# OPPO-Mente-Lab/PEA-Diffusion

Hardware: AMD Instinct MI355X
Metric: training images/sec (SDXL 1024px bf16, adapter-only bwd) (higher is better)
Workload: dtype bf16

## Files before the change

include/pea_hip.h:

```cpp
#ifndef PEA_HIP_H
#define PEA_HIP_H
#include <stdint.h>
#ifdef __cplusplus
extern "C" {
#endif

#define PEA_OK 0
#define PEA_E_INVALID (-1)
#define PEA_E_HIP (-2)
#define PEA_E_SHAPE (-3)
#define PEA_E_STATE (-4)
#define PEA_E_NOTFOUND (-5)
#define PEA_E_TIMEOUT (-6)

const char* pea_last_error(void);
int pea_version(void);
int pea_device_count(void);


int pea_op_gemm(const void* A, int lda, const void* W, int ldw, void* C, int ldc, int M, int N, int K, float alpha,
                const float* bias, const void* rowvec, int ldrv, int rows_per_batch, int act, void* preact,
                int ldpre, const void* res, int ldres, int out_f32, int accum_f32, void* stream);

int pea_op_gemm_qscale(const void* A, int lda, const void* W, int ldw, void* C, int ldc, int M, int N, int K, const float* bias,
                       int qscale_cols, float qscale, void* stream);

int pea_op_gemm_geglu(const void* A, int lda, const void* W, int ldw, const float* bias, void* y, void* stash, int M, int N,
                      int K, int stash_grad, int stash_rows, void* stream);

int pea_op_gemm_geglu_bwd(const void* A, int lda, const void* W, int ldw, const void* pre, int ldpre, void* C, int ldc,
                          int M, int N, int K, int form, void* stream);

int pea_op_ln_linear(const void* x, const float* gamma, const float* beta, const void* W, const float* bias, void* y,
                     void* geglu_y, int M, int N, int K, float eps, void* Wf, float* svec, float* tvec, float* stats,
                     void* stream);

int pea_op_conv3x3(const void* x, const void* w, void* y, int B, int Hs, int Ws, int Cin, int Cout, int stride,
                   int upsample2x, int transposed2, const float* bias, const void* rowvec, int ldrv,
                   const void* res, void* stream);
int pea_op_pack_conv(const float* w, void* out, int Co, int Ci, int dgrad, void* stream);
int pea_op_gemm_geglu_tanh(const void* A, int lda, const void* W, int ldw, const float* bias, void* y, void* stash, int M, int N,
                           int K, int stash_grad, int stash_rows, int geglu_tanh, void* stream);
int pea_op_gemm_splitk(const void* A, int lda, const void* W, int ldw, float* part, int ldc, long long split_stride, int M, int N,
                       int K, float alpha, int ksplit, void* stream);
int pea_op_conv3x3_ex(const void* x, const void* w, int ldw, void* y, int ldc, int B, int Hs, int Ws, int Cin, int Cout,
                      int stride, int pad_off, int act, const float* bias, const void* res, int ldres, void* stream);
int pea_op_pack_conv_padded(const float* w, void* out, int Co, int Ci, int Cip, void* stream);
int pea_op_pack_conv_subpixel(const float* w, void* out, int Co, int Ci, int dgrad, void* stream);
int pea_op_concat2(const void* a, int C1, const void* b, int C2, void* y, long long rows, int aH, int aW, void* stream);
int pea_op_split2(const void* dy, int C1, int C2, void* da, int accum_a, void* db, int accum_b, long long rows, int aH,
                  int aW, void* stream);
long long pea_op_freeu_scratch_bytes(int B, int H, int W, int C2);
int pea_op_freeu_coef(const void* skip, int B, int H, int W, int C2, float* coef, void* scratch, void* stream);
int pea_op_concat2_freeu(const void* a, int C1, const void* b, int C2, const float* coef, void* y, int B, int H, int W, float s,
                         float bscale, int aH, int aW, void* stream);
int pea_op_upconv_subpixel(const void* x, const void* w, void* y, int B, int Hs, int Ws, int Cin, int Cout,
                           const float* bias, void* stream);
int pea_op_upconv_subpixel_dgrad(const void* dy, const void* wt, void* dx, int B, int Hs, int Ws, int Cin, int Cout,
                                 const void* res, void* stream);
int pea_op_conv_in(const float* x_nchw, const float* w, const float* bias, void* y_nhwc, int B, int Cin, int H,
                   int W, int Cout, void* stream);
int pea_op_conv_in_gather(const float* latents, const float* mask, const float* masked_latents, const float* w,
                          const float* bias, void* y_nhwc, int B, int C, int latent_batch, int cond_batch, int H, int W,
                          int Cout, void* stream);
// ... 17 lines not shown
                         float* dgamma, float* dbeta, int R, int C, int accum, void* stream);

int pea_op_attention_fwd(const void* Q, int ldq, const void* K, int ldk, const void* V, int ldv, void* O, int ldo,
                         float* lse, int B, int H, int Sq, int Skv, float scale, int nd, void* stream);
int pea_op_attention_fwd_prescaled(const void* Q, int ldq, const void* K, int ldk, const void* V, int ldv, void* O, int ldo,
                                   float* lse, int B, int H, int Sq, int Skv, float scale, int nd, void* stream);
int pea_op_attention_fwd_masked(const void* Q, int ldq, const void* K, int ldk, const void* V, int ldv, void* O, int ldo,
                                float* lse, int B, int H, int Sq, int Skv, float scale, int causal, const int* kv_len,
                                void* stream);
int pea_op_attention_fwd_text(const void* Q, int ldq, const void* K, int ldk, const void* V, int ldv, void* O, int ldo,
                              float* lse, int B, int H, int Sq, int Skv, float scale, int q_prescaled, int causal,
                              const int* kv_len, const float* bias, void* stream);
int pea_op_attention_fwd_ip(const void* Q, int ldq, const void* K, int ldk, const void* V, int ldv, const void* K2, int ldk2,
                            const void* V2, int ldv2, void* O, int ldo, float* lse, int B, int H, int Sq, int Skv, int Skv2,
                            float scale, float ip_scale, int q_prescaled, int causal, const int* kv_len, void* stream);
typedef struct pea_attn_ip_sets {
  int n_sets;
  int n_keys[4];
  float weight[4];
  const float* mask[4];
  long long mask_stride[4];
} pea_attn_ip_sets;
int pea_op_attention_fwd_ipn(const void* Q, int ldq, const void* K, int ldk, const void* V, int ldv, const void* K2, int ldk2,
                             const void* V2, int ldv2, void* O, int ldo, float* lse, int B, int H, int Sq, int Skv,
                             const pea_attn_ip_sets* sets, float scale, int q_prescaled, int causal, const int* kv_len, void* stream);
int pea_op_attention_fwd_fewq(const void* Q, int ldq, const void* K, int ldk, const void* V, int ldv, const void* K2, int ldk2,
                              const void* V2, int ldv2, void* O, int ldo, float* lse, int B, int H, int Sq, int Skv, int Skv2,
                              float scale, int nd, int q_prescaled, void* stream);
long long pea_op_attention_bwd_scratch_bytes(int B, int H, int Sq, int Skv, int nd);
int pea_op_attention_bwd(const void* Q, int ldq, const void* K, int ldk, const void* V, int ldv, const void* O,
                         int ldo, const void* dO, int lddo, const float* lse, float* delta, void* dQ, int lddq,
                         void* dK, int lddk, void* dV, int lddv, int B, int H, int Sq, int Skv, float scale,
                         int accum_dq, int accum_dkv, int nd, void* scratch, void* stream);

int pea_op_attention_bwd_prescaled(const void* Q, int ldq, const void* K, int ldk, const void* V, int ldv, const void* O,
                                   int ldo, const void* dO, int lddo, const float* lse, float* delta, void* dQ, int lddq,
                                   void* dK, int lddk, void* dV, int lddv, int B, int H, int Sq, int Skv, float scale,
                                   int accum_dq, int accum_dkv, int nd, void* scratch, void* stream);

int pea_op_attention_bwd_masked(const void* Q, int ldq, const void* K, int ldk, const void* V, int ldv, const void* O,
                                int ldo, const void* dO, int lddo, const float* lse, float* delta, void* dQ, int lddq,
                                void* dK, int lddk, void* dV, int lddv, int B, int H, int Sq, int Skv, float scale,
                                int accum_dq, int accum_dkv, int nd, void* scratch, int q_prescaled, const int* kv_len,
                                void* stream);

int pea_op_geglu_fwd(const void* hg, void* y, long long rows, int inner, void* stream);
int pea_op_geglu_bwd(const void* hg, const void* dy, void* dhg, long long rows, int inner, void* stream);
int pea_op_sumpool2(const void* x, void* y, int B, int H, int W, int C, int accum, void* stream);
int pea_op_timestep_embed(const float* t, void* y, int n, int dim, void* stream);
int pea_op_add_noise(const float* x0, const float* eps, const long long* t, const float* ac, float* xt, int B,
                     long long per, void* stream);
int pea_op_cast_f32_bf16(const float* x, void* y, long long n, void* stream);
int pea_op_cast_bf16_f32(const void* x, float* y, long long n, void* stream);

int pea_op_inpaint_prepare(const float* image, const float* mask, int N, int H, int W, float* init_image, float* masked_image,
                           float* latent_mask, void* stream);
long long pea_op_cfg_combine_workspace_bytes(int B);
int pea_op_cfg_combine(const float* eps2, float* out, int B, long long per, float guidance_scale, float guidance_rescale,
                       void* workspace, void* stream);
int pea_op_dpm_update(float* sample, const float* eps, float* x0_prev, long long n, float alpha_s, float sigma_s,
                      float c_s, float c_0, float c_1, void* stream);
int pea_op_lcm_update(float* sample, const float* eps, const float* noise, float* denoised, long long n, float kx, float ke,
                      float c_prev, float c_noise, void* stream);
int pea_op_euler_update(float* sample, const float* eps, const float* noise, float* model_in, long long n, int dup, float k_e,
                        float k_n, float k_s, void* stream);

// ... 72 lines not shown
  int heads[4];
  int cross_dim;
  int linear_proj;
  int groups;
  float eps;
  int text_time;
  int add_time_dim;
  int proj_in_dim;
  int per_layer_depth;
  int depth_down[4][4];
  int depth_up[4][4];
  int depth_mid;
} pea_unet_config;

#define PEA_UNET_GRAD 1
#define PEA_UNET_RESIDUAL_INPUTS 2
#define PEA_UNET_INPAINT_INPUTS 4
int pea_unet_create(const pea_unet_config* cfg, int B, int H, int W, int L, int flags, int own_weights,
                    void** out);
int pea_unet_plan(const pea_unet_config* cfg, int B, int H, int W, int L, int flags, int* n_ops, int* n_weights,
                  long long* n_params, long long* weight_bytes, long long* act_bytes, long long* grad_bytes);
int pea_unet_create_cond(const pea_unet_config* cfg, int B, int H, int W, int L, int flags, int time_cond_proj_dim,
                         int own_weights, void** out);
int pea_unet_plan_cond(const pea_unet_config* cfg, int B, int H, int W, int L, int flags, int time_cond_proj_dim, int* n_ops,
                       int* n_weights, long long* n_params, long long* weight_bytes, long long* act_bytes,
                       long long* grad_bytes, int* n_attn, int* n_prescaled);
int pea_unet_plan_weight(const pea_unet_config* cfg, int B, int H, int W, int L, int flags, int time_cond_proj_dim,
                         const char* name, long long* numel, int* kind, int* d0, int* d1);
int pea_unet_set_timestep_cond(void* unet, const float* cond, void* stream);
int pea_unet_plan_scratch(const pea_unet_config* cfg, int B, int H, int W, int L, int flags, int bwd_batch,
                          long long* scratch_bytes);
int pea_tape_attention_census(void* graph, int* n_attn, int* n_prescaled);
int pea_unet_plan_attention(const pea_unet_config* cfg, int B, int H, int W, int L, int flags, int* n_attn, int* n_prescaled);
int pea_graph_plan_attention(int graph, const pea_unet_config* cfg, int B, int H, int W, int L, int* n_attn,
                             int* n_prescaled);
int pea_unet_num_residuals(void* unet);
int pea_unet_residual_info(void* unet, int i, int* C, int* H, int* W);
int pea_unet_set_residuals(void* unet, int n, const void* const* ptrs, int dtype, float scale, void* stream);
int pea_unet_set_inpaint_cond(void* unet, const float* mask, const float* masked_latents, int cond_batch, int latent_batch,
                              void* stream);
int pea_unet_clear_inpaint_cond(void* unet);
int pea_unet_set_freeu(void* unet, float s1, float s2, float b1, float b2, void* stream);
int pea_unet_clear_freeu(void* unet);
int pea_unet_ip_plan(const pea_unet_config* cfg, int n_tokens, int* n_layers, int* cols, long long* n_params);
int pea_unet_ip_create(void* unet, int n_tokens);
int pea_unet_ip_load_weight(void* unet, const char* key, const float* src, long long numel, void* stream);
int pea_unet_ip_set_tokens(void* unet, const float* tokens, void* stream);
int pea_unet_ip_set_scale(void* unet, float scale);
int pea_unet_ip_clear(void* unet);
int pea_unet_ip_destroy(void* unet);
int pea_unet_ip_export_kv(void* unet, float* out, long long* rows, int* cols, void* stream);
int pea_unet_ip_create_sets(void* unet, int n_sets, const int* n_tokens);
int pea_unet_ip_load_weight_set(void* unet, int set, const char* key, const float* src, long long numel, void* stream);
int pea_unet_ip_set_tokens_set(void* unet, int set, const float* tokens, void* stream);
int pea_unet_ip_set_scale_set(void* unet, int set, float scale);
int pea_unet_ip_clear_set(void* unet, int set);
int pea_unet_ip_set_layer_scales(void* unet, int set, const float* scales, int n_layers);
int pea_unet_ip_query_counts(void* unet, int* counts, int cap, int* n);
int pea_unet_ip_set_mask(void* unet, int set, int Sq, const float* mask, int Bm, void* stream);
int pea_unet_destroy(void* unet);

int pea_controlnet_create(const pea_unet_config* cfg, int B, int H, int W, int L, void** out);
int pea_controlnet_set_cond(void* cn, const float* image, void* stream);
int pea_controlnet_forward(void* cn, const float* x, const float* t, const void* ehs, int ehs_dtype, const void* text,
                           int text_dtype, const float* time_ids, void* stream);
int pea_controlnet_num_outputs(void* cn);
// ... 90 lines not shown
                   const long long* zh_or_not, const float* teacher_ehs, const float* teacher_neg,
                   const float* teacher_pooled, const float* time_ids, float grad_scale, float* grads,
                   int accumulate, float* losses, void* stream);
int pea_trainer_set_option(void* tr, const char* name, int value);
int pea_trainer_backward_context(void* trainer, void** unet);
int pea_trainer_get_option(void* trainer, const char* name);
int pea_trainer_release_activations(void* trainer);
int pea_trainer_export(void* tr, int which, float* out, void* stream);

int pea_comm_unique_id(void* out128);
int pea_comm_init(int rank, int world, const void* unique_id128, void** comm_out);
int pea_comm_init_timeout(int rank, int world, const void* unique_id128, double timeout_s, void** comm_out);
int pea_comm_destroy(void* comm);
int pea_comm_world(void* comm);
int pea_comm_rank(void* comm);
int pea_allreduce_grads(void* comm, float* grads, long long n, void* compute_stream);
int pea_comm_join(void* comm, void* stream);
int pea_comm_last_ms(void* comm, float* ms);
int pea_comm_last_exposed_ms(void* comm, float* ms);
int pea_comm_broadcast(void* comm, float* buf, long long n, int root, void* stream);

void pea_prof_enable(int on);
void pea_prof_reset(void);
const char* pea_prof_family_name(int fam);
int pea_prof_dump(const char* path);
int pea_prof_report(int fam, double* ms, double* flops, double* bytes, long long* launches);
int pea_probe_mfma_peak(double seconds, int shape32, double* tflops, double* clock_mhz, void* stream);

void pea_debug_set_attn_tr(int v);
void pea_debug_set_attn_fused_bwd(int v);
void pea_debug_set_attn_xattn(int v);
void pea_debug_set_xattn_bwd_v2(int v);
void pea_debug_set_geglu_bwd_fused(int v);
void pea_debug_set_gemm_variant(int v);
int pea_debug_gemm_dispatch(int M, int N, int K, int mode, int rows_per_batch, int features, int cus, int forced);
int pea_debug_attn_dispatch(const int* q, int* out);
void pea_debug_set_gemm_debug(int v);
void pea_debug_set_gemm_prefetch(const void* p, long long bytes);

int pea_op_attention_fwd_regions(const void* Q, int ldq, const void* K, int ldk, const void* V, int ldv, void* O, int ldo, int B, int H,
                                 int Sq, int R, int Lr, const float* w, int Bw, float scale, int q_prescaled, void* stream);
int pea_unet_set_prompt_regions(void* unet, int R, int Sq, const float* w, int Bw, void* stream);
int pea_unet_clear_prompt_regions(void* unet);
int pea_debug_attn_regions_dispatch(const int* q, int* out);

int pea_op_attention_maps(const void* Q, int ldq, const void* K, int ldk, float* maps, int B, int H, int Sq, int Skv, float scale,
                          int q_prescaled, const int* kv_len, int accumulate, void* stream);
int pea_unet_enable_attention_maps(void* unet, const float* layer_on, int n_layers);
int pea_unet_reset_attention_maps(void* unet, void* stream);
int pea_unet_disable_attention_maps(void* unet);
int pea_unet_attention_maps(void* unet, int Sq, float** maps, long long* n_accumulated);
int pea_debug_attn_maps_dispatch(const int* q, int* out);

int pea_op_attention_fwd_edit(const void* Q, int ldq, const void* K, int ldk, const void* V, int ldv, void* O, int ldo, int B, int H,
                              int Sq, int Skv, const int* src, const void* Mt, int ldm, const float* c, const float* d, float scale,
                              int q_prescaled, void* stream);
int pea_unet_set_prompt_edit(void* unet, const int* src, const void* Mt, const float* cd, int T, int self_until, int self_max_tokens,
                             void* stream);
int pea_unet_set_prompt_edit_step(void* unet, int step);
int pea_unet_clear_prompt_edit(void* unet);
int pea_debug_attn_edit_dispatch(const int* q, int* out);

long long pea_op_attn_adain_scratch_bytes(int B, int H, int S);
int pea_op_attn_adain_coef(const void* Q, int ldq, const void* K, int ldk, int B, int H, int S, const int* ref, float scale,
                           int q_prescaled, int adain_queries, int adain_keys, float* coef, void* scratch, void* stream);
int pea_op_attention_fwd_shared(const void* Q, int ldq, const void* K, int ldk, const void* V, int ldv, void* O, int ldo, int B, int H,
// ... 42 lines not shown
```

pea_diffusion_amd/csrc/api_model.hip:

```cpp
#include <string.h>

#include <algorithm>
#include <memory>

#include "../../include/pea_hip.h"
#include "model.h"

#define RCX(x)                        \
  do {                                \
    int rc__ = (x);                   \
    if (rc__ != PEA_OK) return rc__;  \
  } while (0)
static_assert(sizeof(pea_unet_config) == sizeof(PeaUnetCfg), "config struct mismatch");

static int finish_create(Tape* u, void** out) {
  int rc = u->build();
  if (rc == PEA_OK) rc = u->alloc();
  if (rc != PEA_OK) {
    delete u;
    return rc;
  }
  *out = u;
  return PEA_OK;
}
// ... 103 lines not shown
  Tape u;
  memcpy(&u.cfg, cfg, sizeof(PeaUnetCfg));
  u.B = B; u.H = H; u.W = W; u.L = L; set_flags(u, flags);
  u.bwd_batch = bwd_batch;
  u.plan_only = true;
  int rc = u.build();
  if (rc == PEA_OK) rc = u.alloc();
  if (rc != PEA_OK) return rc;
  size_t need[8];
  u.scratch_needs(need);
  long long t = 0;
  for (int i = 0; i < 8; ++i) t += (long long)need[i];
  *scratch_bytes = t;
  return PEA_OK;
}
int pea_tape_attention_census(void* h, int* n_attn, int* n_prescaled) {
  NOTNULL(h, "pea_tape_attention_census");
  const Tape* u = (const Tape*)h;
  if (n_attn) *n_attn = u->n_attn;
  if (n_prescaled) *n_prescaled = u->n_attn_pre;
  return PEA_OK;
}
int pea_unet_plan_attention(const pea_unet_config* cfg, int B, int H, int W, int L, int flags, int* n_attn, int* n_prescaled) {
  NOTNULL(cfg, "pea_unet_plan_attention");
  Tape u;
  memcpy(&u.cfg, cfg, sizeof(PeaUnetCfg));
  u.B = B; u.H = H; u.W = W; u.L = L; set_flags(u, flags);
  u.plan_only = true;
  int rc = u.build();
  if (rc == PEA_OK) rc = u.alloc();
  if (rc != PEA_OK) return rc;
  if (n_attn) *n_attn = u.n_attn;
  if (n_prescaled) *n_prescaled = u.n_attn_pre;
  return PEA_OK;
}
static int plan_census(Tape& u, int* n_attn, int* n_prescaled) {
  u.plan_only = true;
  int rc = u.build();
  if (rc == PEA_OK) rc = u.alloc();
  if (rc != PEA_OK) return rc;
  if (n_attn) *n_attn = u.n_attn;
  if (n_prescaled) *n_prescaled = u.n_attn_pre;
  return PEA_OK;
}
int pea_graph_plan_attention(int graph, const pea_unet_config* cfg, int B, int H, int W, int L, int* n_attn, int* n_prescaled) {
  NOTNULL(cfg, "pea_graph_plan_attention");
  if (graph < 1 || graph > 3) { pea_set_error("pea_graph_plan_attention: graph %d (1 VAE encoder, 2 ControlNet, 3 VAE decoder)", graph); return PEA_E_INVALID; }
  Tape u;
  memcpy(&u.cfg, cfg, sizeof(PeaUnetCfg));
  u.graph = graph;
  u.B = B; u.H = H; u.W = W; u.L = graph == 2 ? L : 0; u.needs_grad = false; u.owns_weights = true;
  return plan_census(u, n_attn, n_prescaled);
}
int pea_text_plan_attention(const pea_text_config* cfg, int B, int L, int* n_attn, int* n_prescaled) {
  NOTNULL(cfg, "pea_text_plan_attention");
  Tape u;
  memset(&u.cfg, 0, sizeof(PeaUnetCfg));
  memcpy(&u.tcfg, cfg, sizeof(PeaTextCfg));
  u.graph = 4;
  u.B = B; u.H = 1; u.W = L; u.L = L; u.needs_grad = false; u.owns_weights = true;
  return plan_census(u, n_attn, n_prescaled);
}
int pea_controlnet_create(const pea_unet_config* cfg, int B, int H, int W, int L, void** out) {
  NOTNULL(cfg, "pea_controlnet_create");
  NOTNULL(out, "pea_controlnet_create");
  RCX(require_device("pea_controlnet_create"));
// ... 621 lines not shown
```

pea_diffusion_amd/csrc/api_ops.hip:

```cpp
#include <stdarg.h>
#include <string.h>

#include "../../include/pea_hip.h"
#include "pea_kernels.h"

static thread_local char g_err[512] = "";
void pea_set_error(const char* fmt, ...) {
  va_list ap;
  va_start(ap, fmt);
  vsnprintf(g_err, sizeof(g_err), fmt, ap);
  va_end(ap);
}

static bf16* g_zero_page = nullptr;
int pea_zero_page(const bf16** out) {
  if (!g_zero_page) {
    HIPCHK(hipMalloc((void**)&g_zero_page, 256));
    HIPCHK(hipMemset(g_zero_page, 0, 256));
  }
  *out = g_zero_page;
  return PEA_OK;
}

template <class P = AttnP>
// ... 34 lines not shown
}

int pea_op_gemm(const void* A, int lda, const void* W, int ldw, void* C, int ldc, int M, int N, int K, float alpha,
                const float* bias, const void* rowvec, int ldrv, int rows_per_batch, int act, void* preact,
                int ldpre, const void* res, int ldres, int out_f32, int accum_f32, void* stream) {
  GemmP p;
  memset(&p, 0, sizeof(p));
  p.mode = 0;
  p.A = (const bf16*)A; p.lda = lda; p.W = (const bf16*)W; p.ldw = ldw; p.C = C; p.ldc = ldc;
  p.M = M; p.N = N; p.K = K; p.alpha = alpha; p.bias = bias;
  p.rowvec = (const bf16*)rowvec; p.ldrv = ldrv; p.rows_per_batch = rows_per_batch > 0 ? rows_per_batch : 1;
  p.act = act; p.preact = (bf16*)preact; p.ldpre = ldpre; p.res = (const bf16*)res; p.ldres = ldres;
  p.out_f32 = out_f32; p.accum_f32 = accum_f32;
  return launch_gemm(p, (hipStream_t)stream);
}

int pea_op_gemm_qscale(const void* A, int lda, const void* W, int ldw, void* C, int ldc, int M, int N, int K, const float* bias,
                       int qscale_cols, float qscale, void* stream) {
  GemmP p;
  memset(&p, 0, sizeof(p));
  p.A = (const bf16*)A; p.lda = lda; p.W = (const bf16*)W; p.ldw = ldw; p.C = C; p.ldc = ldc;
  p.M = M; p.N = N; p.K = K; p.alpha = 1.f; p.bias = bias; p.rows_per_batch = 1;
  p.qscale_cols = qscale_cols; p.qscale = qscale;
  return launch_gemm(p, (hipStream_t)stream);
}

int pea_op_gemm_geglu_bwd(const void* A, int lda, const void* W, int ldw, const void* pre, int ldpre, void* C, int ldc,
                          int M, int N, int K, int form, void* stream) {
  GemmP p;
  memset(&p, 0, sizeof(p));
  p.A = (const bf16*)A; p.lda = lda; p.W = (const bf16*)W; p.ldw = ldw; p.C = C; p.ldc = ldc;
  p.M = M; p.N = N; p.K = K; p.alpha = 1.f; p.rows_per_batch = 1;
  p.gbwd_pre = (const bf16*)pre; p.ldgp = ldpre; p.gbwd_form = form;
  return launch_gemm(p, (hipStream_t)stream);
}

int pea_op_gemm_geglu(const void* A, int lda, const void* W, int ldw, const float* bias, void* y, void* stash, int M, int N,
                      int K, int stash_grad, int stash_rows, void* stream) {
  GemmP p;
  memset(&p, 0, sizeof(p));
  p.A = (const bf16*)A; p.lda = lda; p.W = (const bf16*)W; p.ldw = ldw; p.bias = bias;
  p.M = M; p.N = N; p.K = K; p.alpha = 1.f; p.rows_per_batch = 1;
  p.geglu_y = (bf16*)y; p.ldy = N / 2; p.C = stash; p.ldc = N; p.stash_grad = stash_grad; p.stash_rows = stash_rows;
  return launch_gemm(p, (hipStream_t)stream);
}

int pea_op_gemm_geglu_tanh(const void* A, int lda, const void* W, int ldw, const float* bias, void* y, void* stash, int M, int N,
                           int K, int stash_grad, int stash_rows, int geglu_tanh, void* stream) {
  GemmP p;
  memset(&p, 0, sizeof(p));
  p.A = (const bf16*)A; p.lda = lda; p.W = (const bf16*)W; p.ldw = ldw; p.bias = bias;
  p.M = M; p.N = N; p.K = K; p.alpha = 1.f; p.rows_per_batch = 1;
  p.geglu_y = (bf16*)y; p.ldy = N / 2; p.C = stash; p.ldc = N; p.stash_grad = stash_grad; p.stash_rows = stash_rows;
  p.geglu_tanh = geglu_tanh ? 1 : 0;
  return launch_gemm(p, (hipStream_t)stream);
}

int pea_op_gemm_splitk(const void* A, int lda, const void* W, int ldw, float* part, int ldc, long long split_stride, int M, int N,
                       int K, float alpha, int ksplit, void* stream) {
  GemmP p;
  memset(&p, 0, sizeof(p));
  p.A = (const bf16*)A; p.lda = lda; p.W = (const bf16*)W; p.ldw = ldw; p.C = part; p.ldc = ldc;
  SHAPECHK(ksplit >= 2, "gemm_splitk: ksplit=%d (at least two splits)", ksplit);
  p.M = M; p.N = N; p.K = K; p.alpha = alpha; p.rows_per_batch = 1; p.out_f32 = 1;
  p.ksplit = ksplit; p.split_stride = split_stride;
  return launch_gemm(p, (hipStream_t)stream);
// ... 239 lines not shown
  return launch_attention_fwd_edit(p, (hipStream_t)stream);
}
long long pea_op_attn_adain_scratch_bytes(int B, int H, int S) { return (long long)attn_adain_scratch_bytes(B, H, S); }
int pea_op_attn_adain_coef(const void* Q, int ldq, const void* K, int ldk, int B, int H, int S, const int* ref, float scale,
                           int q_prescaled, int adain_queries, int adain_keys, float* coef, void* scratch, void* stream) {
  if (!ref) { pea_set_error("pea_op_attn_adain_coef: null ref (a host int[B]; negative entries for plain samples)"); return PEA_E_INVALID; }
  return launch_attn_adain_coef((const bf16*)Q, ldq, (const bf16*)K, ldk, B, H, S, ref, scale, q_prescaled, adain_queries, adain_keys,
                                coef, (float*)scratch, (hipStream_t)stream);
}
int pea_op_attention_fwd_shared(const void* Q, int ldq, const void* K, int ldk, const void* V, int ldv, void* O, int ldo, int B, int H,
                                int Sq, int Skv, const int* ref, const float* coef, float scale, int q_prescaled,
                                float shared_score_scale, float shared_score_shift, int nd, void* stream) {
  if (!ref) { pea_set_error("pea_op_attention_fwd_shared: null ref (a host int[B]; negative entries for plain samples)"); return PEA_E_INVALID; }
  AttnSharedP p = attn_operands<AttnSharedP>(Q, ldq, K, ldk, V, ldv, O, ldo, nullptr, B, H, Sq, Skv, scale, nd, q_prescaled);
  p.coef = coef; p.share_scale = shared_score_scale; p.share_shift = shared_score_shift;
  for (int b = 0; b < 32; ++b) p.ref[b] = b < B ? ref[b] : -1;
  return launch_attention_fwd_shared(p, (hipStream_t)stream);
}
int pea_op_attention_fwd_fewq(const void* Q, int ldq, const void* K, int ldk, const void* V, int ldv, const void* K2, int ldk2,
                              const void* V2, int ldv2, void* O, int ldo, float* lse, int B, int H, int Sq, int Skv, int Skv2,
                              float scale, int nd, int q_prescaled, void* stream) {
  AttnP p = attn_operands(Q, ldq, K, ldk, V, ldv, O, ldo, lse, B, H, Sq, Skv, scale, nd);
  p.q_prescaled = q_prescaled;
  p.K2 = (const bf16*)K2; p.V2 = (const bf16*)V2; p.ldk2 = ldk2; p.ldv2 = ldv2; p.Skv2 = Skv2;
  return launch_attention_fwd_fewq(p, (hipStream_t)stream);
}
int pea_op_attention_bwd(const void* Q, int ldq, const void* K, int ldk, const void* V, int ldv, const void* O,
                         int ldo, const void* dO, int lddo, const float* lse, float* delta, void* dQ, int lddq,
                         void* dK, int lddk, void* dV, int lddv, int B, int H, int Sq, int Skv, float scale,
                         int accum_dq, int accum_dkv, int nd, void* scratch, void* stream) {
  return attention_bwd_impl(Q, ldq, K, ldk, V, ldv, O, ldo, dO, lddo, lse, delta, dQ, lddq, dK, lddk, dV, lddv, B, H, Sq, Skv,
                            scale, accum_dq, accum_dkv, nd, scratch, 0, nullptr, stream);
}
int pea_op_attention_bwd_prescaled(const void* Q, int ldq, const void* K, int ldk, const void* V, int ldv, const void* O,
                                   int ldo, const void* dO, int lddo, const float* lse, float* delta, void* dQ, int lddq,
                                   void* dK, int lddk, void* dV, int lddv, int B, int H, int Sq, int Skv, float scale,
                                   int accum_dq, int accum_dkv, int nd, void* scratch, void* stream) {
  return attention_bwd_impl(Q, ldq, K, ldk, V, ldv, O, ldo, dO, lddo, lse, delta, dQ, lddq, dK, lddk, dV, lddv, B, H, Sq, Skv,
                            scale, accum_dq, accum_dkv, nd, scratch, 1, nullptr, stream);
}
int pea_op_attention_bwd_masked(const void* Q, int ldq, const void* K, int ldk, const void* V, int ldv, const void* O,
                                int ldo, const void* dO, int lddo, const float* lse, float* delta, void* dQ, int lddq,
                                void* dK, int lddk, void* dV, int lddv, int B, int H, int Sq, int Skv, float scale,
                                int accum_dq, int accum_dkv, int nd, void* scratch, int q_prescaled, const int* kv_len,
                                void* stream) {
  return attention_bwd_impl(Q, ldq, K, ldk, V, ldv, O, ldo, dO, lddo, lse, delta, dQ, lddq, dK, lddk, dV, lddv, B, H, Sq, Skv,
                            scale, accum_dq, accum_dkv, nd, scratch, q_prescaled, kv_len, stream);
}

int pea_op_geglu_fwd(const void* hg, void* y, long long rows, int inner, void* stream) {
  return launch_geglu_fwd((const bf16*)hg, (bf16*)y, rows, inner, (hipStream_t)stream);
}
int pea_op_geglu_bwd(const void* hg, const void* dy, void* dhg, long long rows, int inner, void* stream) {
  return launch_geglu_bwd((const bf16*)hg, (const bf16*)dy, (bf16*)dhg, rows, inner, (hipStream_t)stream);
}
int pea_op_sumpool2(const void* x, void* y, int B, int H, int W, int C, int accum, void* stream) {
  return launch_sumpool2((const bf16*)x, (bf16*)y, B, H, W, C, accum, (hipStream_t)stream);
}
int pea_op_timestep_embed(const float* t, void* y, int n, int dim, void* stream) {
  return launch_timestep_embed(t, (bf16*)y, n, dim, (hipStream_t)stream);
}
int pea_op_add_noise(const float* x0, const float* eps, const long long* t, const float* ac, float* xt, int B,
                     long long per, void* stream) {
  return launch_add_noise(x0, eps, t, ac, xt, B, per, (hipStream_t)stream);
}
int pea_op_cast_f32_bf16(const float* x, void* y, long long n, void* stream) {
// ... 252 lines not shown
```

pea_diffusion_amd/csrc/attention.hip:

```cpp
#include <stdlib.h>

#include "pea_kernels.h"

#define TILE_BYTES 8192
__device__ __forceinline__ float fast_exp2(float x) { return __builtin_amdgcn_exp2f(x); }
#define LOG2E 1.4426950408889634f
__device__ __forceinline__ float xhalf_max(float x) {
  float a = x, b = x;
  asm volatile("s_nop 1\n\tv_permlane32_swap_b32 %0, %1\n\ts_nop 1" : "+v"(a), "+v"(b));
  return fmaxf(a, b);
}

__device__ __forceinline__ bf16x8 scale_frag(bf16x8 f, float c) {
  bf16x8 o;
#pragma unroll
  for (int j = 0; j < 8; ++j) o[j] = (bf16)((float)f[j] * c);
  return o;
}
#define ATTN_MOVE_THR 8.0f

__device__ __forceinline__ int swz_x(int row) {
  const int x = (row >> 1) & 7;
  return ((x & 1) << 2) | (x >> 1);
}
// ... 227 lines not shown
      const float e = fast_exp2(sacc[kb][r]);
      sacc[kb][r] = e;
      ls += e;
    }
  l_run += ls;
  return mx;
}
__device__ __forceinline__ void attn_pack_p(const f32x16 (&sacc)[2], bf16x8 (&pf)[4]) {
#pragma unroll
  for (int ks = 0; ks < 4; ++ks)
#pragma unroll
    for (int j = 0; j < 8; ++j) pf[ks][j] = (bf16)sacc[ks >> 1][8 * (ks & 1) + j];
}
template <bool USE_TR>
__device__ __forceinline__ void attn_cols_product(const char* smem, const AttnFragOff& ro, int sub, const char* Ts, int lane,
                                                  const bf16x8 (&pf)[4], f32x16* acc) {
  bf16x8 tfr[4][2];
#pragma unroll
  for (int ks = 0; ks < 4; ++ks)
#pragma unroll
    for (int db = 0; db < 2; ++db) {
      if constexpr (USE_TR)
        tfr[ks][db] = read_transposed_frag_at(smem + ro.tr[db][0] + (sub + ks * 2048), smem + ro.tr[db][1] + (sub + ks * 2048));
      else tfr[ks][db] = read_transposed_frag<false>(Ts, ks * 16, db * 32, lane);
    }
  __builtin_amdgcn_sched_barrier(0);
#pragma unroll
  for (int ks = 0; ks < 4; ++ks)
#pragma unroll
    for (int db = 0; db < 2; ++db) acc[db] = __builtin_amdgcn_mfma_f32_32x32x16_bf16(tfr[ks][db], pf[ks], acc[db], 0, 0, 0);
}
template <int NO>
__device__ __forceinline__ void attn_fwd_exit(const f32x16 (&oacc)[2 * NO], float m_run, float l_run, float* lse, long long lse_i,
                                              bool lse_lane, char* ost, int lane, bf16* Ob, int ldo, int q0, int Sq) {
  float la = l_run, lb = l_run;
  swap_halves32(la, lb);
  const float l_tot = la + lb;
  const float inv = 1.f / l_tot;
  if (lse && lse_lane) lse[lse_i] = (m_run + log2f(l_tot)) * 0.6931471805599453f;
#pragma unroll
  for (int no = 0; no < NO; ++no)
    store_o_image_144(ost, lane, [&](int db, int i) { return oacc[2 * no + db][i] * inv; }, Ob + no * 64, ldo, q0, Sq);
}

template <int MODE, bool USE_TR, int ND, bool TXT, bool WRITE_DELTA>
__device__ __forceinline__ void attn_q_body(const AttnP& p, char* smem, int blk_x, int head, int b) {
  constexpr int STG = 2 * ND * TILE_BYTES;
  constexpr int NO = MODE == 0 ? ND : 1;
  const int tid = threadIdx.x, lane = tid & 63;
  const int wave = __builtin_amdgcn_readfirstlane(tid >> 6);
  const int qblk = MODE == 0 ? blk_x : blk_x / ND;
  const int chunk = MODE == 0 ? 0 : blk_x % ND;
  const int q0 = qblk * 128 + wave * 32;
  const int frow = lane & 31, fh = lane >> 5;
  const float c = p.scale * LOG2E;

  const bf16* Qb = p.Q + (long long)b * p.Sq * p.ldq + head * 64 * ND;
  const bf16* Kb = p.K + (long long)b * p.Skv * p.ldk + head * 64 * ND;
  const bf16* Vb = p.V + (long long)b * p.Skv * p.ldv + head * 64 * ND;

  int qrow = q0 + frow;
  const bool qvalid = qrow < p.Sq;
  qrow = qvalid ? qrow : p.Sq - 1;
  bf16x8 qf[ND][4], dof[MODE == 1 ? ND : 1][4];
#pragma unroll
  for (int nd = 0; nd < ND; ++nd)
#pragma unroll
    for (int s = 0; s < 4; ++s) {
      qf[nd][s] = *(const bf16x8*)(Qb + (long long)qrow * p.ldq + nd * 64 + 16 * s + 8 * fh);
      if (!p.q_prescaled && !TXT) qf[nd][s] = scale_frag(qf[nd][s], c);
    }
  [[maybe_unused]] const float qs = (TXT && !p.q_prescaled) ? c : 1.f;
  [[maybe_unused]] const float inv_qs = (TXT && !p.q_prescaled) ? 1.f / c : 1.f;
  float lse2 = 0.f, dlt = 0.f;
  if (MODE == 1) {
    const bf16* dOb = p.dO + (long long)b * p.Sq * p.lddo + head * 64 * ND;
#pragma unroll
    for (int nd = 0; nd < ND; ++nd)
#pragma unroll
      for (int s = 0; s < 4; ++s)
        dof[nd][s] = *(const bf16x8*)(dOb + (long long)qrow * p.lddo + nd * 64 + 16 * s + 8 * fh);
    const long long li = ((long long)b * p.H + head) * p.Sq + qrow;
    if (!WRITE_DELTA) {
      dlt = -p.delta[li];
      lse2 = -p.delta[(long long)p.B * p.H * p.Sq + li];
    } else {
      lse2 = p.lse[li] * LOG2E;
      const bf16* Ob = p.O + (long long)b * p.Sq * p.ldo + head * 64 * ND;
      float dsum = 0.f;
#pragma unroll
      for (int nd = 0; nd < ND; ++nd)
#pragma unroll
        for (int s = 0; s < 4; ++s) {
          const bf16x8 o = *(const bf16x8*)(Ob + (long long)qrow * p.ldo + nd * 64 + 16 * s + 8 * fh);
#pragma unroll
          for (int j = 0; j < 8; ++j) dsum += (float)dof[nd][s][j] * (float)o[j];
        }
      { float da = dsum, db = dsum; swap_halves32(da, db); dsum = da + db; }
      dlt = dsum;
      if (WRITE_DELTA && qvalid && fh == 0 && chunk == 0) {
        p.delta[li] = -dsum;
        p.delta[(long long)p.B * p.H * p.Sq + li] = -lse2;
      }
    }
  }
  f32x16 negd, rowc;
#pragma unroll
  for (int r = 0; r < 16; ++r) { negd[r] = -dlt; rowc[r] = MODE == 1 ? -lse2 : 0.f; }

  f32x16 oacc[2 * NO];
#pragma unroll
  for (int i = 0; i < 2 * NO; ++i)
#pragma unroll
    for (int r = 0; r < 16; ++r) oacc[i][r] = 0.f;
  float m_run = 0.f, l_run = 0.f;
  [[maybe_unused]] bool seen = false;

  TileSrc ksrc[ND], vsrc[ND];
#pragma unroll
  for (int nd = 0; nd < ND; ++nd) {
    ksrc[nd] = tile_src(Kb + nd * 64, p.ldk, p.Skv, wave, lane);
    vsrc[nd] = tile_src(Vb + nd * 64, p.ldv, p.Skv, wave, lane);
  }
  auto stage_kv = [&](char* dst, int r0) {
#pragma unroll
    for (int nd = 0; nd < ND; ++nd) {
      stage_tile(ksrc[nd], r0, dst + nd * TILE_BYTES, wave);
      stage_tile(vsrc[nd], r0, dst + (ND + nd) * TILE_BYTES, wave);
    }
  };
  const int nt = (p.Skv + 63) / 64;
  const int skv_all = __builtin_amdgcn_readfirstlane(p.kv_len ? p.kv_len[b] : p.Skv);
  stage_kv(smem, 0);
// ... 41 lines not shown
        attn_mask_tail(sacc, kv0, kmax, fh);
      }
      const float mx = attn_online_softmax<TXT>(sacc, TXT ? !seen : t == 0, m_run, l_run, oacc, rowc,
                                                [&](float m) { return TXT ? -m * inv_qs : -m; });
      if constexpr (TXT) seen = seen || mx > -INFINITY;
    } else {
      const int skv_b = skv_all;
      f32x16 dpacc[2];
      attn_rows_product<ND>(smem, ro, ND * TILE_BYTES, dof, negd, dpacc);
      if (kv0 + 64 > skv_b) {
        attn_mask_tail(sacc, kv0, skv_b, fh);
        __builtin_amdgcn_sched_barrier(0);
      }
#pragma unroll
      for (int kb = 0; kb < 2; ++kb)
#pragma unroll
        for (int r = 0; r < 16; ++r) {
          const float pr = fast_exp2(sacc[kb][r]);
          sacc[kb][r] = pr * dpacc[kb][r];
        }
    }
    bf16x8 pf[4];
    attn_pack_p(sacc, pf);
#pragma unroll
    for (int no = 0; no < NO; ++no)
      attn_cols_product<USE_TR>(smem, ro, no * TILE_BYTES, MODE == 0 ? Vs + no * TILE_BYTES : Ks + chunk * TILE_BYTES, lane, pf, oacc + 2 * no);
    WAIT_VM0();
    __syncthreads();
  }

  char* const ost = smem + wave * (32 * 144);
  if constexpr (MODE == 0)
    attn_fwd_exit<NO>(oacc, m_run, l_run, p.lse, ((long long)b * p.H + head) * p.Sq + qrow, qvalid && fh == 0, ost, lane,
                      p.O + (long long)b * p.Sq * p.ldo + head * 64 * ND, p.ldo, q0, p.Sq);
  else
    store_o_image_144(ost, lane, [&](int db, int i) { return oacc[db][i] * p.scale; }, p.dQ + (long long)b * p.Sq * p.lddq + head * 64 * ND + chunk * 64,
                      p.lddq, q0, p.Sq, p.accum_dq != 0);
}

template <int MODE, bool USE_TR, int ND, bool TXT = false>
__global__ __launch_bounds__(256, (ND == 1 ? (MODE == 0 ? 3 : 2) : 1)) void attn_q_kernel(const AttnP p) {
  extern __shared__ __attribute__((aligned(16))) char smem[];
  int blk_x, head, b;
  attn_block_coords(blk_x, head, b);
  attn_q_body<MODE, USE_TR, ND, TXT, true>(p, smem, blk_x, head, b);
}

struct AttnKeyLane { int k0, krow; bool kstored, wave_active; };
__device__ __forceinline__ AttnKeyLane attn_key_lane(int kblk, int wave, int frow, int Skv) {
  AttnKeyLane k;
  k.k0 = kblk * 128 + wave * 32;
  k.kstored = k.k0 + frow < Skv;
  k.krow = k.kstored ? k.k0 + frow : Skv - 1;
  k.wave_active = k.k0 < Skv;
  return k;
}
__device__ __forceinline__ void stage_rowconst(const float* src, int r0, int rmax, char* dst, int lane) {
  int r = r0 + lane;
  r = r < rmax ? r : rmax - 1;
  lds_dma4(src + r, dst);
}

template <bool USE_TR, int ND>
__device__ __forceinline__ void attn_dkv_body(const AttnP& p, char* smem, int blk_x, int head, int b) {
  constexpr int STG = 2 * ND * TILE_BYTES + 512;
  const int tid = threadIdx.x, lane = tid & 63;
  const int wave = __builtin_amdgcn_readfirstlane(tid >> 6);
  const int nsplit = p.nsplit > 1 ? p.nsplit : 1;
  const int chunk = blk_x % ND;
  const int bx = blk_x / ND;
  const int kblk = bx / nsplit, split = bx - kblk * nsplit;
  const int frow = lane & 31, fh = lane >> 5;
  const auto [k0, krow, kstored, wave_active] = attn_key_lane(kblk, wave, frow, p.Skv);
  const float c = p.scale * LOG2E;

  const bf16* Qb = p.Q + (long long)b * p.Sq * p.ldq + head * 64 * ND;
  const bf16* dOb = p.dO + (long long)b * p.Sq * p.lddo + head * 64 * ND;
  const bf16* Kb = p.K + (long long)b * p.Skv * p.ldk + head * 64 * ND;
  const bf16* Vb = p.V + (long long)b * p.Skv * p.ldv + head * 64 * ND;
  const float* dltb = p.delta + ((long long)b * p.H + head) * p.Sq;
  const float* lseb = dltb + (long long)p.B * p.H * p.Sq;

  const int skv_b = p.kv_len ? p.kv_len[b] : p.Skv;
  const bool kvalid = k0 + frow < skv_b;
  bf16x8 kf[ND][4], vf[ND][4];
#pragma unroll
  for (int nd = 0; nd < ND; ++nd)
#pragma unroll
    for (int s = 0; s < 4; ++s) {
      kf[nd][s] = *(const bf16x8*)(Kb + (long long)krow * p.ldk + nd * 64 + 16 * s + 8 * fh);
      if (!p.q_prescaled) kf[nd][s] = scale_frag(kf[nd][s], c);
      vf[nd][s] = *(const bf16x8*)(Vb + (long long)krow * p.ldv + nd * 64 + 16 * s + 8 * fh);
    }
  f32x16 dk[2], dv[2];
#pragma unroll
  for (int i = 0; i < 2; ++i)
#pragma unroll
    for (int r = 0; r < 16; ++r) dk[i][r] = dv[i][r] = 0.f;
  const bool all_valid = __all(kvalid);

  TileSrc qsrc[ND], dosrc[ND];
#pragma unroll
  for (int nd = 0; nd < ND; ++nd) {
    qsrc[nd] = tile_src(Qb + nd * 64, p.ldq, p.Sq, wave, lane);
    dosrc[nd] = tile_src(dOb + nd * 64, p.lddo, p.Sq, wave, lane);
  }
  auto stage_q = [&](char* dst, int r0) {
#pragma unroll
    for (int nd = 0; nd < ND; ++nd) {
      stage_tile(qsrc[nd], r0, dst + nd * TILE_BYTES, wave);
      stage_tile(dosrc[nd], r0, dst + (ND + nd) * TILE_BYTES, wave);
    }
    if (wave == 0) {
      stage_rowconst(lseb, r0, p.Sq, dst + 2 * ND * TILE_BYTES, lane);
      stage_rowconst(dltb, r0, p.Sq, dst + 2 * ND * TILE_BYTES + 256, lane);
    }
  };
  const int nt_all = (p.Sq + 63) / 64;
  const int tps = (nt_all + nsplit - 1) / nsplit;
  const int t_begin = split * tps;
  const int nt = min(nt_all, t_begin + tps);
  if (t_begin < nt) stage_q(smem, t_begin * 64);
  WAIT_VM0();
  __syncthreads();

  for (int t = t_begin; t < nt; ++t) {
    const int cur = (t - t_begin) & 1;
    if (t + 1 < nt) stage_q(smem + (cur ^ 1) * STG, (t + 1) * 64);
    const char* Qs = smem + cur * STG;
    const char* dOs = Qs + ND * TILE_BYTES;
    const float* rc = (const float*)(Qs + 2 * ND * TILE_BYTES);
    if (t * 64 + 64 > p.Sq) {
      if (wave == 0 && t * 64 + lane >= p.Sq) {
        float* rw = (float*)(Qs + 2 * ND * TILE_BYTES);
        rw[lane] = -INFINITY;
        rw[64 + lane] = 0.f;
      }
      __syncthreads();
    }
    if (wave_active) {
      f32x16 sacc[2], dpacc[2];
      bf16x8 rq[2][ND * 4], rd[2][ND * 4];
      auto load_rows = [&](int buf, int qb) {
#pragma unroll
        for (int nd = 0; nd < ND; ++nd)
#pragma unroll
          for (int s = 0; s < 4; ++s) {
            rq[buf][nd * 4 + s] = read_row_frag(Qs + nd * TILE_BYTES, qb * 32 + frow, s, fh);
            rd[buf][nd * 4 + s] = read_row_frag(dOs + nd * TILE_BYTES, qb * 32 + frow, s, fh);
          }
#pragma unroll
        for (int g = 0; g < 4; ++g) {
          const f32x4 d4 = *(const f32x4*)(rc + 64 + qb * 32 + 8 * g + 4 * fh);
          const f32x4 l4 = *(const f32x4*)(rc + qb * 32 + 8 * g + 4 * fh);
#pragma unroll
          for (int j = 0; j < 4; ++j) {
            dpacc[qb][4 * g + j] = d4[j];
            sacc[qb][4 * g + j] = l4[j];
          }
        }
      };
// ... 26 lines not shown
        __builtin_amdgcn_sched_barrier(0);
      }
      bf16x8 pfr[4], dsfr[4];
#pragma unroll
      for (int qb = 0; qb < 2; ++qb)
#pragma unroll
        for (int g = 0; g < 4; ++g) {
#pragma unroll
          for (int j = 0; j < 4; ++j) {
            const int r = 4 * g + j;
            const float pr = fast_exp2(sacc[qb][r]);
            const float ds = pr * dpacc[qb][r];
            const int ks = qb * 2 + (g >> 1), e = (g & 1) * 4 + j;
            pfr[ks][e] = (bf16)pr;
            dsfr[ks][e] = (bf16)ds;
          }
        }
      __builtin_amdgcn_sched_barrier(0);
      load_tr(0);
      load_tr(1);
      __builtin_amdgcn_sched_barrier(0);
#pragma unroll
      for (int bt = 0; bt < 2; ++bt) {
#pragma unroll
        for (int kk = 0; kk < 2; ++kk)
#pragma unroll
          for (int db = 0; db < 2; ++db) {
            dv[db] = __builtin_amdgcn_mfma_f32_32x32x16_bf16(dot[bt][kk][db], pfr[2 * bt + kk], dv[db], 0, 0, 0);
            dk[db] = __builtin_amdgcn_mfma_f32_32x32x16_bf16(qt[bt][kk][db], dsfr[2 * bt + kk], dk[db], 0, 0, 0);
          }
        __builtin_amdgcn_sched_barrier(0);
      }
    }
    WAIT_VM0();
    __syncthreads();
  }
  const bool lds_epi = p.nsplit <= 1 && !p.accum_dkv;
  if (lds_epi ? !wave_active : !kstored) return;
#pragma unroll
  for (int i = 0; i < 2; ++i)
#pragma unroll
    for (int r = 0; r < 16; ++r) dk[i][r] *= p.q_prescaled ? 0.6931471805599453f : p.scale;
  const int D = 64 * ND;
  if (p.nsplit > 1) {
    float* pr = p.dkv_part + ((((long long)split * p.B + b) * p.H + head) * p.Skv + krow) * 2 * D + chunk * 64;
#pragma unroll
    for (int db = 0; db < 2; ++db)
#pragma unroll
      for (int g = 0; g < 4; ++g) {
        const int d = db * 32 + 8 * g + 4 * fh;
        f32x4 a, cc;
#pragma unroll
        for (int j = 0; j < 4; ++j) { a[j] = dk[db][4 * g + j]; cc[j] = dv[db][4 * g + j]; }
        *(f32x4*)(pr + d) = a;
        *(f32x4*)(pr + D + d) = cc;
      }
    return;
  }
  if (lds_epi) {
    char* const ost = smem + wave * (32 * 144);
    store_o_image_144(ost, lane, [&](int db, int i) { return dk[db][i]; }, p.dK + (long long)b * p.Skv * p.lddk + head * D + chunk * 64,
                      p.lddk, k0, p.Skv, p.accum_dkv != 0);
    store_o_image_144(ost, lane, [&](int db, int i) { return dv[db][i]; }, p.dV + (long long)b * p.Skv * p.lddv + head * D + chunk * 64,
                      p.lddv, k0, p.Skv, p.accum_dkv != 0);
    return;
  }
  bf16* dKr = p.dK + ((long long)b * p.Skv + krow) * p.lddk + head * D + chunk * 64;
  bf16* dVr = p.dV + ((long long)b * p.Skv + krow) * p.lddv + head * D + chunk * 64;
#pragma unroll
  for (int db = 0; db < 2; ++db)
#pragma unroll
    for (int g = 0; g < 4; ++g) {
      const int d = db * 32 + 8 * g + 4 * fh;
      bf16x4 ok, ov;
      if (p.accum_dkv) {
        ok = *(const bf16x4*)(dKr + d);
        ov = *(const bf16x4*)(dVr + d);
      }
#pragma unroll
      for (int j = 0; j < 4; ++j) {
        ok[j] = (bf16)(dk[db][4 * g + j] + (p.accum_dkv ? (float)ok[j] : 0.f));
        ov[j] = (bf16)(dv[db][4 * g + j] + (p.accum_dkv ? (float)ov[j] : 0.f));
      }
      *(bf16x4*)(dKr + d) = ok;
      *(bf16x4*)(dVr + d) = ov;
    }
}

template <bool USE_TR, int ND>
__global__ __launch_bounds__(256, (ND == 1 ? 2 : 1)) void attn_dkv_kernel(const AttnP p) {
  extern __shared__ __attribute__((aligned(16))) char smem[];
  int blk_x, head, b;
  attn_block_coords(blk_x, head, b);
  attn_dkv_body<USE_TR, ND>(p, smem, blk_x, head, b);
}

template <bool USE_TR, int ND>
__global__ __launch_bounds__(256, (ND == 1 ? 2 : 1)) void attn_bwd_fused_kernel(const AttnP p, int n_dq, int n_dkv) {
  extern __shared__ __attribute__((aligned(16))) char smem[];
  const unsigned lin = xcd_contiguous(blockIdx.x, gridDim.x);
  const int per_head = n_dq + n_dkv;
  const int bh = (int)(lin / per_head), rem = (int)(lin - (unsigned)bh * per_head);
  const int b = bh / p.H, head = bh - b * p.H;
  if (rem < n_dkv) attn_dkv_body<USE_TR, ND>(p, smem, rem, head, b);
  else attn_q_body<1, USE_TR, ND, false, false>(p, smem, rem - n_dkv, head, b);
}

struct XattnCtx {
  int split, head, b, u_begin, u_end, skv_b;
  float c;
  const bf16 *Qb, *dOb, *Ob, *Kb, *Vb;
  const float* lseb;
};
template <int UQ, int PRE = -1>
__device__ __forceinline__ XattnCtx xattn_ctx(const AttnP& p, int upw) {
  XattnCtx x;
  attn_block_coords(x.split, x.head, x.b);
  const int nu = (p.Sq + UQ - 1) >> (UQ == 128 ? 7 : 6);
  x.u_begin = x.split * upw;
  x.u_end = min(nu, x.u_begin + upw);
  x.c = (PRE < 0 ? p.q_prescaled != 0 : PRE != 0) ? 1.f : p.scale * LOG2E;
  x.Qb = p.Q + (long long)x.b * p.Sq * p.ldq + x.head * 64;
  x.dOb = p.dO + (long long)x.b * p.Sq * p.lddo + x.head * 64;
  x.Ob = p.O + (long long)x.b * p.Sq * p.ldo + x.head * 64;
  x.Kb = p.K + (long long)x.b * p.Skv * p.ldk + x.head * 64;
  x.Vb = p.V + (long long)x.b * p.Skv * p.ldv + x.head * 64;
  x.lseb = p.lse + ((long long)x.b * p.H + x.head) * p.Sq;
  x.skv_b = __builtin_amdgcn_readfirstlane(p.kv_len ? p.kv_len[x.b] : p.Skv);
  return x;
}
__device__ __forceinline__ float xhalf_sum(float x) {
  float a = x, b = x;
  asm volatile("s_nop 1\n\tv_permlane32_swap_b32 %0, %1\n\ts_nop 1" : "+v"(a), "+v"(b));
  return a + b;
}

__device__ __forceinline__ f32x16 zero_f32x16() {
  return f32x16{0.f, 0.f, 0.f, 0.f, 0.f, 0.f, 0.f, 0.f, 0.f, 0.f, 0.f, 0.f, 0.f, 0.f, 0.f, 0.f};
// ... 1665 lines not shown
  if (idx >= total) return;
  const int d4 = (int)(idx % D4) * 4;
  long long r = idx / D4;
  const int which = (int)(r & 1); r >>= 1;
  const int key = (int)(r % p.Skv); r /= p.Skv;
  const int head = (int)(r % p.H);
  const int b = (int)(r / p.H);
  f32x4 acc = {0.f, 0.f, 0.f, 0.f};
  for (int s = 0; s < p.nsplit; ++s) {
    const f32x4 v = *(const f32x4*)(p.dkv_part + ((((long long)s * p.B + b) * p.H + head) * p.Skv + key) * 2 * D +
                                    which * D + d4);
#pragma unroll
    for (int j = 0; j < 4; ++j) acc[j] += v[j];
  }
  bf16* dst = which ? p.dV + ((long long)b * p.Skv + key) * p.lddv + head * D + d4
                    : p.dK + ((long long)b * p.Skv + key) * p.lddk + head * D + d4;
  bf16x4 o;
  if (p.accum_dkv) o = *(const bf16x4*)dst;
#pragma unroll
  for (int j = 0; j < 4; ++j) o[j] = (bf16)(acc[j] + (p.accum_dkv ? (float)o[j] : 0.f));
  *(bf16x4*)dst = o;
}

enum AttnKernel : int {
  AK_XFWD = 0, AK_Q = 12, AK_Q_TXT = 24, AK_DKV = 25, AK_FUSED = 31, AK_XBWD1 = 37, AK_XBWD2 = 41, AK_XBWD3 = 45, AK_FEWQ = 49,
  AK_DELTA = 50, AK_REDUCE = 51, AK_COUNT = 52
};
struct AttnLaunch { int kernel; dim3 grid; int lds, a0, a1; };
struct AttnPlan {
  AttnLaunch l[3]; int n = 0, nsplit = 1;
  void add(int kernel, dim3 grid, int lds, int a0 = 0, int a1 = 0) { l[n++] = AttnLaunch{kernel, grid, lds, a0, a1}; }
};
struct AttnEnv { int xattn_ver, use_tr, xattn, fused_bwd; };
static AttnEnv g_attn_env = {getenv("PEA_XATTN_BWD_VER") ? atoi(getenv("PEA_XATTN_BWD_VER")) : 3, 1, getenv("PEA_XATTN_OFF") ? 0 : 1,
                             getenv("PEA_ATTN_BWD_SPLIT") ? 0 : 1};
extern "C" void pea_debug_set_xattn_bwd_v2(int v) { g_attn_env.xattn_ver = v; }
extern "C" void pea_debug_set_attn_tr(int v) { g_attn_env.use_tr = v; }
extern "C" void pea_debug_set_attn_xattn(int v) { g_attn_env.xattn = v; }
extern "C" void pea_debug_set_attn_fused_bwd(int v) { g_attn_env.fused_bwd = v; }
static bool xattn_v2_keys(int Skv, const AttnEnv& e) { return e.xattn_ver && Skv > 32 && Skv <= 96; }
static int wgs_per_cu(int lds) { return 2 * lds <= 160 * 1024 ? 2 : 1; }
static int wg_slots(int per_cu) { return 256 * per_cu; }
static int units_per_wg(long long units, int nu, int per_cu) {
  const long long upw = (units + wg_slots(per_cu) - 1) / wg_slots(per_cu);
  return (int)(upw < 1 ? 1 : (upw > nu ? nu : upw));
}
static int attn_nsplit(int B, int H, int Sq, int Skv, const AttnEnv& e) {
  if (Skv > 128 || Sq < 512) return 1;
  const bool v2 = xattn_v2_keys(Skv, e);
  const int uq = v2 ? 64 : 128;
  const int fixed = v2 ? 2 : 0;
  const int nu = (Sq + uq - 1) / uq;
  const long long bh = (long long)B * H;
  long long best = -1;
  int best_ns = 1;
  for (int u = 1; u <= nu; ++u) {
    const int ns = (nu + u - 1) / u;
    const long long rounds = (bh * ns + wg_slots(2) - 1) / wg_slots(2);
    const long long cost = rounds * (u + fixed) * (uq / 2) + ns;
    if (best < 0 || cost < best) { best = cost; best_ns = ns; }
  }
  return best_ns;
}
int attention_bwd_nsplit(int B, int H, int Sq, int Skv) { return attn_nsplit(B, H, Sq, Skv, g_attn_env); }
size_t attention_bwd_scratch_bytes(int B, int H, int Sq, int Skv, int nd) {
  const int ns = attention_bwd_nsplit(B, H, Sq, Skv);
  return ns > 1 ? (size_t)ns * B * H * Skv * 128 * nd * sizeof(float) : 0;
}
static bool attn_resident_kv(const AttnP& p, const AttnEnv& e) { return e.xattn && e.use_tr && p.nd == 1 && p.Skv <= 128; }
static int attn_decide_fwd(const AttnP& p, const AttnEnv& e, AttnPlan& plan) {
  const int nu = cdiv(p.Sq, 128);
  if (p.K2 || (attn_resident_kv(p, e) && !p.causal && !p.bias && p.Sq >= 128)) {
    const int kb = cdiv(p.Skv, 32), kt = (kb + 1) / 2;
    const int lds = 2 * kt * TILE_BYTES + 4 * 32 * 144 + 4 * 4096 + (p.K2 ? 2 * 4096 : 0);
    const int upw = units_per_wg((long long)p.B * p.H * nu, nu, 2);
    plan.add(AK_XFWD + 4 * (!p.K2 ? 0 : p.nset ? 2 : 1) + (kb - 1), dim3(cdiv(nu, upw), p.H, p.B), lds, upw);
    return PEA_OK;
  }
  const bool txt = p.causal || p.kv_len || p.bias;
  SHAPECHK(!txt || p.nd == 1, "attention: causal / key-length masks need head_dim 64");
  plan.add(txt ? AK_Q_TXT : AK_Q + 3 * (e.use_tr != 0) + (p.nd - 1), dim3(nu, p.H, p.B), 2 * 2 * p.nd * TILE_BYTES);
  return PEA_OK;
}
static int attn_decide_bwd(const AttnP& p, const AttnEnv& e, AttnPlan& plan) {
  const int ns = plan.nsplit = p.dkv_part ? attn_nsplit(p.B, p.H, p.Sq, p.Skv, e) : 1;
  const int nd = p.nd, tr = e.use_tr != 0;
  bool all = p.dQ && p.dK && p.dV, partials = true;
  if (attn_resident_kv(p, e) && all) {
    const int kb = cdiv(p.Skv, 32);
    const dim3 grid(ns, p.H, p.B);
    if (xattn_v2_keys(p.Skv, e)) {
      const bool v3 = e.xattn_ver != 2 && p.Skv <= 80;
      const int lds = v3 ? 2 * (TILE_BYTES + TILE_BYTES / 2) + 2 * (2 * TILE_BYTES + 512) + 2 * (TILE_BYTES + 2048)
                         : 4 * TILE_BYTES + 2 * (2 * TILE_BYTES + 512) + 2 * 32 * 144;
      plan.add((v3 ? AK_XBWD3 : AK_XBWD2) + 2 * (kb - 2) + (p.q_prescaled != 0), grid, lds, cdiv(cdiv(p.Sq, 64), ns));
    } else {
      plan.add(AK_XBWD1 + (kb - 1), grid, 4 * TILE_BYTES + (4 * TILE_BYTES + 1024), cdiv(cdiv(p.Sq, 128), ns));
    }
  } else {
    const int lq = 2 * 2 * nd * TILE_BYTES, lk = 2 * (2 * nd * TILE_BYTES + 512);
    const int n_dq = cdiv(p.Sq, 128) * nd, n_dkv = cdiv(p.Skv, 128) * ns * nd;
    const bool fused = all && e.fused_bwd;
    if (fused || !p.dQ) plan.add(AK_DELTA, dim3((unsigned)cdivl((long long)p.B * p.Sq * p.H * 8, 256 * ATTN_DELTA_ROWS)), 0);
    partials = fused || (p.dK && p.dV);
    if (fused) plan.add(AK_FUSED + 3 * tr + (nd - 1), dim3((unsigned)((n_dq + n_dkv) * p.H * p.B)), lk, n_dq, n_dkv);
    if (!fused && p.dQ) plan.add(AK_Q + 6 + 3 * tr + (nd - 1), dim3(n_dq, p.H, p.B), lq);
    if (!fused && partials) plan.add(AK_DKV + 3 * tr + (nd - 1), dim3(n_dkv, p.H, p.B), lk);
  }
  if (ns > 1 && partials) plan.add(AK_REDUCE, dim3((unsigned)cdivl((long long)p.B * p.H * p.Skv * 2 * 16 * nd, 256)), 0);
  return PEA_OK;
}
static int attn_check_ip(const AttnP& p) {
  SHAPECHK(p.K2 != nullptr && p.V2 != nullptr, "attention: a second key set needs both K2 and V2");
  SHAPECHK(p.nd == 1, "attention: a second key set needs head_dim 64 (nd=%d)", p.nd);
  SHAPECHK(!p.causal && !p.bias, "attention: a second key set cannot be combined with a causal mask or a score bias");
  SHAPECHK(p.Skv <= 128, "attention: a second key set needs at most 128 text keys (Skv=%d)", p.Skv);
  SHAPECHK(p.Skv2 >= 1 && p.Skv2 <= 32, "attention: the second key set holds 1..32 keys (Skv2=%d)", p.Skv2);
  SHAPECHK(p.ldk2 % 8 == 0 && p.ldv2 % 8 == 0 && p.ldk2 >= 64 * p.H && p.ldv2 >= 64 * p.H,
           "attention: ldk2 / ldv2 must be multiples of 8 and hold every head (ldk2=%d ldv2=%d)", p.ldk2, p.ldv2);
  SHAPECHK(p.nset >= 0 && p.nset <= 4, "attention: 1..4 image key sets (%d)", p.nset);
  for (int j = 0, lo = 0; j < p.nset; lo = p.set_end[j++]) {
    SHAPECHK(p.set_end[j] > lo, "attention: image key set %d is empty", j);
    SHAPECHK(!p.set_mask[j] || p.set_mstride[j] == 0 || p.set_mstride[j] >= p.Sq,
             "attention: the mask of image key set %d has batch stride %lld: 0 (shared) or >= Sq=%d", j, p.set_mstride[j], p.Sq);
  }
  SHAPECHK(p.nset == 0 || p.set_end[p.nset - 1] == p.Skv2, "attention: the image key sets end at row %d of %d", p.set_end[p.nset - 1], p.Skv2);
  return PEA_OK;
}
static void attn_resolve_sets(AttnP& p) {
  if (!p.nset) return;
  bool any = false;
  for (int j = 0; j < p.nset; ++j) any = any || p.set_w[j] != 0.f;
  if (!any) {
    p.K2 = p.V2 = nullptr;
    p.nset = 0;
  } else if (p.nset == 1 && !p.set_mask[0]) {
// ... 46 lines not shown
    SHAPECHK(p.k2_brows == 0 || p.k2_brows >= p.Skv2, "attention: %d image key rows per sample hold no %d keys", p.k2_brows, p.Skv2);
    if (!p.k2_brows) p.k2_brows = p.Skv2;
    attn_resolve_sets(p);
  }
  return attn_decide_fwd(p, e, plan);
}
template <auto K, int THREADS = 256, int LIMIT = 0, typename... Args>
static int launch_lds(dim3 grid, int bytes, hipStream_t s, const Args&... args) {
  static bool raised = false;
  if (!raised) {
    HIPCHK(hipFuncSetAttribute((const void*)K, hipFuncAttributeMaxDynamicSharedMemorySize, LIMIT ? LIMIT : bytes));
    raised = true;
  }
  hipLaunchKernelGGL(K, grid, dim3(THREADS), bytes, s, args...);
  return PEA_OK;
}
static int attn_launch(const AttnLaunch& l, const AttnP& p, hipStream_t s) {
#define ATTN_CASE(e, K, ...) case e: return launch_lds<K>(l.grid, l.lds, s, p, ##__VA_ARGS__);
  switch (l.kernel) {
    ATTN_CASE(AK_XFWD + 0, (xattn_fwd_kernel<1, false, false>), l.a0) ATTN_CASE(AK_XFWD + 1, (xattn_fwd_kernel<2, false, false>), l.a0)
    ATTN_CASE(AK_XFWD + 2, (xattn_fwd_kernel<3, false, false>), l.a0) ATTN_CASE(AK_XFWD + 3, (xattn_fwd_kernel<4, false, false>), l.a0)
    ATTN_CASE(AK_XFWD + 4, (xattn_fwd_kernel<1, true, false>), l.a0) ATTN_CASE(AK_XFWD + 5, (xattn_fwd_kernel<2, true, false>), l.a0)
    ATTN_CASE(AK_XFWD + 6, (xattn_fwd_kernel<3, true, false>), l.a0) ATTN_CASE(AK_XFWD + 7, (xattn_fwd_kernel<4, true, false>), l.a0)
    ATTN_CASE(AK_XFWD + 8, (xattn_fwd_kernel<1, true, true>), l.a0) ATTN_CASE(AK_XFWD + 9, (xattn_fwd_kernel<2, true, true>), l.a0)
    ATTN_CASE(AK_XFWD + 10, (xattn_fwd_kernel<3, true, true>), l.a0) ATTN_CASE(AK_XFWD + 11, (xattn_fwd_kernel<4, true, true>), l.a0)
    ATTN_CASE(AK_Q + 0, (attn_q_kernel<0, false, 1>)) ATTN_CASE(AK_Q + 1, (attn_q_kernel<0, false, 2>)) ATTN_CASE(AK_Q + 2, (attn_q_kernel<0, false, 3>))
    ATTN_CASE(AK_Q + 3, (attn_q_kernel<0, true, 1>)) ATTN_CASE(AK_Q + 4, (attn_q_kernel<0, true, 2>)) ATTN_CASE(AK_Q + 5, (attn_q_kernel<0, true, 3>))
    ATTN_CASE(AK_Q + 6, (attn_q_kernel<1, false, 1>)) ATTN_CASE(AK_Q + 7, (attn_q_kernel<1, false, 2>)) ATTN_CASE(AK_Q + 8, (attn_q_kernel<1, false, 3>))
    ATTN_CASE(AK_Q + 9, (attn_q_kernel<1, true, 1>)) ATTN_CASE(AK_Q + 10, (attn_q_kernel<1, true, 2>)) ATTN_CASE(AK_Q + 11, (attn_q_kernel<1, true, 3>))
    ATTN_CASE(AK_Q_TXT, (attn_q_kernel<0, true, 1, true>)) ATTN_CASE(AK_FEWQ, attn_fewq_kernel)
    ATTN_CASE(AK_DKV + 0, (attn_dkv_kernel<false, 1>)) ATTN_CASE(AK_DKV + 1, (attn_dkv_kernel<false, 2>)) ATTN_CASE(AK_DKV + 2, (attn_dkv_kernel<false, 3>))
    ATTN_CASE(AK_DKV + 3, (attn_dkv_kernel<true, 1>)) ATTN_CASE(AK_DKV + 4, (attn_dkv_kernel<true, 2>)) ATTN_CASE(AK_DKV + 5, (attn_dkv_kernel<true, 3>))
    ATTN_CASE(AK_FUSED + 0, (attn_bwd_fused_kernel<false, 1>), l.a0, l.a1) ATTN_CASE(AK_FUSED + 1, (attn_bwd_fused_kernel<false, 2>), l.a0, l.a1)
    ATTN_CASE(AK_FUSED + 2, (attn_bwd_fused_kernel<false, 3>), l.a0, l.a1) ATTN_CASE(AK_FUSED + 3, (attn_bwd_fused_kernel<true, 1>), l.a0, l.a1)
    ATTN_CASE(AK_FUSED + 4, (attn_bwd_fused_kernel<true, 2>), l.a0, l.a1) ATTN_CASE(AK_FUSED + 5, (attn_bwd_fused_kernel<true, 3>), l.a0, l.a1)
    ATTN_CASE(AK_XBWD1 + 0, xattn_bwd_kernel<1>, l.a0) ATTN_CASE(AK_XBWD1 + 1, xattn_bwd_kernel<2>, l.a0)
    ATTN_CASE(AK_XBWD1 + 2, xattn_bwd_kernel<3>, l.a0) ATTN_CASE(AK_XBWD1 + 3, xattn_bwd_kernel<4>, l.a0)
    ATTN_CASE(AK_XBWD2 + 0, (xattn_bwd2_kernel<2, false>), l.a0) ATTN_CASE(AK_XBWD2 + 1, (xattn_bwd2_kernel<2, true>), l.a0)
    ATTN_CASE(AK_XBWD2 + 2, (xattn_bwd2_kernel<3, false>), l.a0) ATTN_CASE(AK_XBWD2 + 3, (xattn_bwd2_kernel<3, true>), l.a0)
    ATTN_CASE(AK_XBWD3 + 0, (xattn_bwd3_kernel<2, false>), l.a0) ATTN_CASE(AK_XBWD3 + 1, (xattn_bwd3_kernel<2, true>), l.a0)
    ATTN_CASE(AK_XBWD3 + 2, (xattn_bwd3_kernel<3, false>), l.a0) ATTN_CASE(AK_XBWD3 + 3, (xattn_bwd3_kernel<3, true>), l.a0)
    case AK_DELTA: hipLaunchKernelGGL(attn_delta_kernel, l.grid, dim3(256), 0, s, p); return PEA_OK;
    case AK_REDUCE: hipLaunchKernelGGL(attn_dkv_reduce_kernel, l.grid, dim3(256), 0, s, p); return PEA_OK;
  }
#undef ATTN_CASE
  pea_set_error("attention: no kernel for enumerator %d", l.kernel);
  return PEA_E_SHAPE;
}
static int attn_go(int dir, const AttnP& p0, hipStream_t s) {
  AttnP p = p0;
  AttnPlan plan;
  int rc = attn_plan(dir, p, g_attn_env, plan);
  if (rc) return rc;
  const int keys = p.Skv + (dir != 1 && p.K2 ? p.Skv2 : 0);
  if (g_prof_on) { g_prof_tag[0] = p.B * p.H; g_prof_tag[1] = p.Sq; g_prof_tag[2] = dir == 2 ? keys : p.Skv; g_prof_tag[3] = p.nd; }
  const double w = dir == 1 ? 4.0 : 2.0;
  PROF_BEGIN(dir == 1 ? 3 : 2, (dir == 1 ? 10.0 : 4.0) * p.B * p.H * (double)p.Sq * keys * 64 * p.nd,
             2.0 * p.B * p.H * 64 * p.nd * (w * p.Sq + w * keys), s);
  for (int i = 0; i < plan.n && !rc; ++i) rc = attn_launch(plan.l[i], p, s);
  PROF_END(s);
  if (rc) return rc;
  HIPCHK(hipGetLastError());
  return PEA_OK;
}
int launch_attention_fwd(const AttnP& p, hipStream_t s) { return attn_go(0, p, s); }
int launch_attention_bwd(const AttnP& p, hipStream_t s) { return attn_go(1, p, s); }
int launch_attention_fwd_fewq(const AttnP& p, hipStream_t s) { return attn_go(2, p, s); }
static float g_standin_page[64] __attribute__((aligned(16)));
template <class F>
static F attn_standin(int B, int H, int Sq, int Skv, int nd, int ldk = 0) {
  AttnP a = AttnP();
  a.Q = a.K = a.V = a.O = (bf16*)g_standin_page; a.scale = 0.125f;
  a.B = B; a.H = H; a.Sq = Sq; a.Skv = Skv; a.nd = nd;
  a.ldq = a.ldk = a.ldv = a.ldo = 64 * H * (nd > 0 ? nd : 1);
  if (ldk > 0) a.ldk = ldk;
  return attn_feature_p<F>(a);
}
extern "C" int pea_debug_attn_dispatch(const int* q, int* out) {
  const int dir = q[0], feat = q[6];
  if (dir < 0 || dir > 2) return q[1] >= 0 && q[1] < AK_COUNT ? q[1] : -1;
  const AttnEnv e = {q[10] < 0 ? g_attn_env.xattn_ver : q[10], q[11] < 0 ? g_attn_env.use_tr : q[11],
                     q[12] < 0 ? g_attn_env.xattn : q[12], q[13] < 0 ? g_attn_env.fused_bwd : q[13]};
  float* const page = g_standin_page;
  bf16* const any = (bf16*)page;
  AttnP p = attn_standin<AttnP>(q[1], q[2], q[3], q[4], q[5]);
  p.dO = any; p.lse = p.delta = page;
  p.lddo = p.lddq = p.lddk = p.lddv = p.ldk2 = p.ldv2 = p.ldq;
  p.causal = feat & 1; p.kv_len = feat & 2 ? (const int*)page : nullptr; p.bias = feat & 4 ? page : nullptr; p.q_prescaled = feat >> 3 & 1;
  if (feat & 16) { p.K2 = p.V2 = any; p.Skv2 = q[7]; p.scale2 = 1.f; p.nset = dir == 2 ? 0 : q[8]; }
  for (int j = 0; j < p.nset && j < 4; ++j) {
    p.set_end[j] = (int)((long long)(j + 1) * p.Skv2 / p.nset);
    p.set_w[j] = feat & 32 ? 0.f : 1.f;
    p.set_mask[j] = q[9] >> j & 1 ? page : nullptr;
  }
  p.dQ = feat & 64 ? any : nullptr; p.dK = feat & 128 ? any : nullptr; p.dV = feat & 256 ? any : nullptr;
  p.dkv_part = feat & 512 ? page : nullptr; p.accum_dq = p.accum_dkv = feat >> 10 & 1;
  AttnPlan plan;
  const int rc = attn_plan(dir, p, e, plan);
  if (rc) return rc;
  out[0] = plan.n; out[1] = plan.nsplit;
  for (int i = 0; i < plan.n; ++i) {
    const AttnLaunch& l = plan.l[i];
    int* const o = out + 2 + 7 * i;
    o[0] = l.kernel; o[1] = (int)l.grid.x; o[2] = (int)l.grid.y; o[3] = (int)l.grid.z; o[4] = l.lds; o[5] = l.a0; o[6] = l.a1;
  }
  return PEA_OK;
}

struct AttnOperands { const bf16 *Q, *K, *V; int ldq, ldk, ldv; const bf16* O; int ldo, o_bytes; const void *f32, *f32_opt; bool need_f32; };
static int attn_check_operands(const char* who, const AttnOperands& a, int H, float scale) {
  SHAPECHK(a.Q && a.K && a.V && (a.O || !a.o_bytes) && (a.f32 || !a.need_f32), "%s: null operand", who);
  SHAPECHK(scale > 0.f && scale <= 3.0e38f, "%s: a finite positive scale (%g)", who, (double)scale);
  const int C = 64 * H;
  SHAPECHK(a.ldq % 8 == 0 && a.ldk % 8 == 0 && a.ldv % 8 == 0 && a.ldq >= C && a.ldk >= C && a.ldv >= C,
           "%s: leading dimensions ldq / ldk / ldv must be multiples of 8 and hold every head (%d %d %d)", who, a.ldq, a.ldk, a.ldv);
  SHAPECHK(!a.o_bytes || (a.ldo % (a.o_bytes / 2) == 0 && a.ldo >= C),
           "%s: leading dimension ldo must be a multiple of %d and hold every head (ldo=%d)", who, a.o_bytes / 2, a.ldo);
  const unsigned long long in_bits = (unsigned long long)a.Q | (unsigned long long)a.K | (unsigned long long)a.V;
  SHAPECHK(in_bits % 16 == 0 && (!a.o_bytes || (unsigned long long)a.O % a.o_bytes == 0) &&
               ((unsigned long long)a.f32 | (unsigned long long)a.f32_opt) % 4 == 0,
           "%s: Q / K / V 16-byte, O %d-byte, fp32 operands 4-byte aligned", who, a.o_bytes);
  return PEA_OK;
}
template <class Launch>
static int attn_feature_launch(int BH, int Sq, int keys, double flops, double bytes, hipStream_t s, Launch launch) {
  if (g_prof_on) { g_prof_tag[0] = BH; g_prof_tag[1] = Sq; g_prof_tag[2] = keys; g_prof_tag[3] = 1; }
  PROF_BEGIN(2, flops, bytes, s);
  const int rc = launch();
  PROF_END(s);
// ... 528 lines not shown
```

pea_diffusion_amd/csrc/attn_features.hip:

```cpp
#include <stdio.h>
#include <string.h>

#include <algorithm>
#include <memory>

#include "../../include/pea_hip.h"
#include "model.h"

#define REFUSE(rc, ...)         \
  do {                          \
    pea_set_error(__VA_ARGS__); \
    return rc;                  \
  } while (0)

static const Op* kv_stack_op(const Tape& u) {
  const Op* kv = nullptr;
  for (const Op& o : u.ops)
    if (o.out == u.t_kvall && o.fused >= 0) kv = &o;
  return kv;
}
int Tape::ip_live_set() const {
  for (int j = 0; ip && j < ip->nsets; ++j)
    if (ip->set[j].live) return j;
  return -1;
// ... 174 lines not shown
}

static AttnRegionsP regions_p(const Tape::RegionState& st, const AttnP& p) {
  AttnRegionsP r = attn_feature_p<AttnRegionsP>(p);
  const auto& wt = st.w.find(p.Sq)->second;
  r.R = st.R; r.Lr = p.Skv / st.R; r.w = wt.first; r.Bw = wt.second;
  return r;
}
static AttnEditP edit_p(const Tape::EditState& st, const AttnP& p, int L) {
  AttnEditP e = attn_feature_p<AttnEditP>(p);
  e.Mt = st.Mt; e.ldm = st.ldm;
  e.c = st.cd + (size_t)st.step * 2 * p.B * L; e.d = e.c + (size_t)p.B * L;
  memcpy(e.src, st.src, sizeof(e.src));
  return e;
}
static AttnSharedP shared_p(const Tape::StyleState& st, const AttnP& p) {
  AttnSharedP e = attn_feature_p<AttnSharedP>(p);
  e.coef = st.coef; e.share_scale = st.share_scale; e.share_shift = st.share_shift;
  memcpy(e.ref, st.ref, sizeof(e.ref));
  return e;
}
static AttnColsumP colsum_p(const Tape::SagState& st, const AttnP& p) {
  AttnColsumP c = attn_feature_p<AttnColsumP>(p);
  c.Q = p.Q + (size_t)st.first * p.Sq * p.ldq; c.K = p.K + (size_t)st.first * p.Skv * p.ldk; c.B = st.n;
  c.lse = st.lse + (size_t)st.first * p.H * p.Sq; c.part = st.part;
  return c;
}
static AttnMapsP maps_p(float* acc, const int* kv_len, const AttnP& p) {
  AttnMapsP m = attn_feature_p<AttnMapsP>(p);
  m.maps = acc; m.kv_len = kv_len; m.accumulate = 1;
  return m;
}

int Tape::attn_forward(size_t oi, hipStream_t s) {
  const Op& o = ops[oi];
  const bool text = o.b == t_kvall;
  AttnP p; memset(&p, 0, sizeof(p));
  p.Q = tn[o.a].d + o.acol; p.ldq = tn[o.a].cols; p.K = tn[o.b].d + o.bcol; p.ldk = tn[o.b].cols;
  p.V = tn[o.c].d + o.ccol; p.ldv = tn[o.c].cols; p.O = tn[o.out].d; p.ldo = tn[o.out].cols; p.lse = o.aux;
  p.B = B; p.H = o.p0; p.Sq = o.p1; p.Skv = o.p2; p.scale = o.f0; p.nd = o.p3;
  p.causal = o.mask & 1; p.kv_len = (o.mask & 2) ? kvlen : nullptr;
  p.q_prescaled = o.pre;
  if (o.mask & 4) p.bias = rel_bias;
  if (cross_kvlen && text) p.kv_len = cross_kvlen;
  if (regions && text) return launch_attention_fwd_regions(regions_p(*regions, p), s);
  if (edit && text && edit->cd_live[edit->step])
    return launch_attention_fwd_edit(edit_p(*edit, p, L), s);
  if (ip && text) RC(ip_attach(o, p));
  if (style && style->n_targets && is_self_attn(o) && style->on[style->layer_of_op.find((int)oi)->second]) {
    RC(launch_attn_adain_coef(p.Q, p.ldq, p.K, p.ldk, B, o.p0, o.p1, style->ref, o.f0, o.pre, style->adain_q, style->adain_k,
                              style->coef, style->scratch, s));
    return launch_attention_fwd_shared(shared_p(*style, p), s);
  }
  const int perturbed = perturb && is_self_attn(o) && perturb->on[perturb->layer_of_op.find((int)oi)->second] ? perturb->mode : 0;
  if (perturbed == PerturbState::BLUR) {
    const PerturbState::Grid& g = perturb->grid.find(o.p1)->second;
    RC(launch_query_blur((bf16*)p.Q + (size_t)perturb->first * p.Sq * p.ldq, p.ldq, B - perturb->first, g.h, g.w, 64 * p.H, g.Mh, g.Mw, s));
  }
  if (perturbed == PerturbState::IDENTITY) p.B = perturb->first;
  const bool sag_here = sag && sag->op == (int)oi;
  if (sag_here) p.lse = sag->lse;
  RC(launch_attention_fwd(p, s));
  if (perturbed == PerturbState::IDENTITY) {
    p.B = B;
    RC(launch_copy2d(p.V + (size_t)perturb->first * p.Skv * p.ldv, p.ldv, p.O + (size_t)perturb->first * p.Sq * p.ldo, p.ldo,
                     (long long)(B - perturb->first) * p.Sq, 64 * p.H, 0, s));
  }
  if (sag_here) RC(launch_attention_colsum(colsum_p(*sag, p), s));
  if (edit && graph == 0 && !text && !o.mask && o.p1 == o.p2 && o.p1 <= edit->self_max_tokens && edit->step < edit->self_until) {
    for (int b = 0; b < B; ++b) {
      const int sb = edit->src[b];
      if (sb < 0) continue;
      AttnP e = p;
      e.B = 1; e.lse = nullptr;
      e.Q = p.Q + (size_t)sb * p.Sq * p.ldq; e.K = p.K + (size_t)sb * p.Skv * p.ldk;
      e.V = p.V + (size_t)b * p.Skv * p.ldv; e.O = p.O + (size_t)b * p.Sq * p.ldo;
      RC(launch_attention_fwd(e, s));
    }
  }
  if (maps && text) {
    const auto lay = maps->layer_of_col.find(o.bcol);
    if (lay != maps->layer_of_col.end() && maps->on[lay->second]) {
      RC(launch_attention_maps(maps_p(maps->acc.find(o.p1)->second, cross_kvlen, p), s));
      ++maps->count[o.p1];
    }
  }
  return PEA_OK;
}

static int unet_handle(void* h, const char* who, bool text, const char* why, Tape** out) {
  NOTNULL(h, who);
  Tape* const u = (Tape*)h;
  if (u->graph != 0 || (text && u->t_kvall < 0)) {
    char fmt[160];
// ... 502 lines not shown
```

pea_diffusion_amd/csrc/gemm.hip:

```cpp
#include <stdint.h>
#include <stdlib.h>

#include <type_traits>

#include "pea_kernels.h"

#define BK 64
constexpr int GEMM_ILV_M = 1;
constexpr int GEMM_ILV_HEAD = 4;

__device__ __forceinline__ int swz_off(int row, int chunk) { return row * 128 + ((chunk ^ ((row >> 1) & 7)) << 4); }

#ifdef PEA_GEMM_PROBES
#define PEA_PROBE(bit) (p.debug & (bit))
#else
#define PEA_PROBE(bit) false
#endif

template <int N>
__device__ __forceinline__ void wait_vmcnt() {
  static_assert(N >= 0 && N < 64, "vmcnt is a 6-bit counter");
  asm volatile("s_waitcnt vmcnt(%0)" ::"n"(N) : "memory");
}

// ... 215 lines not shown
        f32x4 o;
        if (p.accum_f32) {
          o = *(const f32x4*)cp;
#pragma unroll
          for (int j = 0; j < 4; ++j) o[j] += v[j];
        } else {
#pragma unroll
          for (int j = 0; j < 4; ++j) o[j] = v[j];
        }
        *(f32x4*)cp = o;
      } else {
        bf16x4 o;
#pragma unroll
        for (int j = 0; j < 4; ++j) o[j] = (bf16)v[j];
        *(bf16x4*)((bf16*)p.C + (long long)m * p.ldc + n) = o;
      }
    }
  }
}

typedef __attribute__((ext_vector_type(4))) unsigned epi_u32x4;
typedef __attribute__((ext_vector_type(2))) unsigned epi_u32x2;
template <typename T>
__device__ __forceinline__ void epi_consumed(const T& v) { asm volatile("" :: "v"(v)); }
__device__ __forceinline__ void epi_store16(void* ptr, epi_u32x4 v) { *(epi_u32x4*)ptr = v; }
__device__ __forceinline__ void epi_store8(void* ptr, epi_u32x2 v) { *(epi_u32x2*)ptr = v; }
__device__ __forceinline__ void epi_store4(void* ptr, unsigned v) { *(unsigned*)ptr = v; }
template <int MT, int NT, int EK = 0>
__device__ __forceinline__ void gemm_epilogue16_fast(const GemmP& p, f32x4 (&acc)[NT][MT], int m_base, int n_base, int r16,
                                                     int q4) {
  constexpr bool LNF = EK == 1;
  typedef __attribute__((ext_vector_type(4))) unsigned u32x4;
  typedef __attribute__((ext_vector_type(2))) unsigned u32x2;
  f32x4 bq[NT];
#pragma unroll
  for (int nt = 0; nt < NT; ++nt) bq[nt] = (f32x4){0.f, 0.f, 0.f, 0.f};
  if (p.bias) {
#pragma unroll
    for (int nt = 0; nt < NT; ++nt) bq[nt] = *(const f32x4*)(p.bias + min(n_base + nt * 16 + 4 * q4, p.N - 4));
  }
  bf16x4 rvq[NT];
  if (!LNF && p.rowvec) {
    const int bidx = min(m_base, p.M - 1) / p.rows_per_batch;
#pragma unroll
    for (int nt = 0; nt < NT; ++nt)
      rvq[nt] = *(const bf16x4*)(p.rowvec + (long long)bidx * p.ldrv + min(n_base + nt * 16 + 4 * q4, p.N - 4));
  }
  if (!LNF && p.rowvec) {
#pragma unroll
    for (int nt = 0; nt < NT; ++nt)
#pragma unroll
      for (int j = 0; j < 4; ++j) bq[nt][j] += (float)rvq[nt][j];
  }
  const bool has_res = !LNF && p.res != nullptr;
  float al[NT];
#pragma unroll
  for (int nt = 0; nt < NT; ++nt) {
    const float f = (n_base + nt * 16 < p.qscale_cols) ? p.qscale : 1.f;
    al[nt] = p.alpha * f;
    if (p.qscale_cols > 0) {
#pragma unroll
      for (int j = 0; j < 4; ++j) bq[nt][j] *= f;
    }
  }
  f32x4 sq[LNF ? NT : 1];
  float2 st[LNF ? MT : 1];
// ... 335 lines not shown
__device__ __forceinline__ __amdgpu_buffer_rsrc_t tile_rsrc(const GemmP& p, int bm, int& org) {
  long long first, left;
  if (MODE == 0) {
    org = __builtin_amdgcn_readfirstlane(bm * BM);
    first = (long long)org * p.lda;
    left = (long long)(p.M - org) * p.lda;
  } else {
    const int hw = p.Ho * p.Wo;
    const long long sample = (long long)p.Hs * p.Ws * conv_pix(p);
    org = __builtin_amdgcn_readfirstlane((bm * BM) / hw);
    first = org * sample;
    left = (p.M / hw - org) * sample;
  }
  return __builtin_amdgcn_make_buffer_rsrc((void*)(p.A + first), 0, (int)min(left * 2, 0x7f000000LL), 0x00020000);
}
#endif

template <int MT, int NT>
__device__ __forceinline__ void mfma_half_interleaved(f32x4 (&acc)[NT][MT], const bf16x8 (&wf)[NT], const bf16x8 (&af)[MT]) {
#pragma unroll
  for (int nt = 0; nt < NT; ++nt)
#pragma unroll
    for (int mt = 0; mt < MT; ++mt)
      acc[nt][mt] = __builtin_amdgcn_mfma_f32_16x16x32_bf16(wf[nt], af[mt], acc[nt][mt], 0, 0, 0);
  __builtin_amdgcn_sched_group_barrier(0x008, GEMM_ILV_HEAD, 0);
#pragma unroll
  for (int i = 0; i < MT + NT; ++i) {
    __builtin_amdgcn_sched_group_barrier(0x100, 1, 0);
    __builtin_amdgcn_sched_group_barrier(0x008, GEMM_ILV_M, 0);
  }
  __builtin_amdgcn_sched_group_barrier(0x008, MT * NT, 0);
}
template <int MODE, int BM, int BN, int WM, int WN, int LW, int S, bool PROBE16 = false, bool M16 = false, int MINW = 1,
          bool LNF = false, bool KSW = false>
__global__ __launch_bounds__((WM * WN * (KSW ? 2 : 1) + LW) * 64, MINW) void gemm_lc_kernel(const bf16* pl_A, const bf16* pl_W, int pl_lda, int pl_ldw, int pl_M,
                                                                           int pl_N, int pl_K, int pl_ksplit, int pl_debug, const GemmP p_in) {
  GemmP p = p_in;
  p.A = pl_A; p.W = pl_W; p.lda = pl_lda; p.ldw = pl_ldw; p.M = pl_M; p.N = pl_N; p.K = pl_K; p.ksplit = pl_ksplit; p.debug = pl_debug;
  extern __shared__ __attribute__((aligned(16))) char smem[];
  constexpr int NWC = WM * WN * (KSW ? 2 : 1);
  constexpr int STAGE = (BM + BN) * 128;
  constexpr int A_BYTES = BM * 128;
  constexpr int PA = BM / 8 / LW, PB = BN / 8 / LW;
  constexpr int PP = PA + PB;
  constexpr int MI = BM / WM / 32, NI = BN / WN / 32;
  static_assert(BM % (8 * LW) == 0 && BN % (8 * LW) == 0, "tile / loader split");
  const int tid = threadIdx.x;
  const int lane = tid & 63;
  const int wave = __builtin_amdgcn_readfirstlane(tid >> 6);

  const int nbm = (p.M + BM - 1) / BM, nbn = (p.N + BN - 1) / BN;
  const int nwg = nbm * nbn;
  int bid = blockIdx.x;
  {
    const int q = nwg >> 3, r = nwg & 7, xcd = bid & 7, idx = bid >> 3;
    bid = (xcd < r ? xcd * (q + 1) : r * (q + 1) + (xcd - r) * q) + idx;
  }
  constexpr int GROUP = BM >= 256 ? 4 : 8;
  const int per_group = GROUP * nbn;
  const int gid = bid / per_group;
  const int first_m = gid * GROUP;
  const int gsize = min(nbm - first_m, GROUP);
  const int bm = first_m + (bid % per_group) % gsize;
  const int bn = (bid % per_group) / gsize;
  int nt = p.K / BK, kt0 = 0;
  if (p.ksplit > 1) {
    const int per = (nt + p.ksplit - 1) / p.ksplit;
// ... 154 lines not shown
      for (int j = 0; j < MH; ++j)
#pragma unroll
        for (int n_ = 0; n_ < NT; ++n_) {
          const f32x4 o = *(const f32x4*)(theirs + (j * NT + n_) * 1024);
          const f32x4 a = acc[n_][K0 + j];
          if constexpr (K0 == 0) fin[n_][j] = (f32x4){a[0] + o[0], a[1] + o[1], a[2] + o[2], a[3] + o[3]};
          else fin[n_][j] = (f32x4){o[0] + a[0], o[1] + a[1], o[2] + a[2], o[3] + a[3]};
        }
    };
    if (wk == 0) xchg(std::integral_constant<int, MH>{}, std::integral_constant<int, 0>{});
    else xchg(std::integral_constant<int, 0>{}, std::integral_constant<int, MH>{});
    const int keep0 = wk == 0 ? 0 : MH;
    gemm_epilogue16_fast<MH, NT>(p, fin, bm * BM + wr * (BM / WM) + keep0 * 16, bn * BN + wc * (BN / WN), r16, q4);
    return;
  }
  if constexpr (M16) {
    constexpr int MT = BM / WM / 16, NT = BN / WN / 16;
    const int wr = wave / WN, wc = wave % WN;
    const int r16 = lane & 15, q4 = lane >> 4;
    const int a_row0 = wr * (BM / WM) + r16, w_row0 = wc * (BN / WN) + r16;
    f32x4 acc[NT][MT];
#pragma unroll
    for (int i = 0; i < NT; ++i)
#pragma unroll
      for (int j = 0; j < MT; ++j) acc[i][j] = (f32x4){0.f, 0.f, 0.f, 0.f};
    bf16x8 af[2][MT], wf[2][NT];
    auto load_frags = [&](int which, const char* tile, int s2) {
#pragma unroll
      for (int mt = 0; mt < MT; ++mt) af[which][mt] = *(const bf16x8*)(tile + swz_off(a_row0 + mt * 16, 4 * s2 + q4));
#pragma unroll
      for (int nt = 0; nt < NT; ++nt)
        wf[which][nt] = *(const bf16x8*)(tile + A_BYTES + swz_off(w_row0 + nt * 16, 4 * s2 + q4));
    };
    __builtin_amdgcn_s_barrier();
    load_frags(0, smem, 0);
    int cur = 0;
    for (int t = 0; t < nt; ++t) {
      const char* tile = smem + cur * STAGE;
      const int nxt = cur + 1 == S ? 0 : cur + 1;
#pragma unroll
      for (int s2 = 0; s2 < 2; ++s2) {
        bool late_frags = false;
        if (s2 == 1) {
          if (t + 1 < nt) {
            asm volatile("s_waitcnt lgkmcnt(0)" ::: "memory");
            __builtin_amdgcn_s_barrier();
            late_frags = true;
          }
        } else if (MT < 4) {
          load_frags(1, tile, 1);
        }
#pragma unroll
        for (int nt_ = 0; nt_ < NT; ++nt_) {
#pragma unroll
          for (int mt = 0; mt < MT; ++mt)
            acc[nt_][mt] = __builtin_amdgcn_mfma_f32_16x16x32_bf16(wf[s2][nt_], af[s2][mt], acc[nt_][mt], 0, 0, 0);
          if (nt_ == 0 && (s2 == 1 || MT >= 4)) {
            __builtin_amdgcn_sched_barrier(0);
            if (s2 == 0) load_frags(1, tile, 1);
            else if (late_frags) load_frags(0, smem + nxt * STAGE, 0);
            __builtin_amdgcn_sched_barrier(0);
          }
        }
      }
      cur = nxt;
    }
    if constexpr (LNF) {
      gemm_epilogue16_lnf<MT, NT>(p, acc, bm * BM + wr * (BM / WM), bn * BN + wc * (BN / WN), r16, q4);
      return;
    }
    if (p.epi_fast) {
      gemm_epilogue16_fast<MT, NT>(p, acc, bm * BM + wr * (BM / WM), bn * BN + wc * (BN / WN), r16, q4);
      return;
    }
    GemmP q = p;
    if (p.ksplit > 1) q.C = (float*)p.C + (long long)blockIdx.y * p.split_stride;
    gemm_epilogue16<MT, NT, 0, MT, true>(q, acc, bm * BM + wr * (BM / WM), bn * BN + wc * (BN / WN), r16, q4);
    return;
  }
  const int wr = wave / WN, wc = wave % WN;
  const int frow = lane & 31, fh = lane >> 5;
  const int a_row0 = wr * (BM / WM) + frow, w_row0 = wc * (BN / WN) + frow;
  f32x16 acc[NI][MI];
#pragma unroll
  for (int i = 0; i < NI; ++i)
#pragma unroll
    for (int j = 0; j < MI; ++j)
#pragma unroll
      for (int r = 0; r < 16; ++r) acc[i][j][r] = 0.f;
  bf16x8 af[2][MI], wf[2][NI];
  auto load_frags = [&](int which, const char* tile, int s) {
#pragma unroll
    for (int mi = 0; mi < MI; ++mi) af[which][mi] = *(const bf16x8*)(tile + swz_off(a_row0 + mi * 32, 2 * s + fh));
#pragma unroll
    for (int ni = 0; ni < NI; ++ni)
      wf[which][ni] = *(const bf16x8*)(tile + A_BYTES + swz_off(w_row0 + ni * 32, 2 * s + fh));
  };
  __builtin_amdgcn_s_barrier();
  load_frags(0, smem, 0);
  int cur = 0;
  for (int t = 0; t < nt; ++t) {
// ... 12 lines not shown
      }
      if constexpr (PROBE16) {
#pragma unroll
        for (int ni = 0; ni < NI; ++ni)
#pragma unroll
          for (int mi = 0; mi < MI; ++mi) {
            f32x4 q0 = {acc[ni][mi][0], acc[ni][mi][1], acc[ni][mi][2], acc[ni][mi][3]};
            f32x4 q1 = {acc[ni][mi][4], acc[ni][mi][5], acc[ni][mi][6], acc[ni][mi][7]};
            q0 = __builtin_amdgcn_mfma_f32_16x16x32_bf16(wf[s & 1][ni], af[s & 1][mi], q0, 0, 0, 0);
            q1 = __builtin_amdgcn_mfma_f32_16x16x32_bf16(wf[s & 1][ni], af[s & 1][mi], q1, 0, 0, 0);
#pragma unroll
            for (int j = 0; j < 4; ++j) { acc[ni][mi][j] = q0[j]; acc[ni][mi][4 + j] = q1[j]; }
          }
      } else {
#pragma unroll
      for (int ni = 0; ni < NI; ++ni)
#pragma unroll
        for (int mi = 0; mi < MI; ++mi)
          acc[ni][mi] = __builtin_amdgcn_mfma_f32_32x32x16_bf16(wf[s & 1][ni], af[s & 1][mi], acc[ni][mi], 0, 0, 0);
      }
    }
    cur = nxt;
  }
  if (p.ksplit > 1) {
    GemmP q = p;
    q.C = (float*)p.C + (long long)blockIdx.y * p.split_stride;
    gemm_epilogue<MI, NI>(q, acc, bm * BM + wr * (BM / WM), bn * BN + wc * (BN / WN), frow, fh);
    return;
  }
  gemm_epilogue<MI, NI>(p, acc, bm * BM + wr * (BM / WM), bn * BN + wc * (BN / WN), frow, fh);
}

template <int MODE, int BM, int BN, int WM, int WN, int LW, int S, bool PROBE16 = false, bool M16 = false, int MINW = 1,
          bool LNF = false, bool KSW = false>
static int launch_lc(const GemmP& p, hipStream_t stream) {
  constexpr int lds = S * (BM + BN) * 128;
  static_assert(lds <= 160 * 1024, "LDS budget");
  static_assert(!KSW || WM * WN * 2 * (BM / WM / 32) * (BN / WN / 16) * 1024 <= lds, "K-split exchange fits the ring");
  static bool attr_set = false;
  if (!attr_set) {
    HIPCHK(hipFuncSetAttribute((const void*)gemm_lc_kernel<MODE, BM, BN, WM, WN, LW, S, PROBE16, M16, MINW, LNF, KSW>,
                               hipFuncAttributeMaxDynamicSharedMemorySize, lds));
    attr_set = true;
  }
  SHAPECHK(!KSW || (p.epi_fast && p.ksplit <= 1), "gemm: the K-split form needs the batched-load epilogue");
  const int grid = cdiv(p.M, BM) * cdiv(p.N, BN);
  hipLaunchKernelGGL((gemm_lc_kernel<MODE, BM, BN, WM, WN, LW, S, PROBE16, M16, MINW, LNF, KSW>),
                     dim3(grid, p.ksplit > 1 ? p.ksplit : 1), dim3((WM * WN * (KSW ? 2 : 1) + LW) * 64), lds, stream, p.A, p.W, p.lda, p.ldw,
                     p.M, p.N, p.K, p.ksplit, p.debug, p);
  return PEA_OK;
}

template <int MODE, int BM, int BN, int WM, int WN, int LW, int S, int SW = 0, int DF = 0, int EPI = 0, int OCC = 1>
__global__ __launch_bounds__((WM * WN + LW + SW) * 64, (OCC == 2 ? 3 : 1)) void gemm_lcp_kernel(const GemmP p) {
  constexpr bool FASTONLY = EPI != 0;
  constexpr int PITCH = BN * 2 + 16;
  extern __shared__ __attribute__((aligned(16))) char smem[];
  constexpr int NWC = WM * WN;
  constexpr int STAGE = (BM + BN) * 128;
  constexpr int A_BYTES = BM * 128;
  constexpr int PA = BM / 8 / LW, PB = BN / 8 / LW;
  constexpr int PP = PA + PB;
  static_assert(BM % (8 * LW) == 0 && BN % (8 * LW) == 0, "tile / loader split");
  const int tid = threadIdx.x;
  const int lane = tid & 63;
  const int wave = __builtin_amdgcn_readfirstlane(tid >> 6);

  const int nbm = (p.M + BM - 1) / BM, nbn = (p.N + BN - 1) / BN;
  const int nwg = nbm * nbn;
  const int nblk = gridDim.x;
  const int xcd = blockIdx.x & 7, idx = blockIdx.x >> 3;
  const int nbx = (nblk - xcd + 7) >> 3;
  const int tq = nwg >> 3, tr = nwg & 7;
  const int cnt_x = tq + (xcd < tr ? 1 : 0);
  const int start_x = xcd < tr ? xcd * (tq + 1) : tr * (tq + 1) + (xcd - tr) * tq;
  const int my_n = idx < cnt_x ? (cnt_x - idx + nbx - 1) / nbx : 0;
  const int nt = p.K / BK;
  const int G = my_n * nt;
  if (G == 0) return;
  constexpr int GROUP = BM >= 256 ? 4 : 8;
// ... 350 lines not shown
  hipLaunchKernelGGL((gemm_lcp_kernel<MODE, BM, BN, WM, WN, LW, S, SW, DF, EPI, OCC>), dim3(grid),
                     dim3((WM * WN + LW + SW) * 64), lds, stream, p);
  return PEA_OK;
}

#define GEMM_TABLE(X)                                                                   \
  X(18, launch_lc,  1, 1,  0, 128, 128, 2, 2, 4, 4)                                     \
  X(19, launch_lc,  1, 1,  0, 128, 160, 4, 1, 4, 3)                                     \
  X(20, launch_lc,  1, 1,  0, 128, 160, 4, 1, 4, 3, true)        \
  X(22, launch_lc,  1, 1,  0, 128, 160, 2, 2, 4, 4, false, true)                        \
  X(23, launch_lc,  1, 1,  0, 128, 128, 2, 2, 4, 4, false, true)                        \
  X(24, launch_lc,  1, 1,  0, 256, 160, 4, 2, 4, 3, false, true)                        \
  X(25, launch_lc,  1, 1,  0, 128, 160, 4, 2, 4, 3, false, true)                        \
  X(27, launch_lcp, 1, 1, 28, 256, 160, 4, 2, 4, 3, 0, 0, 1)                            \
  X(28, launch_lcp, 1, 1,  0, 128, 160, 4, 2, 4, 3)                                     \
  X(29, launch_lcp, 1, 1,  0, 128, 160, 2, 2, 4, 4)                                     \
  X(30, launch_lcp, 1, 1,  0, 128, 128, 2, 2, 4, 4)                                     \
  X(31, launch_lcp, 1, 1,  0, 64, 160, 2, 2, 4, 4)                                      \
  X(33, launch_lcp, 1, 1, 30, 256, 128, 4, 2, 4, 3, 0, 0, 1)                            \
  X(34, launch_lcp, 0, 1,  0, 128, 160, 4, 2, 4, 3, 4)             \
  X(35, launch_lcp, 0, 1,  0, 128, 160, 4, 2, 4, 3, 0, 1)        \
  X(36, launch_lcp, 1, 1,  0, 128, 160, 2, 2, 2, 2, 0, 0, 1, 2)  \
  X(37, launch_lcp, 1, 1,  0, 128, 128, 2, 2, 2, 2, 0, 0, 1, 2)                         \
  X(39, launch_lc,  1, 0,  0, 192, 160, 4, 2, 4, 3, false, true)  \
  X(40, launch_lcp, 1, 0, 28, 192, 160, 4, 2, 4, 3, 0, 0, 1)                            \
  X(41, launch_lc,  1, 1,  0, 128, 160, 2, 2, 4, 3, false, true, 1, false, true)

enum GemmInst : int {
#define X(id, fn, cg, rf, gen, ...) GEMM_V##id = id,
  GEMM_TABLE(X)
#undef X
  GEMM_GBWD_256 = 127, GEMM_GBWD_128 = 128, GEMM_GBWD_64 = 131,
  GEMM_LNF_LC256 = 224, GEMM_LNF_LC128 = 225, GEMM_LNF_256 = 227, GEMM_LNF_128 = 228, GEMM_LNF_64 = 231,
};
static constexpr GemmInst kGemmInsts[] = {
#define X(id, fn, cg, rf, gen, ...) GEMM_V##id,
    GEMM_TABLE(X)
#undef X
    GEMM_GBWD_256, GEMM_GBWD_128, GEMM_GBWD_64, GEMM_LNF_LC256, GEMM_LNF_LC128, GEMM_LNF_256, GEMM_LNF_128, GEMM_LNF_64};
struct GemmVariantRow { int id; bool colscale_geglu, rowvec_fused; int generic_id; };
static constexpr GemmVariantRow kGemmRows[] = {
#define X(id, fn, cg, rf, gen, ...) {id, cg != 0, rf != 0, gen},
    GEMM_TABLE(X)
#undef X
};
static const GemmVariantRow* gemm_row(int id) {
  for (const GemmVariantRow& r : kGemmRows)
    if (r.id == id) return &r;
  return nullptr;
}

struct GemmEnv {
  bool defer;
  int ksw_mink;
  bool slow_epilogue;
  bool pf_on;
  long long pf_max;
};
static const GemmEnv& gemm_env() {
  static const GemmEnv e = {getenv("PEA_GEMM_DEFER") != nullptr, getenv("PEA_GEMM_KSW_MINK") ? atoi(getenv("PEA_GEMM_KSW_MINK")) : 0,
                            getenv("PEA_GEMM_SLOW_EPILOGUE") != nullptr, !(getenv("PEA_GEMM_PF") && atoi(getenv("PEA_GEMM_PF")) == 0),
                            (getenv("PEA_GEMM_PF_MAX_MB") ? atoll(getenv("PEA_GEMM_PF_MAX_MB")) : 64) << 20};
  return e;
}

static bool gemm_epi_fast(const GemmP& p, const GemmEnv& env) {
// ... 11 lines not shown
  const int t128 = cdiv(p.M, 128) * cdiv(p.N, 160), t256 = cdiv(p.M, 256) * cdiv(p.N, 160);
  if (p.mode == 1) {
    if (t256 >= cus) return 27;
    return 29;
  }
  if (p.M < 1024 && t128 > 2 * cus)
    return p.M * 100 >= cdiv(p.M, 256) * 256 * 78 ? 27 : 29;
  if (p.M < 1024 || t128 <= cus * 5 / 8) return 31;
  const bool lean = env.defer && !p.out_f32 && !p.res && !p.rowvec && !p.act && !p.geglu_y && !p.gbwd_pre && !p.preact && !p.qscale_cols && p.ksplit <= 1 &&
                    p.ldc % 8 == 0 && (((unsigned long long)p.C & 15) == 0);
  if (!p.rowvec && p.mode == 0 && epi_fast && p.M >= 1024) {
    const int t192 = cdiv(p.M, 192) * cdiv(p.N, 160);
    const int r128 = cdiv(t128, cus) * 128, r192 = cdiv(t192, cus) * 192, r256 = cdiv(t256, cus) * 256;
    const int cur = t128 <= cus ? r128 : (t256 <= cus ? (t256 > cus * 3 / 4 ? r256 : r128)
                                                       : (t256 * 100 >= cdiv(t256, cus) * cus * 85 ? r256 : r128));
    if (r192 * 10 <= cur * 9) return t192 <= cus ? 39 : 40;
  }
  if (t128 <= cus && env.ksw_mink > 0 && p.K >= env.ksw_mink && (p.K / BK) % 2 == 0 && epi_fast && p.ksplit <= 1 && p.mode == 0 && t128 > cus * 5 / 8) return 41;
  if (t128 <= cus) return lean ? 35 : 25;
  if (t256 <= cus) return t256 > cus * 3 / 4 ? 24 : (lean ? 35 : 28);
  const int rounds = cdiv(t256, cus);
  if (t256 * 100 >= rounds * cus * 85) return 27;
  return lean ? 35 : 28;
}

struct GemmDecision { GemmInst inst; bool epi_fast; };
static GemmDecision gemm_decide(const GemmP& p, int cus, int forced, const GemmEnv& env) {
  const bool epi_fast = gemm_epi_fast(p, env);
  int v = forced >= 0 ? forced : pick_variant(p, epi_fast, cus > 0 ? cus : 256, env);
  const GemmVariantRow* row = gemm_row(v);
  if (row && !row->colscale_geglu && (p.qscale_cols || p.geglu_y)) v = 28;
  if (row && !row->rowvec_fused && (p.gbwd_pre || p.ln_stats || (p.rowvec && epi_fast))) v = 28;
  if (p.ksplit > 1) v = 18;
  if (p.gbwd_pre) {
    return {v == 27 || v == 24 ? GEMM_GBWD_256 : (v == 31 ? GEMM_GBWD_64 : GEMM_GBWD_128), epi_fast};
  }
  row = gemm_row(v);
  if (!epi_fast && row && row->generic_id) v = row->generic_id;
  if (p.ln_stats) {
    switch (v) {
      case 27: return {GEMM_LNF_256, epi_fast};
      case 24: return {GEMM_LNF_LC256, epi_fast};
      case 28: case 35: return {GEMM_LNF_128, epi_fast};
      case 31: return {GEMM_LNF_64, epi_fast};
      default: return {GEMM_LNF_LC128, epi_fast};
    }
  }
  return {gemm_row(v) ? (GemmInst)v : GEMM_V23, epi_fast};
}

int g_gemm_variant = -1;
extern "C" void pea_debug_set_gemm_variant(int v) { g_gemm_variant = v; }
int g_gemm_debug = 0;
extern "C" void pea_debug_set_gemm_debug(int v) { g_gemm_debug = v; }
static const void* g_dbg_pf_ptr = nullptr;
static long long g_dbg_pf_bytes = 0;
extern "C" void pea_debug_set_gemm_prefetch(const void* p, long long bytes) { g_dbg_pf_ptr = p; g_dbg_pf_bytes = bytes; }

extern "C" int pea_debug_gemm_dispatch(int M, int N, int K, int mode, int rows_per_batch, int features, int cus, int forced) {
  if (M <= 0) return N >= 0 && N < (int)(sizeof(kGemmInsts) / sizeof(kGemmInsts[0])) ? (int)kGemmInsts[N] : -1;
  GemmP p = {};
  const bool al = (features & 1024) != 0;
  char* const base = (char*)(uintptr_t)(al ? 0x1000 : 0x1004);
  const int pad = al ? 0 : 4;
  p.mode = mode; p.M = M; p.N = N; p.K = K; p.alpha = 1.f;
  p.lda = K; p.ldw = K;
  p.rows_per_batch = rows_per_batch > 0 ? rows_per_batch : M;
  p.C = base; p.ldc = ((features & 64) ? 2 * N : N) + pad;
  if (features & 1) { p.res = (const bf16*)base; p.ldres = N + pad; }
  if (features & 2) { p.rowvec = (const bf16*)base; p.ldrv = N; }
  if (features & 4) p.out_f32 = 1;
  if (features & 8) p.act = 1;
  if (features & 32) { p.geglu_y = (bf16*)base; p.ldy = N / 2 + pad; if (!(features & 16)) p.C = nullptr; }
  else if (features & 16) { p.preact = (bf16*)base; p.ldpre = N + pad; }
  if (features & 64) { p.gbwd_pre = (const bf16*)base; p.ldgp = 2 * N + pad; }
  if (features & 128) { p.ln_stats = (const float*)base; p.ln_s = (const float*)base; }
  if (features & 256) { p.qscale_cols = 16; p.qscale = 1.f; }
  if (features & 512) p.ksplit = 2;
  return gemm_decide(p, cus, forced, gemm_env()).inst;
}

int launch_gemm(const GemmP& p_in, hipStream_t stream) {
  const GemmP& p0 = p_in;
  SHAPECHK(p0.M > 0 && p0.N > 0 && p0.K > 0, "gemm: empty problem M=%d N=%d K=%d", p0.M, p0.N, p0.K);
  SHAPECHK(p0.K % BK == 0, "gemm: K=%d must be a multiple of %d", p0.K, BK);
  SHAPECHK(p0.N % 4 == 0, "gemm: N=%d must be a multiple of 4", p0.N);
  SHAPECHK(p0.ldw % 8 == 0 && p0.ldc % 4 == 0, "gemm: ldw=%d ldc=%d alignment", p0.ldw, p0.ldc);
  if (p0.mode == 0) {
    SHAPECHK(p0.lda % 8 == 0, "gemm: lda=%d must be a multiple of 8", p0.lda);
  } else {
    const int ntaps = p0.kside == 2 ? 4 : (p0.kside == 4 ? 16 : 9);
    SHAPECHK(p0.kside == 0 || p0.kside == 2 || p0.kside == 3 || p0.kside == 4, "conv: kside=%d", p0.kside);
    SHAPECHK(p0.Cin % BK == 0 && p0.K == ntaps * p0.Cin, "conv: Cin=%d must be a multiple of %d and K=%d*Cin", p0.Cin, BK, ntaps);
    SHAPECHK(p0.pix == 0 || (p0.pix % 8 == 0 && p0.pix >= (p0.kside == 4 ? 4 : 1) * p0.Cin), "conv: pixel stride %d vs Cin=%d", p0.pix, p0.Cin);
    SHAPECHK(p0.kside < 4 || (!p0.shift && !p0.parity && p0.stride == 1), "conv: the 16-tap form is stride 1 on a plain source");
    SHAPECHK(p0.zeros != nullptr, "conv: zero page missing");
    SHAPECHK(p0.M % (p0.Ho * p0.Wo) == 0, "conv: M=%d not a multiple of Ho*Wo", p0.M);
  }
  {
    const long long hw = p0.mode ? (long long)p0.Ho * p0.Wo : 1;
    const long long pix = p0.pix ? p0.pix : p0.Cin;
    const long long span = p0.mode ? (256 / hw + 2) * (long long)p0.Hs * p0.Ws * pix * 2 : 256LL * p0.lda * 2;
    const long long whole = p0.mode ? (p0.M / hw) * (long long)p0.Hs * p0.Ws * pix * 2 : (long long)p0.M * p0.lda * 2;
    SHAPECHK((span < whole ? span : whole) <= 0x7f000000LL, "gemm: one row tile of A spans %lld bytes (limit 0x7f000000)", span);
    SHAPECHK((long long)p0.N * p0.ldw * 2 <= 0x7fffffffLL, "gemm: W of %d x %d exceeds the 2 GB buffer range", p0.N, p0.ldw);
  }
  {
    double fl = 2.0 * p0.M * (double)p0.N * p0.K * (p0.parity ? 0.25 : 1.0);
    double by = 2.0 * ((double)p0.M * p0.N + (double)p0.N * p0.K + (p0.mode ? (double)p0.M * p0.K / (p0.kside == 2 ? 4.0 : (p0.kside == 4 ? 4.0 : 9.0)) : (double)p0.M * p0.K));
    if (g_prof_on) { g_prof_tag[0] = p0.M; g_prof_tag[1] = p0.N; g_prof_tag[2] = p0.K; g_prof_tag[3] = (p0.res ? 1 : 0) | (p0.bias ? 2 : 0) | (p0.rowvec ? 4 : 0); }
    PROF_BEGIN(p0.mode ? 1 : 0, fl, by, stream);
  }
  const GemmEnv& env = gemm_env();
  GemmP p = p_in;
  p.debug = g_gemm_debug;
  if (g_dbg_pf_ptr) { p.pf_ptr = g_dbg_pf_ptr; p.pf_bytes = g_dbg_pf_bytes; g_dbg_pf_ptr = nullptr; }
  if (!env.pf_on || p.pf_bytes <= 0) { p.pf_ptr = nullptr; p.pf_bytes = 0; }
  if (p.pf_bytes > env.pf_max) p.pf_bytes = env.pf_max;
  SHAPECHK(p.qscale_cols % 16 == 0 && p.qscale_cols >= 0 && p.qscale_cols <= p.N && (!p.qscale_cols || (!p.act && !p.geglu_y && !p.gbwd_pre && p.ksplit <= 1)),
           "gemm: qscale_cols=%d must be a multiple of 16 within N, on a plain (no activation / GEGLU / split-K) epilogue", p.qscale_cols);
  if (p.ksplit > 1) {
    SHAPECHK(p.out_f32 && !p.accum_f32 && !p.bias && !p.res && !p.rowvec && !p.preact && p.act == 0 && p.mode == 0,
             "gemm: split-K writes plain fp32 partials");
    SHAPECHK(p.split_stride >= (long long)(p.M - 1) * p.ldc + p.N && p.split_stride % 4 == 0,
             "gemm: split-K split_stride=%lld (M=%d N=%d ldc=%d): partials overlap or leave 16-byte alignment", p.split_stride, p.M, p.N, p.ldc);
  }
  SHAPECHK(!(p.stash_grad && p.geglu_tanh), "gemm: the gradient-form GEGLU stash exists for the erf gate only (geglu_tanh set)");
  if (!g_num_cus) HIPCHK(gemm_query_cus());
  const GemmDecision d = gemm_decide(p, g_num_cus, g_gemm_variant, env);
  p.epi_fast = d.epi_fast;
  if (p.gbwd_pre) {
    SHAPECHK(p.epi_fast && p.mode == 0 && !p.res && !p.rowvec && !p.bias && !p.geglu_y && !p.ln_stats && p.ldgp % 8 == 0 &&
                 p.ldc >= 2 * p.N && (((unsigned long long)p.gbwd_pre & 15) == 0),
             "gemm: the fused GEGLU backward needs the batched-load epilogue (bf16 [M][2N] output, no bias / residual / row vector)");
  } else if (p.ln_stats) {
    SHAPECHK(p.epi_fast && p.ln_s && p.alpha == 1.f && p.mode == 0 && !p.res && !p.rowvec,
             "gemm: the folded-LayerNorm epilogue needs the batched-load epilogue (bf16 output, no activation / residual)");
  }
  int rc = PEA_OK;
  switch (d.inst) {
#define X(id, fn, cg, rf, gen, ...) \
    case GEMM_V##id: rc = p.mode == 0 ? fn<0, __VA_ARGS__>(p, stream) : fn<1, __VA_ARGS__>(p, stream); break;
    GEMM_TABLE(X)
#undef X
    case GEMM_GBWD_256: rc = launch_lcp<0, 256, 160, 4, 2, 4, 3, 0, 0, 3>(p, stream); break;
    case GEMM_GBWD_128: rc = launch_lcp<0, 128, 160, 4, 2, 4, 3, 0, 0, 3>(p, stream); break;
    case GEMM_GBWD_64: rc = launch_lcp<0, 64, 160, 2, 2, 4, 4, 0, 0, 3>(p, stream); break;
    case GEMM_LNF_256: rc = launch_lcp<0, 256, 160, 4, 2, 4, 3, 0, 0, 2>(p, stream); break;
    case GEMM_LNF_LC256: rc = launch_lc<0, 256, 160, 4, 2, 4, 3, false, true, 1, true>(p, stream); break;
    case GEMM_LNF_128: rc = launch_lcp<0, 128, 160, 4, 2, 4, 3, 0, 0, 2>(p, stream); break;
    case GEMM_LNF_64: rc = launch_lcp<0, 64, 160, 2, 2, 4, 4, 0, 0, 2>(p, stream); break;
    case GEMM_LNF_LC128: rc = launch_lc<0, 128, 160, 4, 2, 4, 3, false, true, 1, true>(p, stream); break;
  }
  PROF_END(stream);
  if (rc != PEA_OK) return rc;
  HIPCHK(hipGetLastError());
  return PEA_OK;
}

__global__ __launch_bounds__(256) void conv_in_kernel(const float* __restrict__ x, const float* __restrict__ w,
                                                      const float* __restrict__ bias, bf16* __restrict__ y, int B,
                                                      int Cin, int H, int W, int Cout, int pix_per_block, int ldy,
                                                      int silu) {
  extern __shared__ __attribute__((aligned(16))) char cism[];
  float* wl = (float*)cism;
  const int K = Cin * 9;
  for (int i = threadIdx.x; i < K * Cout; i += blockDim.x) {
    const int co = i / K, k = i - co * K;
    wl[k * Cout + co] = w[i];
  }
  __syncthreads();
  const int nchunk = Cout / 8;
  const int ppb = blockDim.x / nchunk;
  const int ck = threadIdx.x % nchunk, pl = threadIdx.x / nchunk;
  if (pl >= ppb) return;
  const int c0 = ck * 8;
  float bs[8];
#pragma unroll
  for (int j = 0; j < 8; ++j) bs[j] = bias[c0 + j];
  const long long npix = (long long)B * H * W;
  const long long p0 = (long long)blockIdx.x * pix_per_block;
  const long long p1 = p0 + pix_per_block < npix ? p0 + pix_per_block : npix;
  for (long long pix = p0 + pl; pix < p1; pix += ppb) {
    const int xw = (int)(pix % W), yh = (int)((pix / W) % H), b = (int)(pix / ((long long)W * H));
    float acc[8];
// ... 400 lines not shown
```

pea_diffusion_amd/csrc/model.h:

```cpp
#pragma once
#include <string.h>

#include <deque>
#include <map>
#include <string>
#include <vector>

#include "pea_kernels.h"

#define RC(x)                \
  do {                       \
    int rc__ = (x);          \
    if (rc__ != PEA_OK) return rc__; \
  } while (0)

#define NOTNULL(p, what)                         \
  do {                                           \
    if (!(p)) {                                  \
      pea_set_error("%s: null handle", what);    \
      return PEA_E_INVALID;                      \
    }                                            \
  } while (0)

inline size_t al256(size_t x) { return (x + 255) & ~(size_t)255; }
// ... 90 lines not shown
  int B = 0, H = 0, W = 0;
  bf16* d = nullptr; bf16* g = nullptr;
  bool rg = false;
  bool zero_init = false;
  bool gw = false;
  const bf16* gpend = nullptr;
  size_t off_d = 0, off_g = 0;
  bool external = false;
  bool d2s = false;
};

enum OpKind { OP_CONV_IN, OP_CONV3, OP_LINEAR, OP_GN, OP_LN, OP_ATTN, OP_GEGLU, OP_CONCAT, OP_SILU, OP_TEMB,
              OP_CONV_OUT, OP_ADD, OP_ATTN_MAT, OP_EMBED, OP_GATHER_EOS, OP_VIS_EMBED, OP_CLS_ROW, OP_ATTN_FEWQ };
inline bool is_flash_attn(int kind) { return kind == OP_ATTN || kind == OP_ATTN_FEWQ; }

struct Op {
  int kind;
  int a = -1, b = -1, c = -1;
  int acol = 0, bcol = 0, ccol = 0;
  int out = -1;
  int res = -1;
  int rv = -1, rv_off = 0;
  int w = -1, bias = -1;
  int fused = -1;
  int p0 = 0, p1 = 0, p2 = 0, p3 = 0;
  float f0 = 0.f;
  float* aux = nullptr; size_t aux_off = 0, aux_bytes = 0;
  int src = 0;
  int mask = 0;
  int fold = -1;
  int qs_cols = 0; float qs = 1.f;
  int k2col = 0, v2col = 0;
  int pre = 0;
  int stash_form = -1;
};

struct Tape {
  PeaUnetCfg cfg;
  int B, H, W, L;
  bool needs_grad;
  int bwd_batch = 0;
  int graph = 0;
  std::vector<int> cn_out;
  int ce_begin = -1, ce_end = -1;
  bool ce_valid = false;
  const float* cond_in = nullptr;
  int cond_scale_f = 8;
  int w_quant = -1, b_quant = -1;
  bf16* am_scores = nullptr;
  bf16* am_vt = nullptr;
  float* vae_h = nullptr;
  bool residual_inputs = false;
  std::vector<int> ext_res;
  bool inpaint_inputs = false;
  float* inp_buf = nullptr;
  bool inp_set = false;
  int inp_cond_b = 0, inp_lat_b = 0;
  int set_inpaint_cond(const float* mask, const float* masked, int cond_b, int lat_b, hipStream_t s);
  int time_cond_dim = 0;
  int t_tcond = -1;
  int set_timestep_cond(const float* cond, hipStream_t s);
  bool fu_on = false;
  float fu_s[2] = {1.f, 1.f}, fu_b[2] = {1.f, 1.f};
  float* fu_buf = nullptr;
  size_t fu_coef_bytes = 0;
  int set_freeu(float s1, float s2, float b1, float b2, hipStream_t s);
// ... 65 lines not shown
      if (scratch) (void)hipFree(scratch);
    }
  };
  StyleState* style = nullptr;
  bool is_self_attn(const Op& o) const { return graph == 0 && o.kind == OP_ATTN && o.b != t_kvall && !o.mask && o.p1 == o.p2; }
  struct SagState {
    int layer = 0, op = -1, first = 0, n = 0, G = 0, S = 0, H = 0;
    float* lse = nullptr;
    float* part = nullptr;
    ~SagState() {
      if (lse) (void)hipFree(lse);
      if (part) (void)hipFree(part);
    }
  };
  SagState* sag = nullptr;
  struct PerturbState {
    enum { IDENTITY = 1, BLUR = 2 };
    int mode = 0, first = 0;
    std::map<int, int> layer_of_op;
    std::vector<char> on;
    struct Grid { int h = 0, w = 0; float* Mh = nullptr; float* Mw = nullptr; };
    std::map<int, Grid> grid;
    ~PerturbState() {
      for (auto& g : grid) {
        if (g.second.Mh) (void)hipFree(g.second.Mh);
        if (g.second.Mw) (void)hipFree(g.second.Mw);
      }
    }
  };
  PerturbState* perturb = nullptr;
  enum { AF_IP = 1, AF_REGIONS = 2, AF_MAPS = 4, AF_EDIT = 8, AF_STYLE = 16, AF_SAG = 32, AF_PERTURB = 64 };
  int attn_rules(unsigned which, bool forward, int arg = 0) const;
  int attn_forward(size_t oi, hipStream_t s);
  std::deque<WSlot> slots;
  std::map<std::string, int> slot_by_name;
  std::deque<FusedMat> fused;
  std::vector<Tn> tn;
  std::vector<Op> ops;
  std::vector<LnFold> folds;
  bool fold_dirty = true;
  Tape* weights_owner = nullptr;
  bool tap_layout_queried = false;
  int ensure_folded(hipStream_t s);
  std::vector<int> taps;
  std::vector<std::string> tap_names;
  int t_ehs = -1, t_text = -1, t_tproj = -1, t_out_in = -1, t_kvall = -1;
  int tproj_total = 0, kvall_total = 0, kv_nsplit = 1;
  float* kv_part = nullptr;
  bf16* geglu_tmp = nullptr;
  char* warena = nullptr; size_t wbytes = 0; bool owns_weights = true;
  bool plan_only = false;
  char* aarena = nullptr; size_t abytes = 0;
  char* garena = nullptr; size_t gbytes = 0;
  double* gn_scratch = nullptr; float* cs_scratch = nullptr; float* attn_part = nullptr; float* delta = nullptr; bf16* ups_tmp = nullptr; float* tproj_grad = nullptr;
  float* tmp_f32 = nullptr; size_t tmp_f32_elems = 0;
  const bf16* zeros = nullptr;
  const float* x_in = nullptr; const float* t_in = nullptr; const float* tid_in = nullptr;
  float* eps_out = nullptr; const float* deps_in = nullptr;

  int build();
  int check_attn_bwd_tokens() const;
  int build_vae_encoder();
  int build_vae_decoder();
  int release_acts();
  int build_text();
  int build_text_t5();
// ... 104 lines not shown
```

pea_diffusion_amd/csrc/pea_kernels.h:

```cpp
#pragma once
#include "pea_common.h"

struct GemmP {
  int mode;
  const bf16* A; int lda;
  const bf16* W; int ldw;
  void* C; int ldc; int out_f32;
  int accum_f32;
  int M, N, K;
  float alpha;
  const float* bias;
  const bf16* rowvec; int ldrv; int rows_per_batch;
  int act;
  bf16* preact; int ldpre;
  const bf16* res; int ldres;
  int Hs, Ws, Cin, Ho, Wo;
  int stride;
  int pad_off;
  int shift;
  int parity;
  int kside;
  int pad_dx;
  int pix;
  const bf16* zeros;
  int debug;
  bf16* geglu_y; int ldy;
  int geglu_tanh;
  int stash_rows;
  int stash_grad;
  int ksplit; long long split_stride;
  int epi_fast;
  const float* ln_stats; const float* ln_s;
  const bf16* gbwd_pre; int ldgp;
  int qscale_cols; float qscale;
  int gbwd_form;
  const void* pf_ptr; long long pf_bytes;
};
int launch_splitk_reduce(const float* part, int nsplit, long long stride, bf16* out, int ldo, int M, int N, int accum,
                         hipStream_t s);
int launch_gemm(const GemmP& p, hipStream_t stream);

int launch_conv_in(const float* x, const float* w, const float* bias, bf16* y, int B, int Cin, int H, int W,
                   int Cout, hipStream_t s, int ldy = 0, int silu = 0);
int launch_conv_in_gather(const float* lat, const float* mask, const float* masked, const float* w, const float* bias, bf16* y,
                          int B, int C, int lat_b, int cond_b, int H, int W, int Cout, hipStream_t s, int ldy = 0);
int launch_conv_out(const bf16* x, const float* w, const float* bias, float* y, int B, int Cin, int H, int W,
                    int Cout, hipStream_t s);
int launch_conv_out_dgrad(const float* dy, const float* w, bf16* dx, int B, int Cin, int H, int W, int Cout,
                          hipStream_t s);

int launch_groupnorm_fwd(const bf16* x, const float* gamma, const float* beta, bf16* y, float* stats,
                         double* scratch, int B, int HW, int C, int groups, float eps, int silu, hipStream_t s);
int launch_groupnorm_bwd(const bf16* x, const bf16* dy, const float* gamma, const float* beta, const float* stats,
                         bf16* dx, double* scratch, int B, int HW, int C, int groups, int silu, const bf16* add,
                         hipStream_t s);
int launch_layernorm_fwd(const bf16* x, const float* gamma, const float* beta, bf16* y, float* stats, int R, int C,
                         float eps, hipStream_t s);
int launch_rmsnorm_fwd(const bf16* x, const float* gamma, bf16* y, int R, int C, float eps, hipStream_t s);
int launch_layernorm_fwd_f32(const float* x, const float* gamma, const float* beta, float* y, int R, int C, float eps,
                             hipStream_t s);
int launch_layernorm_stats(const bf16* x, float* stats, int R, int C, float eps, hipStream_t s);
int launch_ln_fold(const bf16* W, int ldw, const float* gamma, const float* beta, const float* bias, bf16* Wf, float* svec,
                   float* tvec, int N, int K, hipStream_t s);
int launch_layernorm_bwd(const bf16* x, const bf16* dy, const float* gamma, const float* stats, bf16* dx,
                         float* dgamma, float* dbeta, int R, int C, const bf16* add, hipStream_t s);

struct AttnP {
  const bf16 *Q, *K, *V; int ldq, ldk, ldv;
  bf16* O; int ldo;
  float* lse;
  int B, H, Sq, Skv;
  float scale;
  const bf16* dO; int lddo;
  bf16 *dQ, *dK, *dV; int lddq, lddk, lddv;
  float* delta;
  int accum_dq, accum_dkv;
  float* dkv_part; int nsplit;
  int nd;
  int causal;
  const int* kv_len;
  int q_prescaled;
  const float* bias;
  const bf16 *K2, *V2; int ldk2, ldv2, Skv2;
  float scale2;
  int nset; int set_end[4]; float set_w[4]; int k2_brows;
  const float* set_mask[4]; long long set_mstride[4];
};
int attention_bwd_nsplit(int B, int H, int Sq, int Skv);
size_t attention_bwd_scratch_bytes(int B, int H, int Sq, int Skv, int nd = 1);
int launch_attention_fwd(const AttnP& p, hipStream_t s);
int launch_attention_fwd_fewq(const AttnP& p, hipStream_t s);
int launch_attention_bwd(const AttnP& p, hipStream_t s);
struct AttnRegionsP {
  const bf16 *Q, *K, *V; int ldq, ldk, ldv;
  bf16* O; int ldo;
  int B, H, Sq, R, Lr;
  const float* w; int Bw;
  float scale; int q_prescaled;
  int nd;
};
int launch_attention_fwd_regions(const AttnRegionsP& p, hipStream_t s);
struct AttnEditP {
  const bf16 *Q, *K, *V; int ldq, ldk, ldv;
  bf16* O; int ldo;
  int B, H, Sq, Skv;
  const bf16* Mt; int ldm;
  const float *c, *d;
  float scale; int q_prescaled;
  int nd;
  int src[32];
};
int launch_attention_fwd_edit(const AttnEditP& p, hipStream_t s);
struct AttnSharedP {
  const bf16 *Q, *K, *V; int ldq, ldk, ldv;
  bf16* O; int ldo;
  int B, H, Sq, Skv;
  const float* coef;
  float scale; int q_prescaled;
  float share_scale, share_shift;
  int nd;
// ... 189 lines not shown
```

pea_diffusion_amd/csrc/tape.hip:

```cpp
#include <stdlib.h>

#include <algorithm>

#include "model.h"

int Tape::alloc() {
  tag_q_prescale();
  for (const Op& o : ops) {
    const int in[5] = {o.a, o.kind == OP_LINEAR || o.kind == OP_EMBED ? -1 : o.b, o.kind == OP_LINEAR || o.kind == OP_EMBED ? -1 : o.c, o.res, o.rv};
    for (int k = 0; k < 5; ++k) {
      if (in[k] < 0 || in[k] >= (int)tn.size() || !tn[in[k]].d2s) continue;
      SHAPECHK(o.kind == OP_CONCAT && k == 0 && o.a != o.b, "tape: op kind %d reads a depth-to-space tensor", o.kind);
    }
  }
  size_t off = 0;
  size_t max_numel = 0;
  if (owns_weights) {
    for (FusedMat& f : fused) {
      f.off_w = off; off += al256((size_t)f.N * f.K * 2);
      if (f.need_wt) { f.off_wt = off; off += al256((size_t)f.N * f.K * 2); }
      if (f.has_bias) { f.off_bias = off; off += al256((size_t)f.N * 4); }
    }
    for (WSlot& s : slots) {
      max_numel = std::max(max_numel, (size_t)s.numel);
// ... 674 lines not shown

int Tape::backward(const float* deps, hipStream_t s) {
  SHAPECHK(needs_grad, "unet: created without gradient support");
  RC(ensure_acts());
  const int Bb = bwd_batch > 0 ? bwd_batch : B;
  auto rb = [&](const Tn& t) -> long long { return t.rows / B * Bb; };
  HIPCHK(hipMemsetAsync(tproj_grad, 0, sizeof(float) * Bb * tproj_total, s));
  struct WSeqScope {
    Tape* t; bool ok = false;
    ~WSeqScope() { if (ok) t->wseq_end(); else t->wseq_cur = nullptr; }
  } wscope{this};
  if (graph == 0) wseq_begin(wseq_bwd);
  auto addend = [](Tn& t) -> const bf16* {
    if (t.gw) return t.g;
    const bf16* p = t.gpend;
    t.gpend = nullptr;
    return p;
  };
  auto materialize = [&](Tn& t) -> int {
    if (!t.gw && t.gpend) {
      RC(launch_accum(t.gpend, t.g, rb(t) * t.cols, 0, s));
      t.gpend = nullptr;
      t.gw = true;
    }
    return PEA_OK;
  };
  auto pass_on = [&](Tn& from, Tn& r) -> int {
    if (!r.gw && !r.gpend) { r.gpend = from.g; return PEA_OK; }
    RC(materialize(r));
    RC(launch_accum(from.g, r.g, rb(r) * r.cols, 1, s));
    return PEA_OK;
  };
  int dpre_of = -1;
  for (int oi = (int)ops.size() - 1; oi >= 0; --oi) {
    Op& o = ops[oi];
    if (o.kind == OP_CONV_OUT) {
      if (!deps) continue;
      Tn& a = tn[o.a];
      SHAPECHK(!a.gw, "unet: conv_out input gradient already written");
      RC(launch_conv_out_dgrad(deps, slots[o.w].f32, a.g, Bb, a.cols, H, W, cfg.out_channels, s));
      a.gw = true;
      continue;
    }
    if (o.out < 0) continue;
    Tn& out = tn[o.out];
    if (!out.rg) continue;
    if (o.kind == OP_LINEAR && o.p3 == 1) {
      RC(launch_cast_f32_bf16(tproj_grad, out.g, (long long)Bb * tproj_total, s));
      out.gw = true;
    }
    RC(materialize(out));
    if (!out.gw) continue;
    switch (o.kind) {
      case OP_LINEAR: {
        Tn& a = tn[o.a];
        if (a.rg && o.p3 == 2) {
          FusedMat& f = fused[o.fused];
          GemmP p; fill_gemm(p);
          p.A = out.g; p.lda = out.cols; p.M = (int)rb(out); p.K = out.cols; p.N = a.cols;
          p.W = f.wt; p.ldw = f.N; p.C = kv_part; p.ldc = a.cols; p.out_f32 = 1;
          p.ksplit = kv_nsplit; p.split_stride = rb(out) * a.cols;
          RC(gemm(p, s));
          RC(materialize(a));
          RC(launch_splitk_reduce(kv_part, kv_nsplit, p.split_stride, a.g, a.cols, (int)rb(a), a.cols, a.gw, s));
          a.gw = true;
          break;
// ... 2 lines not shown
          Tn& hg = tn[o.c];
          SHAPECHK(o.stash_form == 1, "unet: GEGLU op %d has no stash from a forward pass", oi);
          if (dpre_of != o.out) RC(launch_geglu_bwd_il(hg.d, out.g, geglu_tmp, rb(out), out.cols, s));
          dpre_of = -1;
          WSlot& w = slots[o.w];
          GemmP p; fill_gemm(p);
          p.A = geglu_tmp; p.lda = hg.cols; p.M = (int)rb(out); p.K = hg.cols; p.N = a.cols;
          p.W = w.wt; p.ldw = w.ldwt; p.C = a.g; p.ldc = a.cols;
          SHAPECHK(p.W != nullptr, "unet: dgrad weights missing for op %d", oi);
          if (const bf16* ad = addend(a)) { p.res = ad; p.ldres = a.cols; }
          RC(gemm(p, s));
          a.gw = true;
          break;
        }
        if (a.rg) {
          GemmP p; fill_gemm(p);
          p.A = out.g; p.lda = out.cols; p.M = (int)rb(out); p.K = out.cols; p.N = a.cols;
          if (o.fused >= 0) { FusedMat& f = fused[o.fused]; p.W = f.wt; p.ldw = f.N; }
          else { WSlot& w = slots[o.w]; p.W = w.wt; p.ldw = w.ldwt; }
          SHAPECHK(p.W != nullptr, "unet: dgrad weights missing for op %d", oi);
          const Op* prev = oi > 0 ? &ops[oi - 1] : nullptr;
          if (g_geglu_bwd_fused && prev && prev->kind == OP_LINEAR && prev->p3 == 3 && prev->out == o.a && prev->c >= 0 &&
              tn[prev->a].rg && !a.gw && !a.gpend && geglu_tmp && a.cols % 16 == 0) {
            Tn& hg = tn[prev->c];
            SHAPECHK(prev->stash_form >= 0, "unet: GEGLU op %d has no stash from a forward pass", oi - 1);
            p.gbwd_pre = hg.d; p.ldgp = hg.cols; p.gbwd_form = prev->stash_form;
            p.C = geglu_tmp; p.ldc = hg.cols;
            RC(gemm(p, s));
            a.gw = true;
            dpre_of = o.a;
          } else {
            p.C = a.g; p.ldc = a.cols;
            if (const bf16* ad = addend(a)) { p.res = ad; p.ldres = a.cols; }
            RC(gemm(p, s));
            a.gw = true;
          }
        }
        if (o.res >= 0 && tn[o.res].rg) RC(pass_on(out, tn[o.res]));
        break;
      }
      case OP_SILU: {
        Tn& a = tn[o.a];
        if (a.rg) { RC(materialize(a)); RC(launch_silu_bwd(a.d, out.g, a.g, rb(a) * a.cols, a.gw, s)); a.gw = true; }
        break;
      }
      case OP_CONCAT: {
        Tn &a = tn[o.a], &b = tn[o.b];
        if (o.a == o.b) {
          if (a.rg) {
            RC(materialize(a));
            RC(launch_split2(out.g, a.cols, b.cols, a.g, a.gw, nullptr, false, rb(a), s));
            RC(launch_split2(out.g, a.cols, b.cols, nullptr, false, a.g, true, rb(a), s));
            a.gw = true;
          }
          break;
        }
        if (a.rg) RC(materialize(a));
        if (b.rg) RC(materialize(b));
        RC(launch_split2(out.g, a.cols, b.cols, a.rg ? a.g : nullptr, a.gw, b.rg ? b.g : nullptr, b.gw, rb(a), s,
                         a.d2s ? a.H : 0, a.d2s ? a.W : 0));
        if (a.rg) a.gw = true;
        if (b.rg) b.gw = true;
        break;
      }
      case OP_CONV3: {
        Tn& a = tn[o.a];
// ... 21 lines not shown
          }
          a.gw = true;
        }
        if (o.rv >= 0 && tn[o.rv].rg)
          RC(launch_colsum_batched(out.g, tproj_grad + o.rv_off, Bb, out.H * out.W, out.cols, tproj_total, cs_scratch, s));
        if (o.res >= 0 && tn[o.res].rg) RC(pass_on(out, tn[o.res]));
        break;
      }
      case OP_GN: {
        Tn& a = tn[o.a];
        if (a.rg) {
          RC(launch_groupnorm_bwd(a.d, out.g, slots[o.w].f32, slots[o.bias].f32, o.aux, a.g, gn_scratch, Bb,
                                  a.H * a.W, a.cols, cfg.groups, o.p0, addend(a), s));
          a.gw = true;
        }
        break;
      }
      case OP_LN: {
        Tn& a = tn[o.a];
        if (a.rg) {
          RC(launch_layernorm_bwd(a.d, out.g, slots[o.w].f32, o.aux, a.g, nullptr, nullptr, (int)rb(a), a.cols,
                                  addend(a), s));
          a.gw = true;
        }
        break;
      }
      case OP_ATTN: {
        Tn &q = tn[o.a], &k = tn[o.b], &v = tn[o.c];
        AttnP p; memset(&p, 0, sizeof(p));
        p.Q = q.d + o.acol; p.ldq = q.cols; p.K = k.d + o.bcol; p.ldk = k.cols; p.V = v.d + o.ccol; p.ldv = v.cols;
        p.O = out.d; p.ldo = out.cols; p.lse = o.aux; p.B = Bb; p.H = o.p0; p.Sq = o.p1; p.Skv = o.p2; p.scale = o.f0;
        p.nd = o.p3; p.q_prescaled = o.pre;
        p.dO = out.g; p.lddo = out.cols; p.delta = delta; p.dkv_part = attn_part;
        if (cross_kvlen && o.b == t_kvall) p.kv_len = cross_kvlen;
        SHAPECHK(!q.gw && !q.gpend && !k.gpend && (!k.gw || o.b == t_kvall), "unet: attention operand gradient written twice");
        if (q.rg) { p.dQ = q.g + o.acol; p.lddq = q.cols; }
        if (k.rg) { p.dK = k.g + o.bcol; p.lddk = k.cols; p.dV = v.g + o.ccol; p.lddv = v.cols; }
        RC(launch_attention_bwd(p, s));
        if (q.rg) q.gw = true;
        if (k.rg) { k.gw = true; v.gw = true; }
        break;
      }
      case OP_GEGLU: {
        Tn& a = tn[o.a];
        if (a.rg) {
          SHAPECHK(!a.gw, "unet: geglu input gradient written twice");
          RC(launch_geglu_bwd(a.d, out.g, a.g, rb(a), out.cols, s));
          a.gw = true;
        }
        break;
      }
      default:
        break;
    }
  }
  for (Tn& t : tn)
    if (t.rg) RC(materialize(t));
  wscope.ok = true;
  return PEA_OK;
}
```

pea_diffusion_amd/ops.py:

```python
from __future__ import annotations

import ctypes
from typing import List, Optional, Sequence

import torch

from ._lib import PeaError, check, lib, ptr, stream_ptr

BF = torch.bfloat16


def _dev(t):
    return t.device


def gemm(a, w, bias=None, rowvec=None, rows_per_batch=1, act=0, res=None, want_preact=False, out_f32=False,
         alpha=1.0, out=None, accum_f32=False):
    M, K = a.shape
    N = w.shape[0]
    if out is None:
        out = torch.empty(M, N, device=a.device, dtype=torch.float32 if out_f32 else BF)
    pre = torch.empty(M, N, device=a.device, dtype=BF) if want_preact else None
    check(lib().pea_op_gemm(ptr(a), a.stride(0), ptr(w), w.stride(0), ptr(out), out.stride(0), M, N, K, alpha,
                            ptr(bias), ptr(rowvec), rowvec.stride(0) if rowvec is not None else 0, rows_per_batch,
# ... 3 lines not shown


def gemm_geglu(a, w, bias=None, want_stash=True, stash_grad=True, stash_rows=0, tanh=False, y=None, stash=None):
    M, K = a.shape
    N = w.shape[0]
    if y is None:
        y = torch.empty(M, N // 2, device=a.device, dtype=BF)
    st = stash if stash is not None else (torch.zeros(M, N, device=a.device, dtype=BF) if want_stash else None)
    if tanh:
        check(lib().pea_op_gemm_geglu_tanh(ptr(a), a.stride(0), ptr(w), w.stride(0), ptr(bias), ptr(y), ptr(st), M, N, K,
                                           int(stash_grad), stash_rows, 1, stream_ptr()))
        return y, st
    check(lib().pea_op_gemm_geglu(ptr(a), a.stride(0), ptr(w), w.stride(0), ptr(bias), ptr(y), ptr(st), M, N, K,
                                  int(stash_grad), stash_rows, stream_ptr()))
    return y, st


def gemm_splitk(a, w, ksplit, part, ldc, split_stride, alpha=1.0):
    M, K = a.shape
    N = w.shape[0]
    assert part.dtype == torch.float32 and part.numel() >= (ksplit - 1) * split_stride + (M - 1) * ldc + N
    check(lib().pea_op_gemm_splitk(ptr(a), a.stride(0), ptr(w), w.stride(0), ptr(part), ldc, split_stride, M, N, K, alpha,
                                   ksplit, stream_ptr()))
    return part


def gemm_geglu_bwd(a, w, pre, form=0):
    M, K = a.shape
    N = w.shape[0]
    out = torch.empty(M, 2 * N, device=a.device, dtype=BF)
    check(lib().pea_op_gemm_geglu_bwd(ptr(a), a.stride(0), ptr(w), w.stride(0), ptr(pre), pre.stride(0), ptr(out), out.stride(0),
                                      M, N, K, form, stream_ptr()))
    return out


def ln_linear(x, gamma, beta, w, bias=None, eps=1e-5, geglu=False):
    M, K = x.shape
    N = w.shape[0]
    y = torch.empty(M, N, device=x.device, dtype=BF)
    gy = torch.empty(M, N // 2, device=x.device, dtype=BF) if geglu else None
    wf = torch.empty(N, K, device=x.device, dtype=BF)
    sv = torch.empty(N, device=x.device, dtype=torch.float32)
    tv = torch.empty(N, device=x.device, dtype=torch.float32)
    st = torch.empty(M, 2, device=x.device, dtype=torch.float32)
    check(lib().pea_op_ln_linear(ptr(x), ptr(gamma), ptr(beta), ptr(w), ptr(bias), ptr(y), ptr(gy), M, N, K, eps, ptr(wf),
                                 ptr(sv), ptr(tv), ptr(st), stream_ptr()))
    return (gy, y) if geglu else y


def pack_conv(w_fp32, dgrad=False, cin_stored=None):
    Co, Ci = w_fp32.shape[:2]
    if cin_stored is not None:
        assert not dgrad, "the padded pack is a forward pack"
        out = torch.empty(Co, 9 * cin_stored, device=w_fp32.device, dtype=BF)
        check(lib().pea_op_pack_conv_padded(ptr(w_fp32.contiguous()), ptr(out), Co, Ci, cin_stored, stream_ptr()))
        return out
    out = torch.empty((Ci, 9 * Co) if dgrad else (Co, 9 * Ci), device=w_fp32.device, dtype=BF)
    check(lib().pea_op_pack_conv(ptr(w_fp32.contiguous()), ptr(out), Co, Ci, int(dgrad), stream_ptr()))
    return out


def conv3x3(x, w_packed, bias=None, stride=1, upsample2x=False, transposed2=False, rowvec=None, res=None):
    B, H, W, Cin = x.shape
    Cout = w_packed.shape[0]
    sh = 1 if (upsample2x or transposed2) else 0
    Hv, Wv = H << sh, W << sh
# ... 372 lines not shown
def attention_bias_pitch(Skv):
    return (Skv + 63) // 64 * 64


def attention_fwd_text(q, k, v, heads, scale=None, q_prescaled=False, causal=False, kv_len=None, bias=None, want_lse=True):
    B, Sq, C = q.shape
    Skv = k.shape[1]
    if bias is not None and (bias.dtype != torch.float32 or tuple(bias.shape) != (heads, Sq, attention_bias_pitch(Skv))
                             or not bias.is_contiguous()):
        raise PeaError(f"attention_fwd_text: bias must be contiguous fp32 [{heads}, {Sq}, {attention_bias_pitch(Skv)}]")
    B, Sq, C, scale, o, lse = _attn_fwd_out(q, heads, scale, want_lse)
    check(lib().pea_op_attention_fwd_text(ptr(q), q.stride(1), ptr(k), k.stride(1), ptr(v), v.stride(1), ptr(o), C, ptr(lse),
                                          B, heads, Sq, Skv, scale, int(q_prescaled), int(causal), ptr(kv_len), ptr(bias),
                                          stream_ptr()))
    return (o, lse) if want_lse else o


def attention_bwd(q, k, v, o, do, lse, heads, scale=None, q_prescaled=False):
    B, Sq, C = q.shape
    Skv = k.shape[1]
    nd = C // heads // 64
    scale = scale if scale is not None else (C // heads) ** -0.5
    dq, dk, dv = torch.empty_like(q), torch.empty_like(k), torch.empty_like(v)
    delta = torch.empty(2, B, heads, Sq, device=q.device, dtype=torch.float32)
    nb = lib().pea_op_attention_bwd_scratch_bytes(B, heads, Sq, Skv, nd)
    scratch = torch.empty(nb, device=q.device, dtype=torch.uint8) if nb else None
    fn = lib().pea_op_attention_bwd_prescaled if q_prescaled else lib().pea_op_attention_bwd
    check(fn(ptr(q), q.stride(1), ptr(k), k.stride(1), ptr(v), v.stride(1), ptr(o), C, ptr(do),
                                     C, ptr(lse), ptr(delta), ptr(dq), C, ptr(dk), C, ptr(dv), C, B, heads, Sq, Skv,
                                     scale, 0, 0, nd, ptr(scratch), stream_ptr()))
    return dq, dk, dv


def attention_bwd_masked(q, k, v, o, do, lse, heads, scale=None, q_prescaled=False, kv_len=None, use_scratch=True):
    B, Sq, C = q.shape
    Skv = k.shape[1]
    nd = C // heads // 64
    scale = scale if scale is not None else (C // heads) ** -0.5
    dq, dk, dv = torch.empty_like(q), torch.empty_like(k), torch.empty_like(v)
    delta = torch.empty(2, B, heads, Sq, device=q.device, dtype=torch.float32)
    nb = lib().pea_op_attention_bwd_scratch_bytes(B, heads, Sq, Skv, nd) if use_scratch else 0
    scratch = torch.empty(nb, device=q.device, dtype=torch.uint8) if nb else None
    check(lib().pea_op_attention_bwd_masked(ptr(q), q.stride(1), ptr(k), k.stride(1), ptr(v), v.stride(1), ptr(o), C, ptr(do),
                                            C, ptr(lse), ptr(delta), ptr(dq), C, ptr(dk), C, ptr(dv), C, B, heads, Sq, Skv,
                                            scale, 0, 0, nd, ptr(scratch), int(q_prescaled), ptr(kv_len), stream_ptr()))
    return dq, dk, dv


def geglu_fwd(hg):
    rows, two = hg.shape
    y = torch.empty(rows, two // 2, device=hg.device, dtype=BF)
    check(lib().pea_op_geglu_fwd(ptr(hg), ptr(y), rows, two // 2, stream_ptr()))
    return y


def geglu_bwd(hg, dy):
    d = torch.empty_like(hg)
    check(lib().pea_op_geglu_bwd(ptr(hg), ptr(dy), ptr(d), hg.shape[0], hg.shape[1] // 2, stream_ptr()))
    return d


def sumpool2(x):
    B, H2, W2, C = x.shape
    y = torch.empty(B, H2 // 2, W2 // 2, C, device=x.device, dtype=BF)
    check(lib().pea_op_sumpool2(ptr(x), ptr(y), B, H2 // 2, W2 // 2, C, 0, stream_ptr()))
    return y
# ... 495 lines not shown
```

Baseline: 41.90.

## Fuse attention-backward row constants into output-projection dgrad GEMM epilogue

Measured after the change: 42.09, median of 6. Within noise of the previous version (+0.4%).

```diff
diff --git a/include/pea_hip.h b/include/pea_hip.h
--- a/include/pea_hip.h
+++ b/include/pea_hip.h
@@ -30,6 +30,9 @@
 
 int pea_op_gemm_geglu_bwd(const void* A, int lda, const void* W, int ldw, const void* pre, int ldpre, void* C, int ldc,
                           int M, int N, int K, int form, void* stream);
+
+int pea_op_gemm_delta(const void* A, int lda, const void* W, int ldw, void* C, int ldc, const void* O, int ldo, float* delta,
+                      long long delta_stride, int M, int N, int K, int heads, int rows_per_sample, int features, void* stream);
 
 int pea_op_ln_linear(const void* x, const float* gamma, const float* beta, const void* W, const float* bias, void* y,
                      void* geglu_y, int M, int N, int K, float eps, void* Wf, float* svec, float* tvec, float* stats,
@@ -113,6 +116,13 @@
                          int ldo, const void* dO, int lddo, const float* lse, float* delta, void* dQ, int lddq,
                          void* dK, int lddk, void* dV, int lddv, int B, int H, int Sq, int Skv, float scale,
                          int accum_dq, int accum_dkv, int nd, void* scratch, void* stream);
+
+int pea_op_attention_fwd_lse2(const void* Q, int ldq, const void* K, int ldk, const void* V, int ldv, void* O, int ldo, float* lse2,
+                              int B, int H, int Sq, int Skv, float scale, void* stream);
+int pea_op_attention_bwd_rowconst(const void* Q, int ldq, const void* K, int ldk, const void* V, int ldv, const void* O,
+                                  int ldo, const void* dO, int lddo, const float* lse2, float* delta, void* dQ, int lddq,
+                                  void* dK, int lddk, void* dV, int lddv, int B, int H, int Sq, int Skv, float scale,
+                                  void* stream);
 
 int pea_op_attention_bwd_prescaled(const void* Q, int ldq, const void* K, int ldk, const void* V, int ldv, const void* O,
                                    int ldo, const void* dO, int lddo, const float* lse, float* delta, void* dQ, int lddq,
@@ -251,6 +261,7 @@
                           long long* scratch_bytes);
 int pea_tape_attention_census(void* graph, int* n_attn, int* n_prescaled);
 int pea_unet_plan_attention(const pea_unet_config* cfg, int B, int H, int W, int L, int flags, int* n_attn, int* n_prescaled);
+int pea_unet_plan_rowconst(const pea_unet_config* cfg, int B, int H, int W, int L, int flags, int* n_self64, int* n_linear);
 int pea_graph_plan_attention(int graph, const pea_unet_config* cfg, int B, int H, int W, int L, int* n_attn,
                              int* n_prescaled);
 int pea_unet_num_residuals(void* unet);
@@ -407,6 +418,8 @@
 void pea_debug_set_attn_xattn(int v);
 void pea_debug_set_xattn_bwd_v2(int v);
 void pea_debug_set_geglu_bwd_fused(int v);
+void pea_debug_set_attn_delta_fused(int v);
+int pea_debug_gemm_delta_dispatch(int M, int N, int K, int cus);
 void pea_debug_set_gemm_variant(int v);
 int pea_debug_gemm_dispatch(int M, int N, int K, int mode, int rows_per_batch, int features, int cus, int forced);
 int pea_debug_attn_dispatch(const int* q, int* out);
diff --git a/pea_diffusion_amd/csrc/api_model.hip b/pea_diffusion_amd/csrc/api_model.hip
--- a/pea_diffusion_amd/csrc/api_model.hip
+++ b/pea_diffusion_amd/csrc/api_model.hip
@@ -159,6 +159,27 @@
   if (rc != PEA_OK) return rc;
   if (n_attn) *n_attn = u.n_attn;
   if (n_prescaled) *n_prescaled = u.n_attn_pre;
+  return PEA_OK;
+}
+int pea_unet_plan_rowconst(const pea_unet_config* cfg, int B, int H, int W, int L, int flags, int* n_self64, int* n_linear) {
+  NOTNULL(cfg, "pea_unet_plan_rowconst");
+  Tape u;
+  memcpy(&u.cfg, cfg, sizeof(PeaUnetCfg));
+  u.B = B; u.H = H; u.W = W; u.L = L; set_flags(u, flags);
+  u.plan_only = true;
+  int rc = u.build();
+  if (rc == PEA_OK) rc = u.alloc();
+  if (rc != PEA_OK) return rc;
+  int ns = 0, nl = 0;
+  std::vector<char> taken(u.ops.size(), 0);
+  for (size_t i = 0; i < u.ops.size(); ++i) {
+    const Op& o = u.ops[i];
+    if (u.needs_grad && u.is_self_attn(o) && o.p3 == 1 && u.tn[o.out].cols == 64 * o.p0 && u.tn[o.a].rg) ++ns;
+    const int l = u.rowconst_linear(i);
+    if (l >= 0 && !taken[l]) { taken[l] = 1; ++nl; }
+  }
+  if (n_self64) *n_self64 = ns;
+  if (n_linear) *n_linear = nl;
   return PEA_OK;
 }
 static int plan_census(Tape& u, int* n_attn, int* n_prescaled) {
diff --git a/pea_diffusion_amd/csrc/api_ops.hip b/pea_diffusion_amd/csrc/api_ops.hip
--- a/pea_diffusion_amd/csrc/api_ops.hip
+++ b/pea_diffusion_amd/csrc/api_ops.hip
@@ -90,6 +90,20 @@
   p.A = (const bf16*)A; p.lda = lda; p.W = (const bf16*)W; p.ldw = ldw; p.C = C; p.ldc = ldc;
   p.M = M; p.N = N; p.K = K; p.alpha = 1.f; p.rows_per_batch = 1;
   p.gbwd_pre = (const bf16*)pre; p.ldgp = ldpre; p.gbwd_form = form;
+  return launch_gemm(p, (hipStream_t)stream);
+}
+
+int pea_op_gemm_delta(const void* A, int lda, const void* W, int ldw, void* C, int ldc, const void* O, int ldo, float* delta,
+                      long long delta_stride, int M, int N, int K, int heads, int rows_per_sample, int features, void* stream) {
+  GemmP p;
+  memset(&p, 0, sizeof(p));
+  p.A = (const bf16*)A; p.lda = lda; p.W = (const bf16*)W; p.ldw = ldw; p.C = C; p.ldc = ldc;
+  p.M = M; p.N = N; p.K = K; p.alpha = 1.f; p.rows_per_batch = 1;
+  p.delta_o = (const bf16*)O; p.lddo = ldo; p.delta_out = delta; p.delta_heads = heads; p.delta_rows = rows_per_sample;
+  p.delta_stride = delta_stride;
+  if (features & 1) p.out_f32 = 1;
+  if (features & 2) p.act = 1;
+  if (features & 4) { p.res = (const bf16*)C; p.ldres = ldc; }
   return launch_gemm(p, (hipStream_t)stream);
 }
 
@@ -395,6 +409,22 @@
   return attention_bwd_impl(Q, ldq, K, ldk, V, ldv, O, ldo, dO, lddo, lse, delta, dQ, lddq, dK, lddk, dV, lddv, B, H, Sq, Skv,
                             scale, accum_dq, accum_dkv, nd, scratch, 0, nullptr, stream);
 }
+int pea_op_attention_fwd_lse2(const void* Q, int ldq, const void* K, int ldk, const void* V, int ldv, void* O, int ldo, float* lse2,
+                              int B, int H, int Sq, int Skv, float scale, void* stream) {
+  AttnP p = attn_operands(Q, ldq, K, ldk, V, ldv, O, ldo, lse2, B, H, Sq, Skv, scale, 1);
+  p.lse_neg_log2 = 1;
+  return launch_attention_fwd(p, (hipStream_t)stream);
+}
+int pea_op_attention_bwd_rowconst(const void* Q, int ldq, const void* K, int ldk, const void* V, int ldv, const void* O,
+                                  int ldo, const void* dO, int lddo, const float* lse2, float* delta, void* dQ, int lddq,
+                                  void* dK, int lddk, void* dV, int lddv, int B, int H, int Sq, int Skv, float scale,
+                                  void* stream) {
+  AttnP p = attn_operands(Q, ldq, K, ldk, V, ldv, O, ldo, lse2, B, H, Sq, Skv, scale, 1);
+  p.dO = (const bf16*)dO; p.lddo = lddo; p.delta = delta;
+  p.dQ = (bf16*)dQ; p.lddq = lddq; p.dK = (bf16*)dK; p.lddk = lddk; p.dV = (bf16*)dV; p.lddv = lddv;
+  p.rowconst_ready = 1;
+  return launch_attention_bwd(p, (hipStream_t)stream);
+}
 int pea_op_attention_bwd_prescaled(const void* Q, int ldq, const void* K, int ldk, const void* V, int ldv, const void* O,
                                    int ldo, const void* dO, int lddo, const float* lse, float* delta, void* dQ, int lddq,
                                    void* dK, int lddk, void* dV, int lddv, int B, int H, int Sq, int Skv, float scale,
diff --git a/pea_diffusion_amd/csrc/attention.hip b/pea_diffusion_amd/csrc/attention.hip
--- a/pea_diffusion_amd/csrc/attention.hip
+++ b/pea_diffusion_amd/csrc/attention.hip
@@ -283,18 +283,19 @@
 }
 template <int NO>
 __device__ __forceinline__ void attn_fwd_exit(const f32x16 (&oacc)[2 * NO], float m_run, float l_run, float* lse, long long lse_i,
-                                              bool lse_lane, char* ost, int lane, bf16* Ob, int ldo, int q0, int Sq) {
+                                              bool lse_lane, char* ost, int lane, bf16* Ob, int ldo, int q0, int Sq,
+                                              bool neg_log2 = false) {
   float la = l_run, lb = l_run;
   swap_halves32(la, lb);
   const float l_tot = la + lb;
   const float inv = 1.f / l_tot;
-  if (lse && lse_lane) lse[lse_i] = (m_run + log2f(l_tot)) * 0.6931471805599453f;
+  if (lse && lse_lane) lse[lse_i] = neg_log2 ? -(m_run + log2f(l_tot)) : (m_run + log2f(l_tot)) * 0.6931471805599453f;
 #pragma unroll
   for (int no = 0; no < NO; ++no)
     store_o_image_144(ost, lane, [&](int db, int i) { return oacc[2 * no + db][i] * inv; }, Ob + no * 64, ldo, q0, Sq);
 }
 
-template <int MODE, bool USE_TR, int ND, bool TXT, bool WRITE_DELTA>
+template <int MODE, bool USE_TR, int ND, bool TXT, int WRITE_DELTA>
 __device__ __forceinline__ void attn_q_body(const AttnP& p, char* smem, int blk_x, int head, int b) {
   constexpr int STG = 2 * ND * TILE_BYTES;
   constexpr int NO = MODE == 0 ? ND : 1;
@@ -332,7 +333,10 @@
       for (int s = 0; s < 4; ++s)
         dof[nd][s] = *(const bf16x8*)(dOb + (long long)qrow * p.lddo + nd * 64 + 16 * s + 8 * fh);
     const long long li = ((long long)b * p.H + head) * p.Sq + qrow;
-    if (!WRITE_DELTA) {
+    if (WRITE_DELTA == 2) {
+      dlt = -(p.delta[li] + p.delta[(long long)p.B * p.H * p.Sq + li]);
+      lse2 = -p.lse[li];
+    } else if (!WRITE_DELTA) {
       dlt = -p.delta[li];
       lse2 = -p.delta[(long long)p.B * p.H * p.Sq + li];
     } else {
@@ -349,7 +353,7 @@
         }
       { float da = dsum, db = dsum; swap_halves32(da, db); dsum = da + db; }
       dlt = dsum;
-      if (WRITE_DELTA && qvalid && fh == 0 && chunk == 0) {
+      if (WRITE_DELTA == 1 && qvalid && fh == 0 && chunk == 0) {
         p.delta[li] = -dsum;
         p.delta[(long long)p.B * p.H * p.Sq + li] = -lse2;
       }
@@ -457,7 +461,7 @@
   char* const ost = smem + wave * (32 * 144);
   if constexpr (MODE == 0)
     attn_fwd_exit<NO>(oacc, m_run, l_run, p.lse, ((long long)b * p.H + head) * p.Sq + qrow, qvalid && fh == 0, ost, lane,
-                      p.O + (long long)b * p.Sq * p.ldo + head * 64 * ND, p.ldo, q0, p.Sq);
+                      p.O + (long long)b * p.Sq * p.ldo + head * 64 * ND, p.ldo, q0, p.Sq, !TXT && p.lse_neg_log2 != 0);
   else
     store_o_image_144(ost, lane, [&](int db, int i) { return oacc[db][i] * p.scale; }, p.dQ + (long long)b * p.Sq * p.lddq + head * 64 * ND + chunk * 64,
                       p.lddq, q0, p.Sq, p.accum_dq != 0);
@@ -468,7 +472,7 @@
   extern __shared__ __attribute__((aligned(16))) char smem[];
   int blk_x, head, b;
   attn_block_coords(blk_x, head, b);
-  attn_q_body<MODE, USE_TR, ND, TXT, true>(p, smem, blk_x, head, b);
+  attn_q_body<MODE, USE_TR, ND, TXT, 1>(p, smem, blk_x, head, b);
 }
 
 struct AttnKeyLane { int k0, krow; bool kstored, wave_active; };
@@ -486,7 +490,7 @@
   lds_dma4(src + r, dst);
 }
 
-template <bool USE_TR, int ND>
+template <bool USE_TR, int ND, bool RC = false>
 __device__ __forceinline__ void attn_dkv_body(const AttnP& p, char* smem, int blk_x, int head, int b) {
   constexpr int STG = 2 * ND * TILE_BYTES + 512;
   const int tid = threadIdx.x, lane = tid & 63;
@@ -504,7 +508,7 @@
   const bf16* Kb = p.K + (long long)b * p.Skv * p.ldk + head * 64 * ND;
   const bf16* Vb = p.V + (long long)b * p.Skv * p.ldv + head * 64 * ND;
   const float* dltb = p.delta + ((long long)b * p.H + head) * p.Sq;
-  const float* lseb = dltb + (long long)p.B * p.H * p.Sq;
+  const float* lseb = RC ? p.lse + ((long long)b * p.H + head) * p.Sq : dltb + (long long)p.B * p.H * p.Sq;
 
   const int skv_b = p.kv_len ? p.kv_len[b] : p.Skv;
   const bool kvalid = k0 + frow < skv_b;
@@ -538,20 +542,31 @@
     }
     if (wave == 0) {
       stage_rowconst(lseb, r0, p.Sq, dst + 2 * ND * TILE_BYTES, lane);
-      stage_rowconst(dltb, r0, p.Sq, dst + 2 * ND * TILE_BYTES + 256, lane);
-    }
+      if constexpr (!RC) stage_rowconst(dltb, r0, p.Sq, dst + 2 * ND * TILE_BYTES + 256, lane);
+    }
+  };
+  [[maybe_unused]] float piece0 = 0.f, piece1 = 0.f;
+  auto fetch_pieces = [&](int r0) {
+    if (RC && wave == 0) {
+      const int r = min(r0 + lane, p.Sq - 1);
+      piece0 = dltb[r];
+      piece1 = dltb[(long long)p.B * p.H * p.Sq + r];
+    }
+  };
+  auto put_pieces = [&](char* dst) {
+    if (RC && wave == 0) ((float*)(dst + 2 * ND * TILE_BYTES + 256))[lane] = piece0 + piece1;
   };
   const int nt_all = (p.Sq + 63) / 64;
   const int tps = (nt_all + nsplit - 1) / nsplit;
   const int t_begin = split * tps;
   const int nt = min(nt_all, t_begin + tps);
-  if (t_begin < nt) stage_q(smem, t_begin * 64);
+  if (t_begin < nt) { stage_q(smem, t_begin * 64); fetch_pieces(t_begin * 64); put_pieces(smem); }
   WAIT_VM0();
   __syncthreads();
 
   for (int t = t_begin; t < nt; ++t) {
     const int cur = (t - t_begin) & 1;
-    if (t + 1 < nt) stage_q(smem + (cur ^ 1) * STG, (t + 1) * 64);
+    if (t + 1 < nt) { stage_q(smem + (cur ^ 1) * STG, (t + 1) * 64); fetch_pieces((t + 1) * 64); }
     const char* Qs = smem + cur * STG;
     const char* dOs = Qs + ND * TILE_BYTES;
     const float* rc = (const float*)(Qs + 2 * ND * TILE_BYTES);
@@ -644,6 +659,7 @@
         __builtin_amdgcn_sched_barrier(0);
       }
     }
+    if (t + 1 < nt) put_pieces(smem + (cur ^ 1) * STG);
     WAIT_VM0();
     __syncthreads();
   }
@@ -707,15 +723,15 @@
   attn_dkv_body<USE_TR, ND>(p, smem, blk_x, head, b);
 }
 
-template <bool USE_TR, int ND>
+template <bool USE_TR, int ND, bool RC = false>
 __global__ __launch_bounds__(256, (ND == 1 ? 2 : 1)) void attn_bwd_fused_kernel(const AttnP p, int n_dq, int n_dkv) {
   extern __shared__ __attribute__((aligned(16))) char smem[];
   const unsigned lin = xcd_contiguous(blockIdx.x, gridDim.x);
   const int per_head = n_dq + n_dkv;
   const int bh = (int)(lin / per_head), rem = (int)(lin - (unsigned)bh * per_head);
   const int b = bh / p.H, head = bh - b * p.H;
-  if (rem < n_dkv) attn_dkv_body<USE_TR, ND>(p, smem, rem, head, b);
-  else attn_q_body<1, USE_TR, ND, false, false>(p, smem, rem - n_dkv, head, b);
+  if (rem < n_dkv) attn_dkv_body<USE_TR, ND, RC>(p, smem, rem, head, b);
+  else attn_q_body<1, USE_TR, ND, false, RC ? 2 : 0>(p, smem, rem - n_dkv, head, b);
 }
 
 struct XattnCtx {
@@ -2447,6 +2463,10 @@
   void add(int kernel, dim3 grid, int lds, int a0 = 0, int a1 = 0) { l[n++] = AttnLaunch{kernel, grid, lds, a0, a1}; }
 };
 struct AttnEnv { int xattn_ver, use_tr, xattn, fused_bwd; };
+static bool attn_rowconst_plan(const AttnP& p, const AttnEnv& e) {
+  const bool resident = e.xattn && e.use_tr && p.nd <= 1 && p.Skv <= 128;
+  return p.nd <= 1 && e.use_tr && e.fused_bwd && p.dQ && p.dK && p.dV && !resident;
+}
 static AttnEnv g_attn_env = {getenv("PEA_XATTN_BWD_VER") ? atoi(getenv("PEA_XATTN_BWD_VER")) : 3, 1, getenv("PEA_XATTN_OFF") ? 0 : 1,
                              getenv("PEA_ATTN_BWD_SPLIT") ? 0 : 1};
 extern "C" void pea_debug_set_xattn_bwd_v2(int v) { g_attn_env.xattn_ver = v; }
@@ -2478,6 +2498,9 @@
   return best_ns;
 }
 int attention_bwd_nsplit(int B, int H, int Sq, int Skv) { return attn_nsplit(B, H, Sq, Skv, g_attn_env); }
+static int g_attn_delta_fused = getenv("PEA_ATTN_DELTA_SEPARATE") ? 0 : 1;
+extern "C" void pea_debug_set_attn_delta_fused(int v) { g_attn_delta_fused = v; }
+bool attention_bwd_takes_rowconst(const AttnP& p) { return g_attn_delta_fused && attn_rowconst_plan(p, g_attn_env); }
 size_t attention_bwd_scratch_bytes(int B, int H, int Sq, int Skv, int nd) {
   const int ns = attention_bwd_nsplit(B, H, Sq, Skv);
   return ns > 1 ? (size_t)ns * B * H * Skv * 128 * nd * sizeof(float) : 0;
@@ -2486,6 +2509,7 @@
 static int attn_decide_fwd(const AttnP& p, const AttnEnv& e, AttnPlan& plan) {
   const int nu = cdiv(p.Sq, 128);
   if (p.K2 || (attn_resident_kv(p, e) && !p.causal && !p.bias && p.Sq >= 128)) {
+    SHAPECHK(!p.lse_neg_log2, "attention: -lse * log2(e) is written by the unmasked general kernel only");
     const int kb = cdiv(p.Skv, 32), kt = (kb + 1) / 2;
     const int lds = 2 * kt * TILE_BYTES + 4 * 32 * 144 + 4 * 4096 + (p.K2 ? 2 * 4096 : 0);
     const int upw = units_per_wg((long long)p.B * p.H * nu, nu, 2);
@@ -2493,6 +2517,7 @@
     return PEA_OK;
   }
   const bool txt = p.causal || p.kv_len || p.bias;
+  SHAPECHK(!p.lse_neg_log2 || !txt, "attention: -lse * log2(e) is written by the unmasked general kernel only");
   SHAPECHK(!txt || p.nd == 1, "attention: causal / key-length masks need head_dim 64");
   plan.add(txt ? AK_Q_TXT : AK_Q + 3 * (e.use_tr != 0) + (p.nd - 1), dim3(nu, p.H, p.B), 2 * 2 * p.nd * TILE_BYTES);
   return PEA_OK;
@@ -2501,6 +2526,7 @@
   const int ns = plan.nsplit = p.dkv_part ? attn_nsplit(p.B, p.H, p.Sq, p.Skv, e) : 1;
   const int nd = p.nd, tr = e.use_tr != 0;
   bool all = p.dQ && p.dK && p.dV, partials = true;
+  SHAPECHK(!p.rowconst_ready || attn_rowconst_plan(p, e), "attention bwd: ready-made row constants are read by the fused head_dim-64 launch only");
   if (attn_resident_kv(p, e) && all) {
     const int kb = cdiv(p.Skv, 32);
     const dim3 grid(ns, p.H, p.B);
@@ -2516,7 +2542,7 @@
     const int lq = 2 * 2 * nd * TILE_BYTES, lk = 2 * (2 * nd * TILE_BYTES + 512);
     const int n_dq = cdiv(p.Sq, 128) * nd, n_dkv = cdiv(p.Skv, 128) * ns * nd;
     const bool fused = all && e.fused_bwd;
-    if (fused || !p.dQ) plan.add(AK_DELTA, dim3((unsigned)cdivl((long long)p.B * p.Sq * p.H * 8, 256 * ATTN_DELTA_ROWS)), 0);
+    if (!p.rowconst_ready && (fused || !p.dQ)) plan.add(AK_DELTA, dim3((unsigned)cdivl((long long)p.B * p.Sq * p.H * 8, 256 * ATTN_DELTA_ROWS)), 0);
     partials = fused || (p.dK && p.dV);
     if (fused) plan.add(AK_FUSED + 3 * tr + (nd - 1), dim3((unsigned)((n_dq + n_dkv) * p.H * p.B)), lk, n_dq, n_dkv);
     if (!fused && p.dQ) plan.add(AK_Q + 6 + 3 * tr + (nd - 1), dim3(n_dq, p.H, p.B), lq);
@@ -2629,7 +2655,10 @@
     ATTN_CASE(AK_DKV + 0, (attn_dkv_kernel<false, 1>)) ATTN_CASE(AK_DKV + 1, (attn_dkv_kernel<false, 2>)) ATTN_CASE(AK_DKV + 2, (attn_dkv_kernel<false, 3>))
     ATTN_CASE(AK_DKV + 3, (attn_dkv_kernel<true, 1>)) ATTN_CASE(AK_DKV + 4, (attn_dkv_kernel<true, 2>)) ATTN_CASE(AK_DKV + 5, (attn_dkv_kernel<true, 3>))
     ATTN_CASE(AK_FUSED + 0, (attn_bwd_fused_kernel<false, 1>), l.a0, l.a1) ATTN_CASE(AK_FUSED + 1, (attn_bwd_fused_kernel<false, 2>), l.a0, l.a1)
-    ATTN_CASE(AK_FUSED + 2, (attn_bwd_fused_kernel<false, 3>), l.a0, l.a1) ATTN_CASE(AK_FUSED + 3, (attn_bwd_fused_kernel<true, 1>), l.a0, l.a1)
+    ATTN_CASE(AK_FUSED + 2, (attn_bwd_fused_kernel<false, 3>), l.a0, l.a1)
+    case AK_FUSED + 3:
+      return p.rowconst_ready ? launch_lds<attn_bwd_fused_kernel<true, 1, true>>(l.grid, l.lds, s, p, l.a0, l.a1)
+                              : launch_lds<attn_bwd_fused_kernel<true, 1>>(l.grid, l.lds, s, p, l.a0, l.a1);
     ATTN_CASE(AK_FUSED + 4, (attn_bwd_fused_kernel<true, 2>), l.a0, l.a1) ATTN_CASE(AK_FUSED + 5, (attn_bwd_fused_kernel<true, 3>), l.a0, l.a1)
     ATTN_CASE(AK_XBWD1 + 0, xattn_bwd_kernel<1>, l.a0) ATTN_CASE(AK_XBWD1 + 1, xattn_bwd_kernel<2>, l.a0)
     ATTN_CASE(AK_XBWD1 + 2, xattn_bwd_kernel<3>, l.a0) ATTN_CASE(AK_XBWD1 + 3, xattn_bwd_kernel<4>, l.a0)
@@ -2692,6 +2721,7 @@
   }
   p.dQ = feat & 64 ? any : nullptr; p.dK = feat & 128 ? any : nullptr; p.dV = feat & 256 ? any : nullptr;
   p.dkv_part = feat & 512 ? page : nullptr; p.accum_dq = p.accum_dkv = feat >> 10 & 1;
+  p.rowconst_ready = feat >> 11 & 1;
   AttnPlan plan;
   const int rc = attn_plan(dir, p, e, plan);
   if (rc) return rc;
diff --git a/pea_diffusion_amd/csrc/attn_features.hip b/pea_diffusion_amd/csrc/attn_features.hip
--- a/pea_diffusion_amd/csrc/attn_features.hip
+++ b/pea_diffusion_amd/csrc/attn_features.hip
@@ -230,8 +230,24 @@
   return m;
 }
 
+int Tape::rowconst_linear(size_t oi) {
+  Op& o = ops[oi];
+  if (o.rc_lin != -2) return o.rc_lin;
+  o.rc_lin = -1;
+  if (!needs_grad || !is_self_attn(o) || o.p3 != 1 || o.out < 0 || oi + 1 >= ops.size()) return -1;
+  const Tn& out = tn[o.out];
+  if (!tn[o.a].rg || !tn[o.b].rg || !tn[o.c].rg || !out.rg || out.cols != 64 * o.p0 || out.cols % 320 != 0) return -1;
+  const Op& lin = ops[oi + 1];
+  if (lin.kind != OP_LINEAR || lin.p3 != 0 || lin.a != o.out || lin.qs_cols || lin.fold >= 0) return -1;
+  int readers = 0;
+  for (const Op& r : ops) readers += (r.a == o.out) + (r.b == o.out && r.b != r.a) + (r.c == o.out) + (r.res == o.out) + (r.rv == o.out);
+  if (readers != 1) return -1;
+  return o.rc_lin = (int)oi + 1;
+}
+
 int Tape::attn_forward(size_t oi, hipStream_t s) {
   const Op& o = ops[oi];
+  ops[oi].rc_form = 0;
   const bool text = o.b == t_kvall;
   AttnP p; memset(&p, 0, sizeof(p));
   p.Q = tn[o.a].d + o.acol; p.ldq = tn[o.a].cols; p.K = tn[o.b].d + o.bcol; p.ldk = tn[o.b].cols;
@@ -258,6 +274,11 @@
   if (perturbed == PerturbState::IDENTITY) p.B = perturb->first;
   const bool sag_here = sag && sag->op == (int)oi;
   if (sag_here) p.lse = sag->lse;
+  if (!perturbed && !sag_here && rowconst_linear(oi) >= 0) {
+    AttnP bw = p;
+    bw.dQ = bw.dK = bw.dV = p.O;
+    if (attention_bwd_takes_rowconst(bw)) ops[oi].rc_form = p.lse_neg_log2 = 1;
+  }
   RC(launch_attention_fwd(p, s));
   if (perturbed == PerturbState::IDENTITY) {
     p.B = B;
diff --git a/pea_diffusion_amd/csrc/gemm.hip b/pea_diffusion_amd/csrc/gemm.hip
--- a/pea_diffusion_amd/csrc/gemm.hip
+++ b/pea_diffusion_amd/csrc/gemm.hip
@@ -271,6 +271,65 @@
   constexpr bool LNF = EK == 1;
   typedef __attribute__((ext_vector_type(4))) unsigned u32x4;
   typedef __attribute__((ext_vector_type(2))) unsigned u32x2;
+  if constexpr (EK == 3) {
+    static_assert(NT == 5, "delta epilogue: 80-column wave tiles");
+    bf16x4 oq[MT][NT];
+#pragma unroll
+    for (int mt = 0; mt < MT; ++mt) {
+      const long long mo = (long long)min(m_base + mt * 16 + r16, p.M - 1) * p.lddo;
+#pragma unroll
+      for (int nt = 0; nt < NT; ++nt) oq[mt][nt] = *(const bf16x4*)(p.delta_o + mo + n_base + nt * 16 + 4 * q4);
+    }
+    __builtin_amdgcn_sched_barrier(0);
+    const int hA = n_base >> 6, ntB = 4 - ((n_base & 63) >> 4);
+    const int heads = p.delta_heads;
+#pragma unroll
+    for (int mt = 0; mt < MT; ++mt) {
+      const int m = m_base + mt * 16 + r16;
+      bf16* crow = (bf16*)p.C + (long long)min(m, p.M - 1) * p.ldc;
+      bf16x4 o[NT];
+      float sa = 0.f, sb = 0.f;
+#pragma unroll
+      for (int nt = 0; nt < NT; ++nt) {
+        float s = 0.f;
+#pragma unroll
+        for (int j = 0; j < 4; ++j) {
+          o[nt][j] = (bf16)(acc[nt][mt][j] * p.alpha);
+          s += (float)o[nt][j] * (float)oq[mt][nt][j];
+        }
+        if (nt < ntB) sa += s;
+        else sb += s;
+      }
+      if (m < p.M) {
+#pragma unroll
+        for (int nt = 0; nt + 1 < NT; nt += 2) {
+          union { bf16x4 h; unsigned u[2]; } a, b;
+          a.h = o[nt]; b.h = o[nt + 1];
+          const auto lo = __builtin_amdgcn_permlane16_swap(a.u[0], b.u[0], false, false);
+          const auto hi = __builtin_amdgcn_permlane16_swap(a.u[1], b.u[1], false, false);
+          const u32x4 oc = {lo[0], hi[0], lo[1], hi[1]};
+          epi_store16(crow + n_base + (nt + (q4 & 1)) * 16 + 8 * (q4 >> 1), oc);
+        }
+        union { bf16x4 h; u32x2 u; } ol;
+        ol.h = o[NT - 1];
+        epi_store8(crow + n_base + (NT - 1) * 16 + 4 * q4, ol.u);
+      }
+      sa += __shfl_xor(sa, 16); sa += __shfl_xor(sa, 32);
+      sb += __shfl_xor(sb, 16); sb += __shfl_xor(sb, 32);
+      if (m < p.M && q4 == 0) {
+        const int bi = m / p.delta_rows, qi = m - bi * p.delta_rows;
+        float* d0 = p.delta_out + ((long long)bi * heads + hA) * p.delta_rows + qi;
+        float* d1 = d0 + p.delta_stride;
+        if ((n_base & 63) == 0) { d0[0] = -sa; d1[0] = 0.f; }
+        else d1[0] = -sa;
+        d0[p.delta_rows] = -sb;
+        if ((n_base & 63) == 48) d1[p.delta_rows] = 0.f;
+      }
+#pragma unroll
+      for (int nt = 0; nt < NT; ++nt) epi_consumed(oq[mt][nt]);
+    }
+    return;
+  }
   f32x4 bq[NT];
 #pragma unroll
   for (int nt = 0; nt < NT; ++nt) bq[nt] = (f32x4){0.f, 0.f, 0.f, 0.f};
@@ -672,7 +731,7 @@
   __builtin_amdgcn_sched_group_barrier(0x008, MT * NT, 0);
 }
 template <int MODE, int BM, int BN, int WM, int WN, int LW, int S, bool PROBE16 = false, bool M16 = false, int MINW = 1,
-          bool LNF = false, bool KSW = false>
+          bool LNF = false, bool KSW = false, bool DLT = false>
 __global__ __launch_bounds__((WM * WN * (KSW ? 2 : 1) + LW) * 64, MINW) void gemm_lc_kernel(const bf16* pl_A, const bf16* pl_W, int pl_lda, int pl_ldw, int pl_M,
                                                                            int pl_N, int pl_K, int pl_ksplit, int pl_debug, const GemmP p_in) {
   GemmP p = p_in;
@@ -893,7 +952,18 @@
       for (int nt = 0; nt < NT; ++nt)
         wf[which][nt] = *(const bf16x8*)(tile + A_BYTES + swz_off(w_row0 + nt * 16, 4 * s2 + q4));
     };
+    [[maybe_unused]] unsigned o_touch[DLT ? MT : 1];
+    if constexpr (DLT) {
+      const int m0 = bm * BM + wr * (BM / WM), n0 = bn * BN + wc * (BN / WN);
+#pragma unroll
+      for (int mt = 0; mt < MT; ++mt)
+        o_touch[mt] = *(const unsigned*)(p.delta_o + (long long)min(m0 + mt * 16 + r16, p.M - 1) * p.lddo + n0 + 26 * q4);
+    }
     __builtin_amdgcn_s_barrier();
+    if constexpr (DLT) {
+#pragma unroll
+      for (int mt = 0; mt < MT; ++mt) epi_consumed(o_touch[mt]);
+    }
     load_frags(0, smem, 0);
     int cur = 0;
     for (int t = 0; t < nt; ++t) {
@@ -928,6 +998,10 @@
     }
     if constexpr (LNF) {
       gemm_epilogue16_lnf<MT, NT>(p, acc, bm * BM + wr * (BM / WM), bn * BN + wc * (BN / WN), r16, q4);
+      return;
+    }
+    if constexpr (DLT) {
+      gemm_epilogue16_fast<MT, NT, 3>(p, acc, bm * BM + wr * (BM / WM), bn * BN + wc * (BN / WN), r16, q4);
       return;
     }
     if (p.epi_fast) {
@@ -1006,20 +1080,20 @@
 }
 
 template <int MODE, int BM, int BN, int WM, int WN, int LW, int S, bool PROBE16 = false, bool M16 = false, int MINW = 1,
-          bool LNF = false, bool KSW = false>
+          bool LNF = false, bool KSW = false, bool DLT = false>
 static int launch_lc(const GemmP& p, hipStream_t stream) {
   constexpr int lds = S * (BM + BN) * 128;
   static_assert(lds <= 160 * 1024, "LDS budget");
   static_assert(!KSW || WM * WN * 2 * (BM / WM / 32) * (BN / WN / 16) * 1024 <= lds, "K-split exchange fits the ring");
   static bool attr_set = false;
   if (!attr_set) {
-    HIPCHK(hipFuncSetAttribute((const void*)gemm_lc_kernel<MODE, BM, BN, WM, WN, LW, S, PROBE16, M16, MINW, LNF, KSW>,
+    HIPCHK(hipFuncSetAttribute((const void*)gemm_lc_kernel<MODE, BM, BN, WM, WN, LW, S, PROBE16, M16, MINW, LNF, KSW, DLT>,
                                hipFuncAttributeMaxDynamicSharedMemorySize, lds));
     attr_set = true;
   }
   SHAPECHK(!KSW || (p.epi_fast && p.ksplit <= 1), "gemm: the K-split form needs the batched-load epilogue");
   const int grid = cdiv(p.M, BM) * cdiv(p.N, BN);
-  hipLaunchKernelGGL((gemm_lc_kernel<MODE, BM, BN, WM, WN, LW, S, PROBE16, M16, MINW, LNF, KSW>),
+  hipLaunchKernelGGL((gemm_lc_kernel<MODE, BM, BN, WM, WN, LW, S, PROBE16, M16, MINW, LNF, KSW, DLT>),
                      dim3(grid, p.ksplit > 1 ? p.ksplit : 1), dim3((WM * WN * (KSW ? 2 : 1) + LW) * 64), lds, stream, p.A, p.W, p.lda, p.ldw,
                      p.M, p.N, p.K, p.ksplit, p.debug, p);
   return PEA_OK;
@@ -1436,6 +1510,7 @@
 #undef X
   GEMM_GBWD_256 = 127, GEMM_GBWD_128 = 128, GEMM_GBWD_64 = 131,
   GEMM_LNF_LC256 = 224, GEMM_LNF_LC128 = 225, GEMM_LNF_256 = 227, GEMM_LNF_128 = 228, GEMM_LNF_64 = 231,
+  GEMM_DLT_LC256 = 324, GEMM_DLT_LC128 = 325,
 };
 static constexpr GemmInst kGemmInsts[] = {
 #define X(id, fn, cg, rf, gen, ...) GEMM_V##id,
@@ -1513,6 +1588,7 @@
   if (row && !row->colscale_geglu && (p.qscale_cols || p.geglu_y)) v = 28;
   if (row && !row->rowvec_fused && (p.gbwd_pre || p.ln_stats || (p.rowvec && epi_fast))) v = 28;
   if (p.ksplit > 1) v = 18;
+  if (p.delta_out) return {v == 24 || v == 27 ? GEMM_DLT_LC256 : GEMM_DLT_LC128, epi_fast};
   if (p.gbwd_pre) {
     return {v == 27 || v == 24 ? GEMM_GBWD_256 : (v == 31 ? GEMM_GBWD_64 : GEMM_GBWD_128), epi_fast};
   }
@@ -1561,6 +1637,14 @@
   return gemm_decide(p, cus, forced, gemm_env()).inst;
 }
 
+extern "C" int pea_debug_gemm_delta_dispatch(int M, int N, int K, int cus) {
+  GemmP p = {};
+  char* const base = (char*)(uintptr_t)0x1000;
+  p.M = M; p.N = N; p.K = K; p.alpha = 1.f; p.lda = K; p.ldw = K; p.rows_per_batch = M; p.C = base; p.ldc = N;
+  p.delta_o = (const bf16*)base; p.lddo = N; p.delta_out = (float*)base; p.delta_heads = N / 64; p.delta_rows = M;
+  return gemm_decide(p, cus, -1, gemm_env()).inst;
+}
+
 int launch_gemm(const GemmP& p_in, hipStream_t stream) {
   const GemmP& p0 = p_in;
   SHAPECHK(p0.M > 0 && p0.N > 0 && p0.K > 0, "gemm: empty problem M=%d N=%d K=%d", p0.M, p0.N, p0.K);
@@ -1606,6 +1690,15 @@
     SHAPECHK(p.split_stride >= (long long)(p.M - 1) * p.ldc + p.N && p.split_stride % 4 == 0,
              "gemm: split-K split_stride=%lld (M=%d N=%d ldc=%d): partials overlap or leave 16-byte alignment", p.split_stride, p.M, p.N, p.ldc);
   }
+  if (p.delta_out) {
+    SHAPECHK(p.delta_o && p.N % 320 == 0 && p.delta_heads * 64 == p.N && p.delta_rows > 0 && p.M % p.delta_rows == 0 && p.lddo % 4 == 0 && p.lddo >= p.N &&
+                 (((unsigned long long)p.delta_o & 7) == 0) && p.delta_stride >= (long long)(p.M / p.delta_rows) * (p.N / 64) * p.delta_rows,
+             "gemm: row constants in the epilogue need heads of width 64 in N %% 320 == 0 columns, O with lddo %% 4 == 0 and whole "
+             "samples (M=%d N=%d heads=%d delta_rows=%d lddo=%d)", p.M, p.N, p.delta_heads, p.delta_rows, p.lddo);
+    SHAPECHK(gemm_epi_fast(p, env) && p.mode == 0 && !p.bias && !p.res && !p.rowvec && !p.geglu_y && !p.gbwd_pre && !p.ln_stats && !p.qscale_cols && p.ksplit <= 1,
+             "gemm: row constants in the epilogue need the plain batched-load epilogue (bf16 output, no bias / activation / residual / row "
+             "vector / GEGLU / LayerNorm fold / column scale / split-K)");
+  }
   SHAPECHK(!(p.stash_grad && p.geglu_tanh), "gemm: the gradient-form GEGLU stash exists for the erf gate only (geglu_tanh set)");
   if (!g_num_cus) HIPCHK(gemm_query_cus());
   const GemmDecision d = gemm_decide(p, g_num_cus, g_gemm_variant, env);
@@ -1632,6 +1725,8 @@
     case GEMM_LNF_128: rc = launch_lcp<0, 128, 160, 4, 2, 4, 3, 0, 0, 2>(p, stream); break;
     case GEMM_LNF_64: rc = launch_lcp<0, 64, 160, 2, 2, 4, 4, 0, 0, 2>(p, stream); break;
     case GEMM_LNF_LC128: rc = launch_lc<0, 128, 160, 4, 2, 4, 3, false, true, 1, true>(p, stream); break;
+    case GEMM_DLT_LC256: rc = launch_lc<0, 256, 160, 4, 2, 4, 3, false, true, 1, false, false, true>(p, stream); break;
+    case GEMM_DLT_LC128: rc = launch_lc<0, 128, 160, 4, 2, 4, 3, false, true, 1, false, false, true>(p, stream); break;
   }
   PROF_END(stream);
   if (rc != PEA_OK) return rc;
diff --git a/pea_diffusion_amd/csrc/model.h b/pea_diffusion_amd/csrc/model.h
--- a/pea_diffusion_amd/csrc/model.h
+++ b/pea_diffusion_amd/csrc/model.h
@@ -146,6 +146,8 @@
   int qs_cols = 0; float qs = 1.f;
   int k2col = 0, v2col = 0;
   int pre = 0;
+  int rc_lin = -2;
+  int rc_form = 0;
   int stash_form = -1;
 };
 
@@ -277,6 +279,7 @@
   enum { AF_IP = 1, AF_REGIONS = 2, AF_MAPS = 4, AF_EDIT = 8, AF_STYLE = 16, AF_SAG = 32, AF_PERTURB = 64 };
   int attn_rules(unsigned which, bool forward, int arg = 0) const;
   int attn_forward(size_t oi, hipStream_t s);
+  int rowconst_linear(size_t oi);
   std::deque<WSlot> slots;
   std::map<std::string, int> slot_by_name;
   std::deque<FusedMat> fused;
diff --git a/pea_diffusion_amd/csrc/pea_kernels.h b/pea_diffusion_amd/csrc/pea_kernels.h
--- a/pea_diffusion_amd/csrc/pea_kernels.h
+++ b/pea_diffusion_amd/csrc/pea_kernels.h
@@ -35,6 +35,7 @@
   int qscale_cols; float qscale;
   int gbwd_form;
   const void* pf_ptr; long long pf_bytes;
+  const bf16* delta_o; int lddo; float* delta_out; int delta_heads, delta_rows; long long delta_stride;
 };
 int launch_splitk_reduce(const float* part, int nsplit, long long stride, bf16* out, int ldo, int M, int N, int accum,
                          hipStream_t s);
@@ -85,7 +86,10 @@
   float scale2;
   int nset; int set_end[4]; float set_w[4]; int k2_brows;
   const float* set_mask[4]; long long set_mstride[4];
-};
+  int lse_neg_log2;
+  int rowconst_ready;
+};
+bool attention_bwd_takes_rowconst(const AttnP& p);
 int attention_bwd_nsplit(int B, int H, int Sq, int Skv);
 size_t attention_bwd_scratch_bytes(int B, int H, int Sq, int Skv, int nd = 1);
 int launch_attention_fwd(const AttnP& p, hipStream_t s);
diff --git a/pea_diffusion_amd/csrc/tape.hip b/pea_diffusion_amd/csrc/tape.hip
--- a/pea_diffusion_amd/csrc/tape.hip
+++ b/pea_diffusion_amd/csrc/tape.hip
@@ -730,6 +730,7 @@
     return PEA_OK;
   };
   int dpre_of = -1;
+  int rc_for = -1;
   for (int oi = (int)ops.size() - 1; oi >= 0; --oi) {
     Op& o = ops[oi];
     if (o.kind == OP_CONV_OUT) {
@@ -798,6 +799,12 @@
           } else {
             p.C = a.g; p.ldc = a.cols;
             if (const bf16* ad = addend(a)) { p.res = ad; p.ldres = a.cols; }
+            if (prev && prev->kind == OP_ATTN && prev->rc_form && prev->out == o.a) {
+              SHAPECHK(rowconst_linear(oi - 1) == oi && !p.res && rc_for < 0, "unet: op %d cannot take the row constants of attention op %d", oi, oi - 1);
+              p.delta_o = a.d; p.lddo = a.cols; p.delta_out = delta; p.delta_heads = prev->p0; p.delta_rows = prev->p1;
+              p.delta_stride = (long long)Bb * prev->p0 * prev->p1;
+              rc_for = oi - 1;
+            }
             RC(gemm(p, s));
             a.gw = true;
           }
@@ -885,6 +892,9 @@
         p.O = out.d; p.ldo = out.cols; p.lse = o.aux; p.B = Bb; p.H = o.p0; p.Sq = o.p1; p.Skv = o.p2; p.scale = o.f0;
         p.nd = o.p3; p.q_prescaled = o.pre;
         p.dO = out.g; p.lddo = out.cols; p.delta = delta; p.dkv_part = attn_part;
+        SHAPECHK(rc_for < 0 || rc_for == oi, "unet: attention op %d runs between op %d and the GEMM that left its row constants", oi, rc_for);
+        SHAPECHK(!o.rc_form || rc_for == oi, "unet: attention op %d has no row constants from its output projection's dgrad", oi);
+        if (o.rc_form) { p.rowconst_ready = 1; rc_for = -1; }
         if (cross_kvlen && o.b == t_kvall) p.kv_len = cross_kvlen;
         SHAPECHK(!q.gw && !q.gpend && !k.gpend && (!k.gw || o.b == t_kvall), "unet: attention operand gradient written twice");
         if (q.rg) { p.dQ = q.g + o.acol; p.lddq = q.cols; }
diff --git a/pea_diffusion_amd/ops.py b/pea_diffusion_amd/ops.py
--- a/pea_diffusion_amd/ops.py
+++ b/pea_diffusion_amd/ops.py
@@ -59,6 +59,19 @@
     check(lib().pea_op_gemm_geglu_bwd(ptr(a), a.stride(0), ptr(w), w.stride(0), ptr(pre), pre.stride(0), ptr(out), out.stride(0),
                                       M, N, K, form, stream_ptr()))
     return out
+
+
+def gemm_delta(a, w, o, rows_per_sample, delta=None, features=0, out=None):
+    M, K = a.shape
+    N = w.shape[0]
+    heads = N // 64
+    if out is None:
+        out = torch.empty(M, N, device=a.device, dtype=torch.float32 if features & 1 else BF)
+    if delta is None:
+        delta = torch.empty(2, max(M // rows_per_sample, 1), max(heads, 1), rows_per_sample, device=a.device, dtype=torch.float32)
+    check(lib().pea_op_gemm_delta(ptr(a), a.stride(0), ptr(w), w.stride(0), ptr(out), out.stride(0), ptr(o), o.stride(0),
+                                  ptr(delta), delta.stride(0), M, N, K, heads, rows_per_sample, features, stream_ptr()))
+    return out, delta
 
 
 def ln_linear(x, gamma, beta, w, bias=None, eps=1e-5, geglu=False):
@@ -497,6 +510,23 @@
     return dq, dk, dv
 
 
+def attention_fwd_lse2(q, k, v, heads, scale=None):
+    B, Sq, C, scale, o, lse2 = _attn_fwd_out(q, heads, scale)
+    check(lib().pea_op_attention_fwd_lse2(ptr(q), q.stride(1), ptr(k), k.stride(1), ptr(v), v.stride(1), ptr(o), C, ptr(lse2),
+                                          B, heads, Sq, k.shape[1], scale, stream_ptr()))
+    return o, lse2
+
+
+def attention_bwd_rowconst(q, k, v, o, do, lse2, delta, heads, scale=None):
+    B, Sq, C = q.shape
+    scale = scale if scale is not None else (C // heads) ** -0.5
+    dq, dk, dv = torch.empty_like(q), torch.empty_like(k), torch.empty_like(v)
+    check(lib().pea_op_attention_bwd_rowconst(ptr(q), q.stride(1), ptr(k), k.stride(1), ptr(v), v.stride(1), ptr(o), C, ptr(do), C,
+                                              ptr(lse2), ptr(delta), ptr(dq), C, ptr(dk), C, ptr(dv), C, B, heads, Sq, k.shape[1],
+                                              scale, stream_ptr()))
+    return dq, dk, dv
+
+
 def attention_bwd_masked(q, k, v, o, do, lse, heads, scale=None, q_prescaled=False, kv_len=None, use_scratch=True):
     B, Sq, C = q.shape
     Skv = k.shape[1]
```
